# tsubo164/Fujiyama-Renderer

Hardware: AMD Instinct MI355X
Metric: Mray/s primary+secondary (and ms/frame) at 1920x1080 64spp (higher is better)
Workload: dtype f64; 1 GPU; dragon-class scene, 1920x1080, 8x8 spp, tile 32x32, 2040 tiles, 32 point lights; mesh=dragon, parallelism=tiles%1, tile_deal=auto, blas_build=host binned SAH

## Files before the change

### fujiyama-renderer_amd/csrc/device/fjgpu_api.hip

```cpp
#include <hip/hip_runtime.h>
#include <mutex>
#include <map>
#include <dlfcn.h>

#include <algorithm>
#include <array>
#include <atomic>
#include <cfloat>
#include <cmath>
#include <cstdio>
#include <cstdint>
#include <cstring>
#include <chrono>
#include <functional>
#include <memory>
#include <string>
#include <thread>
#include <vector>

#include "fjgpu.h"
#include "fjgpu_api_common.h"
#include "fjgpu_build.h"
#include "fjgpu_kernels.h"
#include "fjgpu_lbvh.h"
#include "fjgpu_light_cone.h"
#include "fjgpu_light_hull.h"
#include "fjgpu_matte.h"
#include "fjgpu_raysort.h"
#include "fjgpu_scene.h"
#include "fjgpu_tlas.h"

static thread_local std::string t_last_error;

int fjgpu::fail(int code, const std::string &msg)
{
  t_last_error = msg;
  return code;
}

namespace {

using fjgpu::fail;
using fjgpu::DeviceBuffers;

struct Rccl {
  typedef void *comm_t;
  int (*CommInitAll)(comm_t *, int, const int *) = nullptr;
  int (*CommDestroy)(comm_t) = nullptr;
  int (*GroupStart)() = nullptr;
  int (*GroupEnd)() = nullptr;
  int (*Send)(const void *, size_t, int, int, comm_t, hipStream_t) = nullptr;
  int (*Recv)(void *, size_t, int, int, comm_t, hipStream_t) = nullptr;
  const char *(*GetErrorString)(int) = nullptr;
  void *handle = nullptr;
  bool ok = false;
  static constexpr int kFloat = 7;
};

Rccl &rccl()
{
  static Rccl R;
  static std::once_flag once;
  std::call_once(once, []() {
    for (const char *name : {"librccl.so.1", "librccl.so", "/opt/rocm/lib/librccl.so.1"}) { R.handle = dlopen(name, RTLD_NOW | RTLD_LOCAL); if (R.handle) break; }
    if (!R.handle) return;
    auto sym = [&](const char *n) { return dlsym(R.handle, n); };
    R.CommInitAll = (decltype(R.CommInitAll)) sym("ncclCommInitAll");
    R.CommDestroy = (decltype(R.CommDestroy)) sym("ncclCommDestroy");
    R.GroupStart = (decltype(R.GroupStart)) sym("ncclGroupStart");
    R.GroupEnd = (decltype(R.GroupEnd)) sym("ncclGroupEnd");
    R.Send = (decltype(R.Send)) sym("ncclSend");
    R.Recv = (decltype(R.Recv)) sym("ncclRecv");
    R.GetErrorString = (decltype(R.GetErrorString)) sym("ncclGetErrorString");
    R.ok = R.CommInitAll && R.CommDestroy && R.GroupStart && R.GroupEnd && R.Send && R.Recv;
  });
  return R;
}

#define FJ_RCCL_RETRY_CALLS 64
// ... 176 lines not shown
int fjgpu_global_option(const char *name, long value)
{
  if (!name) return fail(FJGPU_EINVAL, "bad option call");
  if (std::string(name) == "ray_sort") { g_ray_sort = value < -1 ? -1 : (value > 9 ? 9 : value); return 0; }
  if (std::string(name) == "ray_sort_min") { g_ray_sort_min = value < 1 ? 1 : value; return 0; }
  if (std::string(name) == "device_tlas") { g_device_tlas = value != 0; return 0; }
  if (std::string(name) == "tlas_verify") { g_tlas_verify = value != 0; return 0; }
  if (std::string(name) == "split_shadow") { g_split_shadow = value != 0; return 0; }
  if (std::string(name) == "inst_lds") { g_inst_lds = value != 0; return 0; }
  if (std::string(name) == "curve_anyhit") { g_curve_anyhit = value != 0; return 0; }
  if (std::string(name) == "flat_groups") { g_flat_groups = value < 0 ? 0 : (value > 2 ? 2 : value); return 0; }
  if (std::string(name) == "compact_squeue") { g_compact_squeue = value != 0; return 0; }
  if (std::string(name) == "batch_tiles") { g_batch_tiles = value < 0 ? 0 : value; return 0; }
  if (std::string(name) == "device_build") { g_device_build = value < 0 ? -1 : (value > 2 ? 2 : value); return 0; }
  if (std::string(name) == "blas_treelet_passes") { g_treelet_passes = value < 0 ? 0 : (value > 8 ? 8 : value); return 0; }
  if (std::string(name) == "single_frame_build") { g_single_frame = value != 0; return 0; }
  if (std::string(name) == "speculative_walk") { g_spec_walk = value != 0; return 0; }
  if (std::string(name) == "anyhit_filter_off") { set_anyhit_filter_off(value); return 0; }
  if (std::string(name) == "cold_start") { g_cold_start = value != 0; return 0; }
  if (std::string(name) == "cold_batch_samples") { g_cold_batch_samples = value > 0 ? value : (long) FJ_COLD_BATCH_SAMPLES; return 0; }
  if (std::string(name) == "multi_exchange") { if (value < 0 || value > 1) return fail(FJGPU_EINVAL, "multi_exchange: 0 peer copies, 1 RCCL send / recv"); g_multi_exchange = value; return 0; }
  return fail(FJGPU_EINVAL, std::string("unknown global option ") + name);
}

const char *fjgpu_last_error(void) { return t_last_error.c_str(); }

int fjgpu_device_count(void)
{
  int n = 0;
  if (hipGetDeviceCount(&n) != hipSuccess) return 0;
  return n;
}

int fjgpu_tile_count(const fj_render_desc *render)
{
  if (!render) return 0;
  if (const char *why = bad_tiling(render)) { (void) fail(FJGPU_EINVAL, why); return 0; }
  std::vector<fjgpu::TileRect> t;
  fjgpu::GenerateTiles(*render, &t);
  return (int) t.size();
}

int fjgpu_tile_rect(const fj_render_desc *render, int tile_id, int32_t rect[4])
{
  if (!render || !rect) return fail(FJGPU_EINVAL, "null argument");
  if (const char *why = bad_tiling(render)) return fail(FJGPU_EINVAL, why);
  std::vector<fjgpu::TileRect> t;
  fjgpu::GenerateTiles(*render, &t);
  if (tile_id < 0 || tile_id >= (int) t.size()) return FJGPU_EINVAL;
  rect[0] = t[tile_id].xmin; rect[1] = t[tile_id].ymin; rect[2] = t[tile_id].xmax; rect[3] = t[tile_id].ymax;
  return 0;
}

}

static void build_light_hull_rows(const fjgpu::HostScene &hs, const std::vector<double> &cone_reach, std::vector<DLightCone> &hulls,
    std::vector<int32_t> &rows, int *n_rows, int *n_records)
{
  const size_t nl = hs.light_samples.size();
  rows.assign(hs.groups.size(), -1);
  hulls.clear();
  if (!hs.area_lights.empty()) return;
  for (size_t g = 0; g < hs.groups.size() && nl; g++) {
    if (hs.groups[g].n_instances != 1) continue;
    const DInstance &I = hs.instances[hs.group_members[hs.group_member_first[g]]];
    const fjgpu::HostPrimSet &ps = hs.primsets[I.primset];
    if (I.xform >= 0 || ps.type != FJ_PRIMSET_MESH || !ps.mesh || ps.mesh->velocity || ps.mesh->n_points <= 0) continue;
    std::vector<size_t> lights;
    for (size_t l = 0; l < nl; l++) if (hs.light_samples[l].type == FJ_POINT_LIGHT) lights.push_back(l);
    if (lights.empty()) continue;
    const size_t nv = (size_t) ps.mesh->n_points, nk = lights.size();
    const size_t chunk = 16384, nchunks = (nv + chunk - 1) / chunk;
    size_t workers = std::min(16u, std::max(1u, std::thread::hardware_concurrency()));
    if (const char *omp = getenv("OMP_NUM_THREADS")) { const long v = atol(omp); if (v >= 1) workers = std::min<size_t>(workers, (size_t) v); }
    const unsigned hc = (unsigned) std::max<size_t>(1, std::min(workers, nchunks));
    auto over_chunks = [&](const std::function<void(size_t)> &fn) {
      std::atomic<size_t> next(0);
      std::vector<std::thread> th;
      for (unsigned t = 0; t < hc; t++) th.emplace_back([&]() { for (size_t c; (c = next.fetch_add(1)) < nchunks;) fn(c); });
      for (auto &t : th) t.join();
    };
    std::vector<double> W(3 * nv), csum(3 * nchunks, 0.);
    over_chunks([&](size_t c) {
      double s[3] = {0., 0., 0.};
      for (size_t i = c * chunk; i < std::min(nv, (c + 1) * chunk); i++) {
        light_hull_world(I.M, ps.mesh->P + 3 * i, &W[3 * i]);
        for (int k = 0; k < 3; k++) s[k] += W[3 * i + k];
      }
      for (int k = 0; k < 3; k++) csum[3 * c + k] = s[k];
    });
    double ctr[3] = {0., 0., 0.};
    for (size_t c = 0; c < nchunks; c++) for (int k = 0; k < 3; k++) ctr[k] += csum[3 * c + k];
    for (int k = 0; k < 3; k++) ctr[k] /= (double) nv;
    std::vector<LightHullAcc> acc(nk), part(nk * nchunks);
    for (size_t k = 0; k < nk; k++) light_hull_frame(hs.light_samples[lights[k]].P, ctr, &acc[k]);
    over_chunks([&](size_t c) {
      for (size_t k = 0; k < nk; k++) {
        LightHullAcc A = acc[k];
        for (size_t i = c * chunk; i < std::min(nv, (c + 1) * chunk) && A.ok; i++) light_hull_add(&A, &W[3 * i]);
        part[k * nchunks + c] = A;
      }
    });
    for (size_t k = 0; k < nk; k++) for (size_t c = 0; c < nchunks; c++) light_hull_merge(&acc[k], &part[k * nchunks + c]);
    const size_t at = hulls.size();
    hulls.resize(at + nl);
    std::memset(&hulls[at], 0, nl * sizeof(DLightCone));
// ... 134 lines not shown
    const fj_texture_desc &t = desc->textures[i];
    dtex[i].width = t.width; dtex[i].height = t.height; dtex[i].nchannels = t.nchannels; dtex[i].tilesize = t.tilesize;
    const size_t n = (t.width && t.tiles) ? (size_t) (t.width / t.tilesize) * (t.height / t.tilesize) * t.tilesize * t.tilesize * t.nchannels : 0;
    e |= M.upload(t.tiles, n, &dtex[i].tiles);
    if (!dtex[i].tiles) dtex[i].width = dtex[i].height = 0;
  }
  DScene &S = sc->S;
  std::memset(&S, 0, sizeof(S));
  {
    std::vector<std::array<double, 6>> qgrid(dps.size());
    for (size_t i = 0; i < dps.size(); i++) {
      DPrimSet &P = dps[i];
      P.qnodes = nullptr;
      if (P.type != FJ_PRIMSET_MESH || P.n_prims == 0 || e) continue;
      const size_t n_nodes = std::max<size_t>(1, hs.primsets[i].nodes.size());
      for (int a = 0; a < 3; a++) {
        qgrid[i][a] = P.bounds[a];
        qgrid[i][3 + a] = std::max(1e-300, (P.bounds[3 + a] - P.bounds[a]) / 65535. * (1 + 1e-9));
      }
      DNodeQ *q = nullptr;
      if (M.alloc(n_nodes, &q)) { e = 1; continue; }
      if (launch_quantize_nodes(nullptr, P.nodes, (uint32_t) n_nodes, &qgrid[i][0], &qgrid[i][3], q)) e = 1;
      P.qnodes = q;
    }
    std::vector<const DNodeQ *> cq(dps.size(), nullptr);
    for (size_t i = 0; FJ_CURVE_QNODES && FJ_CLOSEST_QNODES && i < dps.size(); i++) {
      const DPrimSet &P = dps[i];
      if (P.type != FJ_PRIMSET_CURVE || P.n_prims == 0 || e) continue;
      const size_t n_nodes = std::max<size_t>(1, hs.primsets[i].nodes.size());
      for (int a = 0; a < 3; a++) {
        const double pad = 1e-4 * std::max(1., P.bounds[3 + a] - P.bounds[a]);
        qgrid[i][a] = P.bounds[a] - pad;
        qgrid[i][3 + a] = std::max(1e-300, (P.bounds[3 + a] - P.bounds[a] + 2 * pad) / 65535. * (1 + 1e-9));
      }
      DNodeQ *q = nullptr;
      if (M.alloc(n_nodes, &q)) { e = 1; continue; }
      if (launch_quantize_nodes(nullptr, P.nodes, (uint32_t) n_nodes, &qgrid[i][0], &qgrid[i][3], q)) e = 1;
      cq[i] = q;
    }
    lap("quantised nodes");
    e |= M.upload(dps.data(), dps.size(), &S.primsets);
    {
      std::vector<DInstance> di = hs.instances;
      for (DInstance &I : di) {
        const DPrimSet &P = dps[I.primset];
        std::memcpy(I.pbounds, P.bounds, sizeof(I.pbounds));
        I.pnodes = P.nodes; I.proot = P.root; I.pn_prims = P.n_prims;
        I.pqnodes = P.qnodes ? P.qnodes : cq[I.primset];
        I.sh_indices = P.indices; I.sh_N = P.N; I.sh_vN = P.vN; I.sh_uv = P.uv; I.sh_face_group = P.face_group; I.sh_type = P.type; I.sh_pad = 0;
        for (int k = 0; k < 3; k++) { I.qorigin[k] = qgrid[I.primset][k]; I.qcell[k] = qgrid[I.primset][3 + k]; }
      }
      e |= M.upload(di.data(), di.size(), &S.instances);
      std::vector<DInstEntry> ie(di.size());
      bool any_curves = false, any_motion = !hs.xforms.empty();
      for (const auto &ps : hs.primsets) {
        if (ps.type == FJ_PRIMSET_CURVE && ps.n_prims > 0) any_curves = true;
        if (!ps.tri_vel.empty() || !ps.curve_vel.empty()) any_motion = true;
      }
      for (size_t k = 0; k < di.size(); k++) {
        const DInstance &I = di[k];
        DInstEntry &E = ie[k];
        std::memcpy(E.Minv, I.Minv, sizeof(E.Minv));
        std::memcpy(E.pbounds, I.pbounds, sizeof(E.pbounds));
        for (int a = 0; a < 3; a++) { E.tbounds[a] = -INFINITY; E.tbounds[3 + a] = INFINITY; }
        if (I.xform < 0 && I.pn_prims > 0) {
          double mn[3] = {INFINITY, INFINITY, INFINITY}, mx[3] = {-INFINITY, -INFINITY, -INFINITY};
          for (int c = 0; c < 8; c++) {
            const double p[3] = {I.pbounds[(c & 1) ? 3 : 0], I.pbounds[(c & 2) ? 4 : 1], I.pbounds[(c & 4) ? 5 : 2]};
            for (int a = 0; a < 3; a++) {
              const double w = I.M[4 * a] * p[0] + I.M[4 * a + 1] * p[1] + I.M[4 * a + 2] * p[2] + I.M[4 * a + 3];
              mn[a] = std::min(mn[a], w); mx[a] = std::max(mx[a], w);
            }
          }
          bool finite = true;
          for (int a = 0; a < 3; a++) finite = finite && std::isfinite(mn[a]) && std::isfinite(mx[a]);
          if (finite)
            for (int a = 0; a < 3; a++) {
              const double pad = 1e-7 * (mx[a] - mn[a]) + 1e-7 * std::max(std::fabs(mn[a]), std::fabs(mx[a])) + 1e-9;
              E.tbounds[a] = mn[a] - pad; E.tbounds[3 + a] = mx[a] + pad;
            }
        }
        for (int a = 0; a < 3; a++) { E.qorigin[a] = I.qorigin[a]; E.qcell[a] = I.qcell[a]; }
        const DPrimSet &P = dps[I.primset];
        const bool quantised = FJ_CLOSEST_QNODES && (!any_curves || FJ_CURVE_QNODES) && !any_motion;
        E.nodes = quantised ? (const void *) I.pqnodes : (const void *) I.pnodes;
        E.ptype = P.type; E.pad = 0;
        E.proot = I.proot; E.pn_prims = I.pn_prims; E.primset = I.primset; E.xform = I.xform;
        E.tri_verts = P.tri_verts; E.tri_verts32 = P.type == FJ_PRIMSET_CURVE ? P.curve_capsule : P.tri_verts32; E.tri_vel = P.tri_vel; E.prim_ids = P.prim_ids;
      }
      e |= M.upload(ie.data(), ie.size(), &S.inst_entries);
    }
    uintptr_t lo = UINTPTR_MAX, hi = 0;
    auto tris_of = [](const DPrimSet &P) { return (uintptr_t) (P.tri_verts32 ? (const void *) P.tri_verts32 : (const void *) P.tri_verts); };
    for (size_t i = 0; i < dps.size(); i++) {
      const DPrimSet &P = dps[i];
      if (!P.qnodes) continue;
      const uintptr_t pn = (uintptr_t) P.qnodes, pt = tris_of(P);
      lo = std::min(lo, std::min(pn, pt)); hi = std::max(hi, std::max(pn, pt));
    }
    bool fits = lo != UINTPTR_MAX && lo % 128 == 0 && (hi - lo) / 128 < 0xffffffffull;
    for (size_t i = 0; i < dps.size(); i++) {
      const DPrimSet &P = dps[i];
      if (P.qnodes && (((uintptr_t) P.qnodes - lo) % 128 != 0 || (tris_of(P) - lo) % 128 != 0)) fits = false;
    }
    for (const DPrimSet &P : dps) if (P.qnodes && !P.tri_verts32) fits = false;
    S.blas_base = fits ? (const char *) lo : nullptr;
    if (!fits && lo != UINTPTR_MAX && getenv("FJGPU_VERBOSE"))
      fprintf(stderr, "fjgpu: BLAS arrays span %zu bytes from %p: no 32-bit offsets, the general shadow walk is used\n", (size_t) (hi - lo), (void *) lo);
    std::vector<DAnyInst> ai(hs.instances.size());
    for (size_t i = 0; i < hs.instances.size(); i++) {
      const DInstance &I = hs.instances[i];
      const DPrimSet &P = dps[I.primset];
      DAnyInst &a = ai[i];
      std::memset(&a, 0, sizeof(a));
      std::memcpy(a.Minv, I.Minv, sizeof(a.Minv));
      std::memcpy(a.bounds, P.bounds, sizeof(a.bounds));
      a.root = P.root;
      a.n_prims = (P.qnodes && S.blas_base) ? P.n_prims : 0;
      if (a.n_prims) {
        for (int k = 0; k < 3; k++) { a.qorigin[k] = qgrid[I.primset][k]; a.qcell[k] = qgrid[I.primset][3 + k]; }
        a.node_base = (uint32_t) (((uintptr_t) P.qnodes - lo) / 128);
        a.tri_base = (uint32_t) ((tris_of(P) - lo) / 128);
        a.tris_f32 = P.tri_verts32 ? 1 : 0;
        double bm = 0;
        for (int k = 0; k < 6; k++) bm = std::max(bm, std::fabs(P.bounds[k]));
        a.fbound = std::nextafter((float) bm, INFINITY);
      }
    }
    e |= M.upload(ai.data(), ai.size(), &S.any_insts);
  }
  if (g_device_tlas && e == 0 && !hs.groups.empty()) {
    std::vector<int> mcount(hs.groups.size()), nfirst, ncount;
    for (size_t g = 0; g < hs.groups.size(); g++) mcount[g] = hs.groups[g].n_instances;
    DTNode *d_nodes = nullptr;
    std::string terr;
    if (TlasBuildDevice(S.instances, hs.group_members, hs.group_member_first, mcount, &nfirst, &ncount, &d_nodes, &terr))
      return fail(FJGPU_ENODEV, terr);
    M.ptrs.push_back(d_nodes);
    size_t total = 0;
    for (int c : ncount) total += (size_t) c;
    if (g_tlas_verify) {
      std::vector<DTNode> got(total);
      HIP_TRY(hipMemcpy(got.data(), d_nodes, total * sizeof(DTNode), hipMemcpyDeviceToHost));
      bool same = total == hs.group_nodes.size();
      for (size_t g = 0; same && g < hs.groups.size(); g++) same = nfirst[g] == hs.groups[g].first && ncount[g] == hs.groups[g].count;
      if (same && total) same = std::memcmp(got.data(), hs.group_nodes.data(), total * sizeof(DTNode)) == 0;
      if (!same) return fail(FJGPU_ENODEV, "device TLAS build differs from the host's build");
    }
    std::vector<DGroup> groups = hs.groups;
    for (size_t g = 0; g < groups.size(); g++) { groups[g].first = nfirst[g]; groups[g].count = ncount[g]; }
    e |= M.upload(groups.data(), groups.size(), &S.groups);
    S.group_nodes = d_nodes;
    S.n_group_nodes = (int32_t) total;
  } else {
    e |= M.upload(hs.groups.data(), hs.groups.size(), &S.groups);
    e |= M.upload(hs.group_nodes.data(), hs.group_nodes.size(), &S.group_nodes);
    S.n_group_nodes = (int32_t) hs.group_nodes.size();
  }
  static_assert(sizeof(DInstEntry) == 8 * FJ_INST_LDS_ENTRY_WORDS && sizeof(DTNode) == 56 && sizeof(DGroup) == 64, "LDS copy of the instance level");
  S.curve_anyhit = (g_curve_anyhit && !getenv("FJGPU_NO_CURVE_ANYHIT")) ? 1 : 0;
  S.inst_lds = (g_inst_lds && !getenv("FJGPU_NO_INST_LDS")) ? 1 : 0;
  e |= M.upload(hs.shaders.data(), hs.shaders.size(), &S.shaders);
  e |= M.upload(hs.xforms.data(), hs.xforms.size(), &S.xforms);
  S.cam_xform = nullptr;
  if (!hs.cam_static) e |= M.upload(&hs.cam_xform, 1, &S.cam_xform);
  S.has_motion = hs.xforms.empty() ? 0 : 1;
  for (const auto &ps : hs.primsets) if (!ps.tri_vel.empty() || !ps.curve_vel.empty()) S.has_motion = 1;
  S.multi_shadow_groups = 0;
  for (const DInstance &I : hs.instances) {
    bool gathers = false;
    for (int k = 0; k < I.n_shaders; k++)
      if (I.shaders[k] >= 0 && (hs.shaders[I.shaders[k]].type == FJ_SHADER_PLASTIC || hs.shaders[I.shaders[k]].type == FJ_SHADER_HAIR)) gathers = true;
    if (gathers && I.shadow_target >= 0 && I.shadow_target < (int) hs.groups.size() && hs.groups[I.shadow_target].n_instances > 1)
      S.multi_shadow_groups = 1;
  }
  S.time_tab = nullptr; S.time_start = 0; S.time_end = 0;
  S.lrec_hair = nullptr;
  e |= M.upload(dtex.data(), dtex.size(), &S.textures);
  e |= M.upload(hs.light_samples.data(), hs.light_samples.size(), &S.light_samples);
  e |= M.upload(hs.area_lights.data(), hs.area_lights.size(), &S.area_lights);
  S.light_cones = nullptr; S.cone_rows = nullptr;
  std::vector<double> cone_reach;
  {
    const size_t nl = hs.light_samples.size();
    std::vector<int32_t> rows(hs.groups.size(), -1);
    std::vector<DLightCone> cones;
    cone_reach.assign(hs.groups.size(), -1.);
    for (size_t g = 0; g < hs.groups.size() && nl; g++) {
      if (hs.groups[g].n_instances != 1) continue;
      const size_t at = cones.size();
      cones.resize(at + nl);
      int built = 0;
      double reach = 1e300;
      for (size_t l = 0; l < nl; l++) {
        DLightCone &C = cones[at + l];
        const DLightSample &LS = hs.light_samples[l];
        if (LS.type == FJ_POINT_LIGHT || LS.type == FJ_DOME_LIGHT) light_cone_build(LS.P, hs.groups[g].sbounds, &C);
        else std::memset(&C, 0, sizeof(C));
        if (C.count > 0) { built++; reach = std::min(reach, C.reach); }
      }
      if (!built) { cones.resize(at); continue; }
      for (size_t l = 0; l < nl; l++) cones[at + l].reach = reach;
      rows[g] = (int32_t) (at / nl);
      cone_reach[g] = reach;
      sc->cone_rows++; sc->cone_records += built;
    }
    if (!cones.empty()) {
      e |= M.upload(cones.data(), cones.size(), &S.light_cones);
      e |= M.upload(rows.data(), rows.size(), &S.cone_rows);
    }
  }
  S.light_hulls = nullptr; S.hull_rows = nullptr;
  {
// ... 187 lines not shown
  for (hipEvent_t e : scene->ev_frame) if (e) (void) hipEventDestroy(e);
  for (hipEvent_t e : scene->ev_pool) (void) hipEventDestroy(e);
  if (scene->d_frame) (void) hipFree(scene->d_frame);
  if (scene->d_slab) (void) hipFree(scene->d_slab);
  if (scene->d_rects) (void) hipFree(scene->d_rects);
  delete scene;
}

int fjgpu_host_instance_level(const fj_scene_desc *desc, int group, int32_t *out_inst, int32_t *out_skip, double *out_box, int cap)
{
  if (!desc || group < 0 || group >= desc->n_groups) return fail(FJGPU_EINVAL, "bad instance-level query");
  fjgpu::HostScene hs;
  std::string err;
  const int e = fjgpu::BuildHostScene(desc, &hs, &err, true);
  if (e) return fail(e, err);
  const DGroup &G = hs.groups[group];
  for (int k = 0; k < G.count && k < cap; k++) {
    const DTNode &nd = hs.group_nodes[G.first + k];
    if (out_inst) out_inst[k] = nd.inst;
    if (out_skip) out_skip[k] = nd.inst < 0 ? nd.skip - G.first : 0;
    if (out_box) std::memcpy(out_box + 6 * (size_t) k, nd.box, sizeof(nd.box));
  }
  return G.count;
}

int fjgpu_host_light_hulls(const fj_scene_desc *desc, int group, void *out_records, double *out_Pl, int cap, double *out_M)
{
  if (!desc || group < 0 || group >= desc->n_groups) return fail(FJGPU_EINVAL, "bad light-hull query");
  fjgpu::HostScene hs;
  std::string err;
  const int e = fjgpu::BuildHostScene(desc, &hs, &err, true);
  if (e) return fail(e, err);
  std::vector<int32_t> rows;
  std::vector<DLightCone> hulls;
  int n_rows = 0, n_records = 0;
  std::vector<double> cone_reach(hs.groups.size(), -1.);
  for (size_t g = 0; g < hs.groups.size(); g++) cone_reach[g] = box_cone_row_reach(hs, g);
  build_light_hull_rows(hs, cone_reach, hulls, rows, &n_rows, &n_records);
  if (out_M) {
    if (hs.groups[group].n_instances != 1) return fail(FJGPU_EINVAL, "light-hull query: the group has several instances");
    std::memcpy(out_M, hs.instances[hs.group_members[hs.group_member_first[group]]].M, 12 * sizeof(double));
  }
  const size_t nl = hs.light_samples.size();
  for (size_t l = 0; l < nl && (int) l < cap; l++) {
    if (out_records) {
      if (rows[group] >= 0) std::memcpy((char *) out_records + l * sizeof(DLightCone), &hulls[(size_t) rows[group] * nl + l], sizeof(DLightCone));
      else std::memset((char *) out_records + l * sizeof(DLightCone), 0, sizeof(DLightCone));
    }
    if (out_Pl) for (int k = 0; k < 3; k++) out_Pl[3 * l + k] = hs.light_samples[l].P[k];
  }
  return (int) nl;
}

int fjgpu_host_curve_blas(const fj_scene_desc *desc, int curve_set, int32_t *out_curve, float *out_capsule, int32_t *out_depth,
                          float *out_box, int cap, int32_t *out_grid_n, double *out_grid_cell, double *out_bounds)
{
  if (!desc || curve_set < 0 || curve_set >= desc->n_curves) return fail(FJGPU_EINVAL, "bad curve-BLAS query");
  fjgpu::HostPrimSet ps;
  std::string err;
  const int e = fjgpu::BuildCurveSet(desc->curves[curve_set], &ps, &err);
  if (e) return fail(e, err);
  const int n = ps.n_prims;
  for (int k = 0; k < 3; k++) {
    if (out_grid_n) out_grid_n[k] = ps.grid_n[k];
    if (out_grid_cell) out_grid_cell[k] = ps.grid_cell[k];
  }
  if (out_bounds) std::memcpy(out_bounds, ps.bounds, sizeof(ps.bounds));
  for (int s = 0; s < n && s < cap; s++) {
    if (out_curve) out_curve[s] = (int32_t) ps.prim_ids[s];
    if (out_capsule) std::memcpy(out_capsule + 7 * (size_t) s, &ps.curve_capsule[(size_t) s * 8], 7 * sizeof(float));
    if (out_depth) out_depth[s] = ps.curve_depth[s];
  }
  if (out_box && n > 0) {
    if (ps.root & FJ_LEAF_FLAG) {
      if (cap > 0) for (int k = 0; k < 6; k++) out_box[k] = (float) ps.bounds[k];
    } else {
      std::vector<char> seen((size_t) n, 0);
      std::vector<uint32_t> todo(1, ps.root);
      while (!todo.empty()) {
        const uint32_t at = todo.back();
        todo.pop_back();
        if (at >= ps.nodes.size()) return fail(FJGPU_EINVAL, "curve-BLAS query: node index out of range");
        const DNode &nd = ps.nodes.data()[at];
        for (int k = 0; k < 4; k++) {
          const uint32_t c = nd.child[k];
          if (c == FJ_NO_CHILD) continue;
          if (!(c & FJ_LEAF_FLAG)) { todo.push_back(c); continue; }
          const uint32_t first = (c & ~FJ_LEAF_FLAG) >> 3, count = (c & 7u) + 1;
          for (uint32_t s = first; s < first + count && s < (uint32_t) n; s++) {
            seen[s] = 1;
            if ((int) s < cap) for (int a = 0; a < 3; a++) { out_box[6 * (size_t) s + a] = nd.box[k][2 * a]; out_box[6 * (size_t) s + 3 + a] = nd.box[k][2 * a + 1]; }
          }
        }
      }
      for (int s = 0; s < n; s++) if (!seen[s]) return fail(FJGPU_EINVAL, "curve-BLAS query: a slot has no leaf");
    }
  }
  return n;
}

int fjgpu_build_config(const char *name, double *value)
{
  if (!name || !value) return fail(FJGPU_EINVAL, "bad build_config call");
  if (!kernels_build_config(name, value)) return fail(FJGPU_EINVAL, std::string("unknown build_config name ") + name);
  return 0;
}
// ... 5 lines not shown
  if (n == "node_record_bytes") { *value = (double) sizeof(DNode); return 0; }
  if (n == "anyhit_node_record_bytes") { *value = (double) sizeof(DNodeQ); return 0; }
  if (n == "tri_record_bytes") { *value = scene->tri_record_bytes; return 0; }
  if (n == "scene_bytes") { *value = (double) scene->mem.bytes; return 0; }
  if (n == "work_bytes") { *value = (double) (scene->work ? scene->work->bytes : 0); return 0; }
  if (n == "stack_need") { *value = scene->stack_need; return 0; }
  if (n == "sampler_seed") { *value = (double) scene->sampler_seed; return 0; }
  if (n == "blas_nodes") { *value = (double) scene->blas_nodes; return 0; }
  if (n == "blas_treelet_passes") { *value = (double) scene->blas_treelet_passes; return 0; }
  if (n == "blas_treelets_changed") { *value = (double) scene->blas_treelets_changed; return 0; }
  if (n == "blas_sah_cost_initial") { *value = scene->blas_sah_cost_initial; return 0; }
  if (n == "blas_sah_cost") { *value = scene->blas_sah_cost; return 0; }
  if (n == "stack_peak") { *value = (double) std::max(scene->stack_peak_closest, scene->stack_peak_shadow); return 0; }
  if (n == "stack_peak_closest") { *value = (double) scene->stack_peak_closest; return 0; }
  if (n == "stack_peak_shadow") { *value = (double) scene->stack_peak_shadow; return 0; }
  if (n == "stack_lds") { *value = FJ_STACK_LDS; return 0; }
  if (n == "stack_lds_anyhit") { *value = FJ_STACK_LDS_ANYHIT; return 0; }
  if (n == "stack_lds_curves") { *value = FJ_STACK_LDS_CURVES; return 0; }
  if (n == "stack_lds_canyhit") { *value = FJ_STACK_LDS_CANYHIT; return 0; }
  if (n == "stack_lds_min") { *value = FJ_STACK_LDS_MIN; return 0; }
  if (n == "curve_anyhit") {
    const DScene &S = scene->S;
    *value = (S.has_curves && !S.has_motion && S.all_opaque && S.curve_anyhit && S.inst_lds && S.n_group_nodes <= FJ_INST_LDS_NODES_CURVES &&
              S.n_instances <= FJ_INST_LDS_INSTS_CURVES && S.n_groups <= FJ_INST_LDS_GROUPS_CURVES && FJ_CURVE_QNODES && FJ_CLOSEST_QNODES) ? 1 : 0;
    return 0;
  }
  if (n == "lean_anyhit") { *value = (scene->S.all_opaque && !scene->S.has_curves && !scene->S.has_motion && scene->S.blas_base) ? 1 : 0; return 0; }
  if (n == "closest_kernel") {
    const DScene &S = scene->S;
    const bool flat = !S.has_motion && !S.has_curves && S.flats;
    *value = S.has_motion ? 3 : (S.has_curves ? 2 : (flat ? 4 : (S.incoherent_rays ? 1 : 0)));
    return 0;
  }
  if (n == "closest_node_record_bytes") { *value = (double) ((scene->S.has_motion || (scene->S.has_curves && !FJ_CURVE_QNODES) || !FJ_CLOSEST_QNODES) ? sizeof(DNode) : sizeof(DNodeQ)); return 0; }
  if (n == "light_cone_rows") { *value = scene->cone_rows; return 0; }
  if (n == "light_cone_records") { *value = scene->cone_records; return 0; }
  if (n == "light_cone_verdicts" || n == "light_cone_contradictions") {
    double v = -1, c = -1;
    if (hipSetDevice(scene->device) != hipSuccess || hipDeviceSynchronize() != hipSuccess) return fail(FJGPU_ENODEV, "hipSetDevice / hipDeviceSynchronize");
    light_cone_validate_counts(&v, &c);
    *value = n == "light_cone_verdicts" ? v : c;
    return 0;
  }
  if (n == "light_hull_rows") { *value = scene->hull_rows; return 0; }
  if (n == "light_hull_records") { *value = scene->hull_records; return 0; }
  if (n == "light_hull_verdicts" || n == "light_hull_contradictions") {
    double v = -1, c = -1;
    if (hipSetDevice(scene->device) != hipSuccess || hipDeviceSynchronize() != hipSuccess) return fail(FJGPU_ENODEV, "hipSetDevice / hipDeviceSynchronize");
    light_hull_validate_counts(&v, &c);
    if (n == "light_hull_verdicts") *value = v >= 0 ? v : (double) scene->hull_verdicts;
    else *value = c;
    return 0;
  }
  {
    static const char *const tf[5] = {"tri_filter_miss", "tri_filter_hit", "tri_filter_maybe", "tri_filter_exact_hits", "tri_filter_contradictions"};
    for (int k = 0; k < 5; k++)
      if (n == tf[k]) {
        double c[5];
        if (hipSetDevice(scene->device) != hipSuccess || hipDeviceSynchronize() != hipSuccess) return fail(FJGPU_ENODEV, "hipSetDevice / hipDeviceSynchronize");
        tri_filter_validate_counts(c);
        *value = c[k];
        return 0;
      }
  }
  if (n == "accum_memsets") { *value = (double) scene->accum_memsets; return 0; }
  if (n == "has_curves") { *value = scene->S.has_curves; return 0; }
  if (n == "has_motion") { *value = scene->S.has_motion; return 0; }
  return fail(FJGPU_EINVAL, "unknown query " + n);
}

int fjgpu_set_batch_callback(fjgpu_scene *scene, fjgpu_batch_fn fn, void *user)
{
  if (!scene) return fail(FJGPU_EINVAL, "null scene");
  scene->batch_fn = fn; scene->batch_user = fn ? user : nullptr;
  return 0;
}

int fjgpu_dev_rccl_selftest(int device, int n_floats)
{
  int nd = 0;
  if (hipGetDeviceCount(&nd) != hipSuccess || device < 0 || device >= nd) return fail(FJGPU_ENODEV, "no such HIP device");
  if (n_floats < 1) return fail(FJGPU_EINVAL, "bad size");
  HIP_TRY(hipSetDevice(device));
  std::string why;
  const std::vector<Rccl::comm_t> *comms = rccl_comms(std::vector<int>{device}, &why);
  if (!comms) return fail(FJGPU_ENODEV, "RCCL: " + why);
  Rccl &R = rccl();
  DeviceBuffers M;
  std::vector<float> src((size_t) n_floats), got((size_t) n_floats, -1.f);
  for (int i = 0; i < n_floats; i++) src[(size_t) i] = (float) (i % 1013) * .5f;
  const float *d_src = nullptr;
  float *d_dst = nullptr;
  if (M.upload(src.data(), src.size(), &d_src) || M.alloc(src.size(), &d_dst)) return fail(FJGPU_ENOMEM, "device allocation failed");
  HIP_TRY(hipMemset(d_dst, 0xff, sizeof(float) * src.size()));
  int e = R.GroupStart();
  if (!e) e = R.Send(d_src, src.size(), Rccl::kFloat, 0, (*comms)[0], nullptr);
  if (!e) e = R.Recv(d_dst, src.size(), Rccl::kFloat, 0, (*comms)[0], nullptr);
  const int e2 = R.GroupEnd();
  if (e || e2) return fail(FJGPU_ENODEV, std::string("RCCL self exchange: ") + (R.GetErrorString ? R.GetErrorString(e ? e : e2) : "error"));
  HIP_TRY(hipStreamSynchronize(nullptr));
  HIP_TRY(hipMemcpy(got.data(), d_dst, sizeof(float) * got.size(), hipMemcpyDeviceToHost));
  for (size_t i = 0; i < got.size(); i++) if (got[i] != src[i]) return fail(FJGPU_ENODEV, "RCCL self exchange returned other data");
  return 0;
}

int fjgpu_dev_sort_pairs(int device, const uint32_t *keys, int n, int key_bits, uint32_t *keys_out, uint32_t *perm, int repeats, double *sort_ms)
// ... 28 lines not shown
  if (sort_ms) *sort_ms = best;
  if (keys_out) HIP_TRY(hipMemcpy(keys_out, d_out, sizeof(uint32_t) * (size_t) n, hipMemcpyDeviceToHost));
  if (perm) HIP_TRY(hipMemcpy(perm, d_perm, sizeof(uint32_t) * (size_t) n, hipMemcpyDeviceToHost));
  return 0;
}

int fjgpu_dev_slab32_batch(int device, int n, const double *rays, const double *grid, const uint32_t *words, void *out)
{
  if (n < 0 || (n > 0 && (!rays || !grid || !words || !out))) return fail(FJGPU_EINVAL, "bad slab32 batch call");
  int nd = 0;
  if (hipGetDeviceCount(&nd) != hipSuccess || device < 0 || device >= nd) return fail(FJGPU_ENODEV, "no such HIP device");
  HIP_TRY(hipSetDevice(device));
  if (n == 0) return 0;
  DeviceBuffers M;
  const double *d_rays = nullptr, *d_grid = nullptr;
  const uint32_t *d_words = nullptr;
  char *d_out = nullptr;
  if (M.upload(rays, (size_t) n * 8, &d_rays) || M.upload(grid, (size_t) n * 6, &d_grid) || M.upload(words, (size_t) n * 3, &d_words) || M.alloc((size_t) n * 128, &d_out))
    return fail(FJGPU_ENOMEM, "device allocation failed for the slab32 batch");
  if (launch_slab32_batch(nullptr, (uint32_t) n, d_rays, d_grid, d_words, d_out)) return fail(FJGPU_ENODEV, "the slab32 batch launch failed");
  HIP_TRY(hipStreamSynchronize(nullptr));
  HIP_TRY(hipMemcpy(out, d_out, (size_t) n * 128, hipMemcpyDeviceToHost));
  return 0;
}

int fjgpu_dev_quantize_nodes(int device, int n, const void *nodes, const double *origin, const double *cell, void *out)
{
  if (n < 0 || !origin || !cell || (n > 0 && (!nodes || !out))) return fail(FJGPU_EINVAL, "bad quantize call");
  int nd = 0;
  if (hipGetDeviceCount(&nd) != hipSuccess || device < 0 || device >= nd) return fail(FJGPU_ENODEV, "no such HIP device");
  HIP_TRY(hipSetDevice(device));
  if (n == 0) return 0;
  DeviceBuffers M;
  const DNode *d_nodes = nullptr;
  DNodeQ *d_out = nullptr;
  if (M.upload((const DNode *) nodes, (size_t) n, &d_nodes) || M.alloc((size_t) n, &d_out)) return fail(FJGPU_ENOMEM, "device allocation failed for the quantiser");
  if (launch_quantize_nodes(nullptr, d_nodes, (uint32_t) n, origin, cell, d_out)) return fail(FJGPU_ENODEV, "the quantiser's launch failed");
  HIP_TRY(hipStreamSynchronize(nullptr));
  HIP_TRY(hipMemcpy(out, d_out, sizeof(DNodeQ) * (size_t) n, hipMemcpyDeviceToHost));
  return 0;
}

int fjgpu_set_option(fjgpu_scene *scene, const char *name, long value)
{
  if (!scene || !name) return fail(FJGPU_EINVAL, "bad option call");
  const std::string n(name);
  if (n == "batch_tiles") { scene->batch_tiles = value; return 0; }
  if (n == "batch_samples") { scene->batch_samples = value < 0 ? 0 : value; return 0; }
  if (n == "aov_batch_samples") { scene->aov_batch_samples = value < 0 ? 0 : value; return 0; }
  if (n == "count_nodes") { scene->count_events = value != 0; return 0; }
  if (n == "count_all_shadow") { scene->count_all_shadow = value != 0; return 0; }
  if (n == "light_cones") { scene->light_cones = value != 0; return 0; }
  if (n == "light_hulls") { scene->light_hulls = value != 0; return 0; }
  if (n == "shade_first_touch") {
    if (value != 0 && value != 1) return fail(FJGPU_EINVAL, "shade_first_touch: 0 (memset and atomic adds at the camera level) or 1 (one store per sample)");
    scene->shade_first_touch = value;
    return 0;
  }
  if (n == "sampler_seed") {
    if (value < 0 || value > 65535) return fail(FJGPU_EINVAL, "sampler_seed: " + std::to_string(value) + " is outside 0..65535 (0: the unseeded streams)");
    scene->sampler_seed = value;
    return 0;
  }
  if (n == "overlap_shadow") {
    if (value < 0 || value > 2) return fail(FJGPU_EINVAL, "overlap_shadow: 0 off, 1 on, 2 by the batch size");
    scene->overlap = value;
    return 0;
  }
  if (n == "release_work") {
    if (value && scene->work) {
      if (hipSetDevice(scene->device) != hipSuccess) return fail(FJGPU_ENODEV, "hipSetDevice");
      (void) hipDeviceSynchronize();
      fjgpu::ForgetWorkArena(scene);
    }
    return 0;
  }
  return fail(FJGPU_EINVAL, "unknown option " + n);
}

int fjgpu_render_frame_multi(fjgpu_scene *const *scenes, int n_scenes, const fj_render_desc *r,
    const int32_t *tile_ids, int n_tiles, float *h_fb, fjgpu_stats *stats)
{
  if (!scenes || n_scenes < 1 || !r || !h_fb) return fail(FJGPU_EINVAL, "null argument");
  for (int k = 0; k < n_scenes; k++) if (!scenes[k]) return fail(FJGPU_EINVAL, "null scene");
  if (const char *why = bad_render(r)) return fail(FJGPU_EINVAL, why);
  std::vector<fjgpu::TileRect> all;
  fjgpu::GenerateTiles(*r, &all);
  std::vector<int32_t> ids;
  if (const int e = listed_tiles(tile_ids, n_tiles, all.size(), &ids)) return e;
  const int G = n_scenes;
  const size_t npx = (size_t) r->xres * r->yres;
  const int tile_px = r->tile_w * r->tile_h;
  std::vector<std::vector<int32_t>> mine(G);
  for (size_t k = 0; k < ids.size(); k++) mine[k % G].push_back(ids[k]);
  fjgpu_scene *first = scenes[0];

  HIP_TRY(hipSetDevice(first->device));
  if (grow((void **) &first->d_frame, &first->d_frame_n, npx * 4, sizeof(float))) return fail(FJGPU_ENOMEM, "device allocation failed for the frame");
  HIP_TRY(hipMemset(first->d_frame, 0, npx * 4 * sizeof(float)));
  std::vector<size_t> stage_off(G, 0);
  size_t stage_px = 0, rects_n = 0;
  for (int d = 1; d < G; d++) { stage_off[d] = stage_px; stage_px += mine[d].size() * (size_t) tile_px; rects_n += mine[d].size(); }
  if (G > 1) {
    if (grow((void **) &first->d_slab, &first->d_slab_n, stage_px * 4, sizeof(float)) ||
        grow((void **) &first->d_rects, &first->d_rects_n, rects_n * 4, sizeof(int32_t)))
      return fail(FJGPU_ENOMEM, "device allocation failed for the tile slabs");
// ... 113 lines not shown
  return fjgpu_render_frame_multi(one, 1, r, nullptr, 0, h_fb, stats);
}

int fjgpu_trace(fjgpu_scene *sc, int group, int n, const double *rays, double *out_t, int32_t *out_ids,
    double *out_uv, fjgpu_stats *stats)
{
  if (!sc || !rays || !out_t || !out_ids || n < 0) return fail(FJGPU_EINVAL, "null argument");
  if (group < 0 || group >= sc->S.n_groups) return fail(FJGPU_EINVAL, "group out of range");
  if (n == 0) return 0;
  HIP_TRY(hipSetDevice(sc->device));
  DeviceBuffers W;
  DRay *d_rays; DHit *d_hits; DCounters *d_cnt;
  double *d_ranges;
  if (W.alloc((size_t) n, &d_rays) || W.alloc((size_t) n * 2, &d_ranges) || W.alloc((size_t) n, &d_hits) || W.alloc(1, &d_cnt))
    return fail(FJGPU_ENOMEM, "device allocation failed");
  {
    std::vector<DRay> hr((size_t) n);
    std::vector<double> hg((size_t) n * 2);
    for (int i = 0; i < n; i++) {
      for (int k = 0; k < 3; k++) { hr[i].o[k] = rays[8 * (size_t) i + k]; hr[i].d[k] = rays[8 * (size_t) i + 3 + k]; }
      hg[2 * (size_t) i] = rays[8 * (size_t) i + 6]; hg[2 * (size_t) i + 1] = rays[8 * (size_t) i + 7];
    }
    HIP_TRY(hipMemcpy(d_rays, hr.data(), sizeof(DRay) * (size_t) n, hipMemcpyHostToDevice));
    HIP_TRY(hipMemcpy(d_ranges, hg.data(), sizeof(double) * 2 * (size_t) n, hipMemcpyHostToDevice));
  }
  HIP_TRY(hipMemset(d_cnt, 0, sizeof(DCounters)));
  DScene S = sc->S;
  S.target_group = group;
  S.trace_ranges = d_ranges;
  hipEvent_t e0, e1;
  HIP_TRY(hipEventCreate(&e0));
  HIP_TRY(hipEventCreate(&e1));
  (void) hipEventRecord(e0, nullptr);
  const int le = launch_trace_closest(nullptr, S, d_rays, nullptr, d_hits, (uint32_t) n, d_cnt, (int) sc->count_events);
  (void) hipEventRecord(e1, nullptr);
  if (le) return fail(FJGPU_ENODEV, std::string("trace launch: ") + hipGetErrorString((hipError_t) le));
  HIP_TRY(hipDeviceSynchronize());
  float ms = 0;
  (void) hipEventElapsedTime(&ms, e0, e1);
  (void) hipEventDestroy(e0); (void) hipEventDestroy(e1);
  std::vector<DHit> h((size_t) n);
  HIP_TRY(hipMemcpy(h.data(), d_hits, sizeof(DHit) * (size_t) n, hipMemcpyDeviceToHost));
  for (int i = 0; i < n; i++) {
    out_t[i] = h[i].inst >= 0 ? h[i].t : DBL_MAX;
    out_ids[2 * i] = h[i].inst;
    out_ids[2 * i + 1] = h[i].inst >= 0 ? h[i].prim : -1;
    if (out_uv) { out_uv[2 * i] = h[i].inst >= 0 ? h[i].u : 0; out_uv[2 * i + 1] = h[i].inst >= 0 ? h[i].v : 0; }
  }
  sc->stack_peak_closest = sc->stack_peak_shadow = 0;
  DCounters hc;
  if (stats || sc->count_events) {
    HIP_TRY(hipMemcpy(&hc, d_cnt, sizeof(hc), hipMemcpyDeviceToHost));
    sc->stack_peak_closest = hc.stack_peak;
  }
  if (stats) {
    std::memset(stats, 0, sizeof(*stats));
    stats->nodes_visited = hc.nodes; stats->prims_tested = hc.prims; stats->insts_tested = hc.insts; stats->rays_traced = hc.traced;
    stats->trace_ms = ms; stats->total_ms = ms; stats->trace_launches = 1;
  }
  return 0;
}

#ifndef FJ_AOV_BATCH_SAMPLES
#define FJ_AOV_BATCH_SAMPLES ((long) 4 << 20)
#endif

struct AovSetup {
  std::vector<fjgpu::TileRect> all;
  int margin[2];
  GenParams gp;
  DScene S;
};
static int aov_setup(fjgpu_scene *sc, const fj_render_desc *r, const char *who, AovSetup *a)
{
  if (r->sampler_type == 1) return fail(FJGPU_EUNSUPPORTED, std::string(who) + ": the adaptive sampler is not supported (fixed-grid sampler only)");
  if (r->sampler_type != 0) return fail(FJGPU_EINVAL, "unknown sampler_type");
  if (const char *why = bad_render(r)) return fail(FJGPU_EINVAL, why);
  if (sc->S.cam_xform) return fail(FJGPU_EUNSUPPORTED, std::string(who) + ": a time-sampled camera is not supported (static cameras only)");
  if (sc->S.has_motion) return fail(FJGPU_EUNSUPPORTED, std::string(who) + ": a scene with motion (time-sampled transforms or vertex velocities) is not supported (static scenes only)");
  fjgpu::GenerateTiles(*r, &a->all);
  fjgpu::SamplerMargin(*r, a->margin);
  a->gp = gen_params(r, a->margin);
  a->S = sc->S;
  camera_uv_size(sc->cam_fov, r, a->S.cam_uv_size);
  a->S.time_start = r->time_start; a->S.time_end = r->time_end;
  a->S.lrec_hair = nullptr;
  a->S.cam_uv = nullptr; a->S.cam_tk = nullptr; a->S.cam_slot0 = 0;
  a->S.trace_ranges = nullptr; a->S.trace_n_dev = nullptr; a->S.ray_perm = nullptr;
  a->S.shadow_join = nullptr;
  return 0;
}

struct MatteCall { const fjgpu_matte_desc *desc; const fjgpu_matte_buffers *out; };
static int render_aov_body(const char *who_, fjgpu_scene *sc, const fj_render_desc *r, const int32_t *tile_ids, int n_tiles,
    const fjgpu_aov_buffers *out, float *d_albedo, void *hip_stream, fjgpu_stats *stats, const MatteCall *matte = nullptr)
{
  const std::string who(who_);
  const bool reduce = out && (out->depth || out->position || out->normal || out->uv || out->ids || out->coverage);
  if (!reduce && !d_albedo && !matte) return fail(FJGPU_EINVAL, who + ": every buffer pointer is NULL, nothing to write");
  if (tile_ids && n_tiles < 0) return fail(FJGPU_EINVAL, who + ": negative tile count");
  AovSetup A;
  if (const int e = aov_setup(sc, r, who_, &A)) return e;
  HIP_TRY(hipSetDevice(sc->device));
  hipStream_t st = static_cast<hipStream_t>(hip_stream);

  std::vector<int32_t> ids;
// ... 226 lines not shown
```

### fujiyama-renderer_amd/csrc/device/fjgpu_dev_math.h

```cpp
#ifndef FJGPU_DEV_MATH_H
#define FJGPU_DEV_MATH_H

#include "fjgpu_slab32.h"
__device__ __forceinline__ V3 mk(double x, double y, double z) { V3 r; r.x = x; r.y = y; r.z = z; return r; }
__device__ __forceinline__ V3 operator+(V3 a, V3 b) { return mk(a.x + b.x, a.y + b.y, a.z + b.z); }
__device__ __forceinline__ V3 operator-(V3 a, V3 b) { return mk(a.x - b.x, a.y - b.y, a.z - b.z); }
__device__ __forceinline__ V3 operator*(V3 a, double s) { return mk(a.x * s, a.y * s, a.z * s); }
__device__ __forceinline__ V3 operator*(double s, V3 a) { return mk(a.x * s, a.y * s, a.z * s); }
__device__ __forceinline__ double dot(V3 a, V3 b) { return a.x * b.x + a.y * b.y + a.z * b.z; }
__device__ __forceinline__ V3 cross(V3 a, V3 b) { return mk(a.y * b.z - a.z * b.y, a.z * b.x - a.x * b.z, a.x * b.y - a.y * b.x); }
__device__ __forceinline__ V3 normalize(V3 a)
{
  const double len = sqrt(dot(a, a));
  if (len == 0) return a;
  const double inv = 1. / len;
  return a * inv;
}
#define FJ_GLOBAL __attribute__((address_space(1)))
typedef float fj_v4f __attribute__((ext_vector_type(4)));
typedef uint32_t fj_v4u __attribute__((ext_vector_type(4)));

__device__ __forceinline__ V3 ld3(const double *p) { return mk(p[0], p[1], p[2]); }
__device__ __forceinline__ V3 ld3(const FJ_GLOBAL double *p) { return mk(p[0], p[1], p[2]); }
#define FJ_G(T, ptr) ((const FJ_GLOBAL T *) (ptr))
// ... 100 lines not shown
    *v0 = mk(p[0], p[1], p[2]); *v1 = mk(p[3], p[4], p[5]); *v2 = mk(p[6], p[7], p[8]);
  }
}

__device__ __forceinline__ bool tri_ray(V3 v0, V3 v1, V3 v2, V3 orig, V3 dir, double *t, double *u, double *v)
{
  const V3 edge1 = v1 - v0;
  const V3 edge2 = v2 - v0;
  const V3 pvec = cross(dir, edge2);
  const double det = dot(edge1, pvec);
  if (det > -1e-6 && det < 1e-6) return false;
  const double inv_det = 1.0 / det;
  const V3 tvec = orig - v0;
  const double uu = dot(tvec, pvec) * inv_det;
  if (uu < 0.0 || uu > 1.0) return false;
  const V3 qvec = cross(tvec, edge1);
  const double vv = dot(dir, qvec) * inv_det;
  if (vv < 0.0 || uu + vv > 1.0) return false;
  *t = dot(edge2, qvec) * inv_det;
  *u = uu;
  *v = vv;
  return true;
}

__device__ __forceinline__ bool tri_ray_early(V3 v0, V3 v1, V3 v2, V3 orig, V3 dir, double *t, double *u, double *v)
{
  const V3 edge1 = v1 - v0;
  const V3 edge2 = v2 - v0;
  const V3 pvec = cross(dir, edge2);
  const double det = dot(edge1, pvec);
  if (det > -1e-6 && det < 1e-6) return false;
  const double adet = fabs(det);
  const V3 tvec = orig - v0;
  const double U = dot(tvec, pvec);
  const double aU = fabs(U);
  if (((U < 0.0) != (det < 0.0)) ? aU > 1e-100 * adet : aU > adet * (1.0 + 1e-10)) return false;
  const V3 qvec = cross(tvec, edge1);
  const double V = dot(dir, qvec);
  const double aV = fabs(V);
  if (((V < 0.0) != (det < 0.0)) ? aV > 1e-100 * adet : aV > adet * (1.0 + 1e-10)) return false;
  const double inv_det = 1.0 / det;
  const double uu = U * inv_det;
  if (uu < 0.0 || uu > 1.0) return false;
  const double vv = V * inv_det;
  if (vv < 0.0 || uu + vv > 1.0) return false;
  *t = dot(edge2, qvec) * inv_det;
  *u = uu;
  *v = vv;
  return true;
}

struct Best { double t, u, v; int inst, prim; };

struct LocalCounters { uint32_t nodes, prims, insts, stack_peak; };

__device__ __forceinline__ unsigned long long wave_sum(unsigned long long v)
{
  for (int off = 32; off > 0; off >>= 1) {
    const unsigned lo = __shfl_xor((unsigned) (v & 0xffffffffull), off);
    const unsigned hi = __shfl_xor((unsigned) (v >> 32), off);
    v += ((unsigned long long) hi << 32) | lo;
  }
  return v;
}

__device__ __forceinline__ void flush_counters(DCounters *cnt, unsigned long long nodes, unsigned long long prims,
    unsigned long long insts, unsigned long long traced, unsigned long long shadow)
{
  nodes = wave_sum(nodes); prims = wave_sum(prims); insts = wave_sum(insts);
  traced = wave_sum(traced); shadow = wave_sum(shadow);
  if (__lane_id() == 0) {
    if (nodes) atomicAdd(&cnt->nodes, nodes);
    if (prims) atomicAdd(&cnt->prims, prims);
    if (insts) atomicAdd(&cnt->insts, insts);
    if (traced) atomicAdd(&cnt->traced, traced);
    if (shadow) atomicAdd(&cnt->rays[CXT_SHADOW_RAY], shadow);
  }
}

__device__ __forceinline__ void flush_stack_peak(unsigned long long *peak, uint32_t v)
{
  for (int off = 32; off > 0; off >>= 1) { const uint32_t o = __shfl_xor(v, off); v = o > v ? o : v; }
  if (__lane_id() == 0 && v) atomicMax(peak, (unsigned long long) v);
}

__device__ __forceinline__ void flush_shadow_walk_counters(DCounters *cnt, unsigned long long nodes, unsigned long long prims,
    unsigned long long insts)
{
  nodes = wave_sum(nodes); prims = wave_sum(prims); insts = wave_sum(insts);
  if (__lane_id() == 0) {
    if (nodes) atomicAdd(&cnt->sh_nodes, nodes);
    if (prims) atomicAdd(&cnt->sh_prims, prims);
    if (insts) atomicAdd(&cnt->sh_insts, insts);
  }
}

#endif
```

### fujiyama-renderer_amd/csrc/device/fjgpu_dev_shadow.h

```cpp
#ifndef FJGPU_DEV_SHADOW_H
#define FJGPU_DEV_SHADOW_H

#ifndef SQ_CHUNK
#define SQ_CHUNK 512u
#endif
#ifndef JQ_CHUNK
#define JQ_CHUNK 64u
#endif
#define SQ_INVALID 0xffffffffu
__device__ __forceinline__ const DShadowRayC *sq_c(const DShadowRay *squeue, uint32_t i) { return (const DShadowRayC *) squeue + i; }
#define SQ_FIELD(S, squeue, i, f) ((S).compact_squeue ? sq_c(squeue, i)->f : (squeue)[i].f)
__device__ __forceinline__ const float *sq_colour(const DScene &S, const DShadowRay *squeue, uint32_t i) { return S.compact_squeue ? sq_c(squeue, i)->c : squeue[i].c; }
__device__ __forceinline__ void sq_ray(const DScene &S, const DShadowRay *squeue, uint32_t i, V3 *o, V3 *d, double *tmax)
{
  if (!S.compact_squeue) {
    const DShadowRay *q = &squeue[i];
    *o = mk(q->o[0], q->o[1], q->o[2]); *d = mk(q->d[0], q->d[1], q->d[2]); *tmax = q->tmax;
    return;
  }
  const DShadowRayC *q = sq_c(squeue, i);
  const V3 Ps = mk(q->o[0], q->o[1], q->o[2]);
  const DLightSample *LS = &S.light_samples[q->light];
  const V3 Pl = mk(LS->P[0], LS->P[1], LS->P[2]);
  V3 Ln = mk(Pl.x - Ps.x, Pl.y - Ps.y, Pl.z - Ps.z);
// ... 422 lines not shown
  const DShadowRay *squeue;
  float *s_accum;
  __device__ bool fetch(uint32_t i, RayIn *r) const
  {
    const DShadowRay q = squeue[i];
    if (q.sample == SQ_INVALID) return false;
    r->o = mk(q.o[0], q.o[1], q.o[2]); r->d = mk(q.d[0], q.d[1], q.d[2]);
    r->tmin = .0001; r->tmax = q.tmax;
    r->time = S->has_motion ? sample_time(*S, q.tindex) : 0.;
    r->group = q.group;
    r->anyhit = S->groups[q.group].all_opaque != 0;
    return true;
  }
  __device__ void finish(uint32_t i, const Best &b) const
  {
    float ac = 1.f;
    if (b.inst >= 0) {
      float Os = 1.f;
      const DInstance *I = &S->instances[b.inst];
      const DPrimSet *P = &S->primsets[I->primset];
      const int sg = (P->face_group && b.prim >= 0) ? P->face_group[b.prim] : 0;
      int sid;
      if (sg < 0 || sg >= I->n_shaders) sid = I->shaders[0];
      else { sid = I->shaders[sg]; if (sid < 0) sid = I->shaders[0]; }
      if (sid >= 0 && S->shaders[sid].type == FJ_SHADER_PLASTIC) Os = S->shaders[sid].opacity;
      Os = (float) clampd(Os, 0, 1);
      ac = 1 - Os;
    }
    if (ac == 0.f) return;
    const DShadowRay *q = &squeue[i];
    const float r0 = q->c[0] * ac, r1 = q->c[1] * ac, r2 = q->c[2] * ac;
    float *acc = s_accum + 4 * (size_t) q->sample;
    if (r0 != 0.f) atomicAdd(acc + 0, r0);
    if (r1 != 0.f) atomicAdd(acc + 1, r1);
    if (r2 != 0.f) atomicAdd(acc + 2, r2);
  }
};

template <bool kCurves, bool kCount, bool kMotion, bool kInstLds = false, bool kAnyOnly = false>
__global__ void __launch_bounds__(BLOCK, kMotion ? FJ_MOTION_MINB : (kCurves ? FJ_CURVE_MINB : FJ_SHADOW_MINB)) k_shadow_trace(DScene S, const DShadowRay *squeue, float *s_accum,
    DCounters *cnt, TravTune tune)
{
  __shared__ uint32_t s_stack[(kCurves ? FJ_STACK_LDS_CURVES : FJ_STACK_LDS) * BLOCK];
  __shared__ double s_rayspace[kCurves ? FJ_RAYSPACE_DOUBLES * BLOCK : 1];
  __shared__ double s_inst[kInstLds ? InstLdsOf<kCurves>::T::WORDS : 1];
  if (kInstLds) InstLdsOf<kCurves>::T::fill(S, s_inst);
  const uint32_t n = cnt->shadow_count;
  ShadowPolicy pol;
  pol.S = &S; pol.squeue = squeue; pol.s_accum = s_accum;
  LocalCounters lc = {0, 0, 0, 0};
  traverse_persistent<kCurves, kCount, kMotion, kInstLds, kAnyOnly>(S, pol, tune, n, &cnt->shadow_xcd_head[0][0], make_stack(s_stack, S.stack_overflow_shadow, kCurves ? s_rayspace : nullptr), &lc, s_inst);
  if (kCount) {
    flush_counters(cnt, lc.nodes, lc.prims, lc.insts, 0, 0);
    flush_stack_peak(&cnt->sh_stack_peak, lc.stack_peak);
    flush_shadow_walk_counters(cnt, lc.nodes, lc.prims, lc.insts);
    if (blockIdx.x == 0 && threadIdx.x == 0) atomicAdd(&cnt->squeued, (unsigned long long) n);
  }
}

#endif
```

### fujiyama-renderer_amd/csrc/device/fjgpu_dev_traverse.h

```cpp
#ifndef FJGPU_DEV_TRAVERSE_H
#define FJGPU_DEV_TRAVERSE_H

#define TRAV_DONE 0xffffffffu
#ifndef FJ_TINY_PRIMS
#define FJ_TINY_PRIMS 4
#endif
#ifdef FJ_PHASE_STATS
__device__ unsigned long long g_phase[16];
#endif
#ifdef FJ_WAVE_TIMELINE
#define FJ_TL_WAVES 8192
__device__ unsigned long long g_timeline[FJ_TL_WAVES * 6];
struct WaveTimeline {
  unsigned long long t0, tdry, tclaim;
  uint32_t iters, tail, iclaim, worst_ticks, worst_iters, claims;
  __device__ __forceinline__ void begin() { t0 = tclaim = wall_clock64(); tdry = 0; iters = tail = iclaim = worst_ticks = worst_iters = claims = 0; }
  __device__ __forceinline__ void iter(bool dry) { iters++; if (dry) { if (!tdry) tdry = wall_clock64(); tail++; } }
  __device__ __forceinline__ void claim()
  {
    const unsigned long long now = wall_clock64();
    const uint32_t d = (uint32_t) (now - tclaim);
    if (claims && d > worst_ticks) { worst_ticks = d; worst_iters = iters - iclaim; }
    tclaim = now; iclaim = iters; claims++;
  }
  __device__ __forceinline__ void end()
  {
    claim();
    const uint32_t w = blockIdx.x * (BLOCK / 64) + (threadIdx.x >> 6);
    if (__lane_id() == 0 && w < FJ_TL_WAVES) {
      const unsigned long long t1 = wall_clock64();
      g_timeline[6 * w + 0] = t0; g_timeline[6 * w + 1] = tdry ? tdry : t1; g_timeline[6 * w + 2] = t1;
      g_timeline[6 * w + 3] = ((unsigned long long) iters << 32) | tail;
      g_timeline[6 * w + 4] = ((unsigned long long) worst_ticks << 32) | worst_iters;
      g_timeline[6 * w + 5] = claims;
    }
  }
};
__device__ unsigned long long g_rayhist[64];
#ifdef FJ_RAY_HIST
#define FJ_TL_RAY(steps) do { const uint32_t s_ = (steps); const int b_ = 31 - __clz((int) (s_ | 1u)); atomicAdd(&g_rayhist[b_], 1ull); atomicAdd(&g_rayhist[32 + b_], (unsigned long long) s_); } while (0)
#else
#define FJ_TL_RAY(steps) do { } while (0)
#endif
#define FJ_TL_CLAIM() tl_.claim()
#define FJ_TL_DECL() WaveTimeline tl_; tl_.begin()
#define FJ_TL_ITER(dry) tl_.iter(dry)
#define FJ_TL_END() tl_.end()
#else
#define FJ_TL_RAY(steps) do { } while (0)
#define FJ_TL_CLAIM() do { } while (0)
#define FJ_TL_DECL() do { } while (0)
#define FJ_TL_ITER(dry) do { } while (0)
#define FJ_TL_END() do { } while (0)
#endif
struct TravTune { uint32_t refill, steps, grab, leaf_wait, min_inner, anyhit_steps, refill_curves, steps_curves, steps_phased, min_inner_phased, refill_canyhit, steps_canyhit, min_inner_canyhit, leaf_wait_canyhit, refill_flat, steps_flat, min_inner_flat, leaf_bias8, leaf_bias8_flat, leaf_bias8_phased, leaf_bias8_canyhit, exact_min, filter_off; };
#define TRAV_REFILL tune.refill
#define TRAV_STEPS (int) tune.steps
#define TRAV_GRAB tune.grab

__device__ __forceinline__ uint32_t adaptive_grab(uint32_t grab, uint32_t n)
{
// ... 51 lines not shown
  uint32_t ovf_stride;
  double *rayspace;
  int lds_n;
  __device__ __forceinline__ void push(int &sp, uint32_t v) const
  {
    if (sp < lds_n) lds[sp * BLOCK] = v;
    else ovf[(size_t) (sp - lds_n) * ovf_stride] = v;
    sp++;
  }
  __device__ __forceinline__ uint32_t pop(int &sp) const
  {
    --sp;
    uint32_t v;
    if (sp < lds_n) v = lds[sp * BLOCK];
    else v = ovf[(size_t) (sp - lds_n) * ovf_stride];
    return v;
  }
};
__device__ __forceinline__ TravStack make_stack(uint32_t *s_stack, uint32_t *ovf, double *s_rayspace = nullptr, int lds_entries = 0)
{
  TravStack st;
  st.lds = (trav_lds_u32 *) (s_stack + threadIdx.x);
  st.lds_n = lds_entries ? lds_entries : (s_rayspace ? FJ_STACK_LDS_CURVES : FJ_STACK_LDS);
  st.rayspace = s_rayspace ? s_rayspace + threadIdx.x : nullptr;
  st.ovf_stride = gridDim.x * BLOCK;
  st.ovf = ovf ? (FJ_GLOBAL uint32_t *) (ovf + (size_t) blockIdx.x * BLOCK + threadIdx.x) : nullptr;
  return st;
}

template <int NODES_, int INSTS_, int GROUPS_> struct InstLdsT {
  static constexpr int NODES = NODES_, INSTS = INSTS_, GROUPS = GROUPS_;
  static constexpr int ENTRIES_AT = NODES * 7, GROUPS_AT = ENTRIES_AT + INSTS * FJ_INST_LDS_ENTRY_WORDS;
  static constexpr int WORDS = GROUPS_AT + GROUPS * 8;
  static bool fits(const DScene &S)
  {
    return S.inst_lds && S.n_group_nodes <= NODES && S.n_instances <= INSTS && S.n_groups <= GROUPS;
  }
  static __device__ __forceinline__ void fill(const DScene &S, double *s_inst)
  {
    const unsigned long long *src_n = (const unsigned long long *) S.group_nodes, *src_e = (const unsigned long long *) S.inst_entries;
    const unsigned long long *src_g = (const unsigned long long *) S.groups;
    unsigned long long *dst = (unsigned long long *) s_inst;
    for (uint32_t w = threadIdx.x; w < (uint32_t) S.n_group_nodes * 7u; w += BLOCK) dst[w] = src_n[w];
    for (uint32_t w = threadIdx.x; w < (uint32_t) S.n_instances * FJ_INST_LDS_ENTRY_WORDS; w += BLOCK) dst[ENTRIES_AT + w] = src_e[w];
    for (uint32_t w = threadIdx.x; w < (uint32_t) S.n_groups * 8u; w += BLOCK) dst[GROUPS_AT + w] = src_g[w];
    __syncthreads();
  }
};
typedef InstLdsT<FJ_INST_LDS_NODES, FJ_INST_LDS_INSTS, FJ_INST_LDS_GROUPS> InstLds;
typedef InstLdsT<FJ_INST_LDS_NODES_BIG, FJ_INST_LDS_INSTS_BIG, FJ_INST_LDS_GROUPS_BIG> InstLdsBig;
typedef InstLdsT<FJ_INST_LDS_NODES_CURVES, FJ_INST_LDS_INSTS_CURVES, FJ_INST_LDS_GROUPS_CURVES> InstLdsCurves;
template <bool kCurves> struct InstLdsOf { typedef InstLdsBig T; };
template <> struct InstLdsOf<true> { typedef InstLdsCurves T; };

template <bool kCurves, bool kCount, bool kMotion, bool kInstLds, bool kAnyOnly, class Policy>
__device__ void traverse_persistent(const DScene &S, Policy &pol, TravTune tune, uint32_t n, uint32_t *head, TravStack stk, LocalCounters *lc, const double *s_inst)
{
  const DTNode *gnodes = kInstLds ? (const DTNode *) s_inst : S.group_nodes;
  typedef typename InstLdsOf<kCurves>::T IL;
  const DInstEntry *gents = kInstLds ? (const DInstEntry *) (s_inst + IL::ENTRIES_AT) : S.inst_entries;
  const DGroup *ggroups = kInstLds ? (const DGroup *) (s_inst + IL::GROUPS_AT) : S.groups;
  const unsigned lane = __lane_id();
  bool head_live = true;
  const unsigned long long lt_mask = (1ull << lane) - 1ull;
  uint32_t next = 0, range_end = 0;
  tune.grab = adaptive_grab(tune.grab, n);
  QueueClaim qc;
  qc.init(head, n, tune.grab);
  if (kCurves) { tune.refill = tune.refill_curves; tune.steps = tune.steps_curves; }
  bool have = false;
  uint32_t idx = 0;
  V3 o = mk(0, 0, 0), oo = o, od = o, d = o, winv = o;
  Slab32 s32 = {{0, 0, 0}, {0, 0, 0}, {0, 0, 0}};
  double tmin = kAnyOnly ? .0001 : 0, tmax = 0, rtime = 0;
  Best best;
  best.t = DBL_MAX; best.u = best.v = 0; best.inst = -1; best.prim = -1;
  int ti = 0, tend = 0, ii = -1;
  int group = 0;
  bool single = false;
  const double *gsb = nullptr;
  bool anyhit = kAnyOnly, dead_ray = false, plain = false;
  bool deep = false;
  const DPrimSet *P = nullptr;
  const DNode *nodes = nullptr;
  uint32_t cur = TRAV_DONE;
  uint32_t last_curve = 0xffffffffu;
  uint32_t pend = 0xffffffffu;
  int sp = 0;
#ifdef FJ_PHASE_STATS
  unsigned long long it_all = 0, it_tail = 0;
  unsigned long long cyc[4] = {0, 0, 0, 0}, c_prev = __builtin_readcyclecounter();
#define FJ_CYC(k) do { const unsigned long long c_now = __builtin_readcyclecounter(); cyc[k] += c_now - c_prev; c_prev = c_now; } while (0)
#else
#define FJ_CYC(k) do { } while (0)
#endif

  FJ_TL_DECL();
  for (;;) {
    FJ_TL_ITER(!head_live && next >= range_end);
#ifdef FJ_PHASE_STATS
    it_all++;
    if (!head_live && next >= range_end) it_tail++;
#endif
    const unsigned long long idle = __ballot(!have);
    if (next >= range_end && head_live && (idle == ~0ull || (unsigned) __popcll(idle) >= TRAV_REFILL))
      { head_live = qc.claim(lane, &next, &range_end); FJ_TL_CLAIM(); }
    if (idle == ~0ull || ((unsigned) __popcll(idle) >= TRAV_REFILL && next < range_end)) {
      if (!have) {
        const uint32_t my = next + (uint32_t) __popcll(idle & lt_mask);
        if (my < range_end) {
          RayIn r;
          r.o = r.d = mk(0, 0, 1); r.tmin = r.tmax = r.time = 0; r.group = 0; r.anyhit = false;
          have = pol.fetch(my, &r);
          idx = my;
          tmin = kAnyOnly ? .0001 : r.tmin; tmax = r.tmax; anyhit = kAnyOnly ? true : r.anyhit;
          if (kMotion) rtime = r.time;
          group = r.group;
          const DGroup *G = &ggroups[r.group];
          ti = G->first; tend = ti + G->count;
          best.t = DBL_MAX; best.u = best.v = 0; best.inst = -1; best.prim = -1;
          cur = TRAV_DONE; sp = 0;
          if (!kCurves) {
            o = r.o; d = r.d;
            single = G->n_instances == 1;
            gsb = G->sbounds;
            dead_ray = has_negative_zero(d);
            winv = mk(filter_rcp(d.x), filter_rcp(d.y), filter_rcp(d.z));
            plain = plain_dir(d);
          }
        }
      }
      next += (uint32_t) __popcll(idle);
      if (__ballot(have) == 0ull) {
        if (next >= range_end && !head_live) {
#ifdef FJ_PHASE_STATS
          if (lane == 0) { atomicMax(&g_phase[12], it_tail); atomicAdd(&g_phase[13], it_tail); atomicAdd(&g_phase[14], it_all); atomicAdd(&g_phase[15], 1ull);
            atomicAdd(&g_phase[1], cyc[0]); atomicAdd(&g_phase[3], cyc[1]); atomicAdd(&g_phase[5], cyc[2]); atomicAdd(&g_phase[7], cyc[3]); }
#endif
          FJ_TL_END();
          break;
        }
        continue;
      }
    }

    if (have && cur == TRAV_DONE && (!kCurves || pend == 0xffffffffu)) {
      bool found = false;
      uint32_t root = TRAV_DONE;
      if (kCurves) {
        RayIn r;
        r.o = r.d = mk(0, 0, 1); r.tmin = r.tmax = r.time = 0; r.group = 0; r.anyhit = false;
        pol.fetch(idx, &r);
        o = r.o; d = r.d;
        single = ggroups[group].n_instances == 1;
        gsb = ggroups[group].sbounds;
        dead_ray = has_negative_zero(d);
        winv = mk(filter_rcp(d.x), filter_rcp(d.y), filter_rcp(d.z));
        plain = plain_dir(d);
      }
      while (!dead_ray && ti < tend) {
        const DTNode *tn_ = &gnodes[ti];
        if (tn_->inst < 0) {
          double tq;
          ti = slab(tn_->box, tn_->box + 3, o, winv, tmin, tmax, &tq) ? ti + 1 : tn_->skip;
          continue;
        }
        ii = tn_->inst;
        ti++;
        const DInstEntry *I = &gents[ii];
        if (kCount) lc->insts++;
        double tn;
        const double tfar = anyhit ? tmax : fmin(tmax, best.t);
        if (!slab(I->tbounds, I->tbounds + 3, o, winv, tmin, tfar, &tn)) continue;
        if (!box_ray_ref_fast(single ? gsb : tn_->box, o, d, winv, plain, tmin, tmax)) continue;
        if (kMotion && I->xform >= 0) {
          double tm[12], tmi[12];
          xform_at(&S.xforms[I->xform], rtime, tm, tmi);
          oo = xpoint(tmi, o);
          od = xvector(tmi, d);
        } else {
          oo = xpoint(I->Minv, o);
          od = xvector(I->Minv, d);
        }
        if (has_negative_zero(od)) continue;
        const V3 inv = mk(filter_rcp(od.x), filter_rcp(od.y), filter_rcp(od.z));
        P = &S.primsets[I->primset];
        nodes = (const DNode *) I->nodes;
        if (I->pn_prims == 0) continue;
        if (!slab(I->pbounds, I->pbounds + 3, oo, inv, tmin, tfar, &tn)) continue;
        if (FJ_CLOSEST_QNODES && (!kCurves || (FJ_CURVE_QNODES && !kMotion))) s32 = slab32q_setup(oo, inv, I->qorigin, I->qcell);
        else s32 = slab32_setup(oo, inv, I->pbounds);
        root = I->proot;
        found = true;
        break;
      }
      if (found) {
        cur = root; sp = 0; last_curve = 0xffffffffu;
      }
      else { pol.finish(idx, best); have = false; }
    }

    FJ_CYC(0);
    for (int step = 0; step < TRAV_STEPS; step++) {
      const bool inner = have && !(cur & FJ_LEAF_FLAG);
      if (__ballot(inner) == 0ull) break;
        if (inner) {
        if (kCount) lc->nodes++;
        const double tf2 = anyhit ? tmax : fmin(tmax, best.t);
        const float tmin32 = f32_below(tmin), tmax32 = f32_above(tf2);
        float t0, t1, t2, t3;
        bool h0, h1, h2, h3;
        fj_v4u e;
        if (FJ_CLOSEST_QNODES && (!kCurves || (FJ_CURVE_QNODES && !kMotion))) {
          const FJ_GLOBAL fj_v4u *nq = (const FJ_GLOBAL fj_v4u *) ((const DNodeQ *) nodes + cur);
          const fj_v4u w0 = nq[0], w1 = nq[1], w2 = nq[2];
          e = nq[3];
          const uint32_t shx = slab32_shift(s32.x.i), shy = slab32_shift(s32.y.i), shz = slab32_shift(s32.z.i);
          h0 = slab32q_test(w0.x, w0.y, w0.z, s32, shx, shy, shz, tmin32, tmax32, &t0);
          h1 = slab32q_test(w0.w, w1.x, w1.y, s32, shx, shy, shz, tmin32, tmax32, &t1);
          h2 = slab32q_test(w1.z, w1.w, w2.x, s32, shx, shy, shz, tmin32, tmax32, &t2) && e.z != FJ_NO_CHILD;
          h3 = slab32q_test(w2.y, w2.z, w2.w, s32, shx, shy, shz, tmin32, tmax32, &t3) && e.w != FJ_NO_CHILD;
        } else {
        const FJ_GLOBAL fj_v4f *nd = (const FJ_GLOBAL fj_v4f *) (nodes + cur);
        const fj_v4f q0 = nd[0], q1 = nd[1], q2 = nd[2], q3 = nd[3], q4 = nd[4], q5 = nd[5];
        e = ((const FJ_GLOBAL fj_v4u *) nd)[6];
        h0 = slab32_test(q0.xy, q0.zw, q1.xy, s32, tmin32, tmax32, &t0);
        h1 = slab32_test(q1.zw, q2.xy, q2.zw, s32, tmin32, tmax32, &t1);
        h2 = e.z != FJ_NO_CHILD && slab32_test(q3.xy, q3.zw, q4.xy, s32, tmin32, tmax32, &t2);
        h3 = e.w != FJ_NO_CHILD && slab32_test(q4.zw, q5.xy, q5.zw, s32, tmin32, tmax32, &t3);
        }
        float k0 = h0 ? t0 : INFINITY, k1 = h1 ? t1 : INFINITY;
        float k2 = h2 ? t2 : INFINITY, k3 = h3 ? t3 : INFINITY;
        uint32_t r0 = e.x, r1 = e.y, r2 = e.z, r3 = e.w;
#define FJ_CSWAP(ka, ra, kb, rb) { const bool sw = kb < ka; const float tk = sw ? ka : kb; const uint32_t tr = sw ? ra : rb; ka = sw ? kb : ka; ra = sw ? rb : ra; kb = tk; rb = tr; }
        FJ_CSWAP(k0, r0, k1, r1) FJ_CSWAP(k2, r2, k3, r3) FJ_CSWAP(k0, r0, k2, r2) FJ_CSWAP(k1, r1, k3, r3) FJ_CSWAP(k1, r1, k2, r2)
#undef FJ_CSWAP
        const int nh = (int) h0 + (int) h1 + (int) h2 + (int) h3;
        if (nh == 0) cur = (sp == 0) ? TRAV_DONE : stk.pop(sp);
        else {
          cur = r0;
          if (nh > 3) stk.push(sp, r3);
          if (nh > 2) stk.push(sp, r2);
          if (nh > 1) stk.push(sp, r1);
          if (kCount && (uint32_t) sp > lc->stack_peak) lc->stack_peak = (uint32_t) sp;
        }
      }
    }

    FJ_CYC(1);
    if (have && !deep && (cur & FJ_LEAF_FLAG) && cur != TRAV_DONE) {
      const uint32_t first = (cur & 0x7fffffffu) >> 3;
      const uint32_t cnt = (cur & 7u) + 1;
      bool stop = false;
      if (kCurves && P->type == FJ_PRIMSET_CURVE) {
        const size_t sl = first;
        const uint32_t cid = FJ_G(uint32_t, P->prim_ids)[sl];
        if (cid != last_curve && (!P->curve_capsule || capsule_may_hit(FJ_G(float, P->curve_capsule) + sl * 8, oo, od))) {
          last_curve = cid;
          if (kCount) lc->prims++;
          const FJ_GLOBAL double *cvel = (kMotion && P->curve_vel) ? FJ_G(double, P->curve_vel) + sl * 12 : nullptr;
          deep = true;
          if (deep && pend == 0xffffffffu) { pend = (uint32_t) sl; deep = false; }
        }
      } else {
        for (uint32_t k = 0; k < cnt; k++) {
          double t, u = 0, v = 0;
          if (kCount) lc->prims++;
          V3 v0, v1, v2;
          load_tri(P->tri_verts, P->tri_verts32, first + k, &v0, &v1, &v2);
          if (kMotion && P->tri_vel) {
            const FJ_GLOBAL double *w = FJ_G(double, P->tri_vel) + (size_t) (first + k) * 9;
            v0 = v0 + rtime * ld3(w); v1 = v1 + rtime * ld3(w + 3); v2 = v2 + rtime * ld3(w + 6);
          }
          if (!tri_ray(v0, v1, v2, oo, od, &t, &u, &v)) continue;
          if (!(tmin <= t && t <= tmax)) continue;
          if (kAnyOnly) { stop = true; break; }
          const int pid = (int) FJ_G(uint32_t, P->prim_ids)[first + k];
          if (t < best.t || (t == best.t && best.inst == ii && pid > best.prim)) {
            best.t = t; best.u = u; best.v = v; best.inst = ii; best.prim = pid;
            if (anyhit) { stop = true; break; }
          }
        }
      }
      if (stop) { if (!kAnyOnly) pol.finish(idx, best); have = false; cur = TRAV_DONE; }
      else if (!deep) cur = (sp == 0) ? TRAV_DONE : stk.pop(sp);
    }

    FJ_CYC(2);
    if (kCurves) {
      const bool carrying = have && pend != 0xffffffffu;
      const unsigned long long pendm = __ballot(carrying);
      if (pendm) {
        const unsigned long long busym = __ballot(have && !deep && cur != TRAV_DONE);
        if ((unsigned) __popcll(pendm) >= tune.leaf_wait || busym == 0ull) {
          if (lane == (unsigned) __ffsll((long long) pendm) - 1u) { FJ_CURVE_STAT(2, 1); FJ_CURVE_STAT(3, __popcll(pendm)); }
          double t = 0, u = 0;
          bool hitc = false;
          if (carrying) {
            bool stop = false;
            const size_t sl = pend;
            pend = 0xffffffffu;
            const FJ_GLOBAL double *cvel = (kMotion && P->curve_vel) ? FJ_G(double, P->curve_vel) + sl * 12 : nullptr;
            hitc = curve_ray(FJ_G(double, P->curve_cp) + sl * 12, cvel, rtime, FJ_G(double, P->curve_width)[2 * sl], FJ_G(double, P->curve_width)[2 * sl + 1],
                          (int) FJ_G(int8_t, P->curve_depth)[sl], RaySpace{stk.rayspace, oo, od}, &t, &u);
            if (hitc &&
                (cvel ? curve_listed_in_cell_of_moving(P, FJ_G(double, P->curve_cp) + sl * 12, cvel, oo + t * od)
                      : curve_listed_in_cell_of(P, FJ_G(double, P->curve_cp) + sl * 12, oo + t * od)) &&
                (tmin <= t && t <= tmax)) {
              FJ_CURVE_STAT(4, 1);
              if (kAnyOnly) stop = true;
              else {
                const int pid = (int) FJ_G(uint32_t, P->prim_ids)[sl];
                if (t < best.t || (t == best.t && best.inst == ii && pid > best.prim)) {
                  best.t = t; best.u = u; best.v = (double) sl; best.inst = ii; best.prim = pid;
                  stop = anyhit;
                }
              }
            }
            if (stop) { if (!kAnyOnly) pol.finish(idx, best); have = false; deep = false; cur = TRAV_DONE; }
            else if (deep) {
              pend = (cur & 0x7fffffffu) >> 3;
              deep = false;
              cur = (sp == 0) ? TRAV_DONE : stk.pop(sp);
            }
          }
        }
      }
    }
    FJ_CYC(3);
  }
}

template <bool kCount, bool kMotion, bool kInstLds, class Policy>
__device__ void traverse_phased(const DScene &S, Policy &pol, TravTune tune, uint32_t n, uint32_t *head, TravStack stk, LocalCounters *lc, const double *s_inst)
{
  const DTNode *gnodes = kInstLds ? (const DTNode *) s_inst : S.group_nodes;
  const DInstEntry *gents = kInstLds ? (const DInstEntry *) (s_inst + InstLds::ENTRIES_AT) : S.inst_entries;
  const DGroup *ggroups = kInstLds ? (const DGroup *) (s_inst + InstLds::GROUPS_AT) : S.groups;
  const unsigned lane = __lane_id();
  bool head_live = true;
  uint32_t next = 0, range_end = 0;
  tune.grab = adaptive_grab(tune.grab, n);
  QueueClaim qc;
  qc.init(head, n, tune.grab);
  bool have = false;
  uint32_t idx = 0;
  V3 o = mk(0, 0, 0), oo = o, od = o, d = o;
  Slab32 s32 = {{0, 0, 0}, {0, 0, 0}, {0, 0, 0}};
  double tmin = 0, tmax = 0, rtime = 0;
  Best best;
  best.t = DBL_MAX; best.u = best.v = 0; best.inst = -1; best.prim = -1;
  int ti = 0, tend = 0, ii = -1;
  int group = 0;
  bool anyhit = false;
  const DNode *nodes = nullptr;
  uint32_t cur = TRAV_DONE;
  int sp = 0;
#ifdef FJ_PHASE_STATS
  unsigned long long pcyc[3] = {0, 0, 0}, pex[3] = {0, 0, 0}, pln[3] = {0, 0, 0}, trips_lane = 0, trips_wave = 0, pc_prev = __builtin_readcyclecounter();
#define FJ_PCYC(k, mask) do { const unsigned long long c_now = __builtin_readcyclecounter(); pcyc[k] += c_now - pc_prev; pc_prev = c_now; pex[k]++; pln[k] += __popcll(mask); } while (0)
#else
#define FJ_PCYC(k, mask) do { } while (0)
#endif

  for (;;) {
    const bool fin = cur == TRAV_DONE;
    const bool at_leaf = !fin && (cur & FJ_LEAF_FLAG);
    const bool at_inner = !fin && !at_leaf;
    const unsigned n_leaf = (unsigned) __popcll(__ballot(at_leaf)), n_inner = (unsigned) __popcll(__ballot(at_inner));
    const bool can_fetch = head_live || next < range_end;
    const unsigned long long m_turn = __ballot(fin && (have || can_fetch));

    if ((unsigned) __popcll(m_turn) >= TRAV_REFILL || (n_inner == 0 && n_leaf == 0)) {
      if (m_turn == 0ull) {
#ifdef FJ_PHASE_STATS
        if (lane == 0) {
          for (int k = 0; k < 3; k++) { atomicAdd(&g_phase[1 + 2 * k], pcyc[k]); atomicAdd(&g_phase[2 + 2 * k], pln[k]); atomicAdd(&g_phase[7 + k], pex[k]); }
          atomicAdd(&g_phase[10], trips_lane); atomicAdd(&g_phase[11], trips_wave);
        }
#endif
        break;
      }
      if (next >= range_end && head_live) head_live = qc.claim(lane, &next, &range_end);
      const bool fetch = fin && !have;
      const unsigned long long m_fetch = __ballot(fetch);
      if (fetch) {
        const uint32_t my = next + __builtin_amdgcn_mbcnt_hi((uint32_t) (m_fetch >> 32), __builtin_amdgcn_mbcnt_lo((uint32_t) m_fetch, 0u));
        if (my < range_end) {
          RayIn r;
          r.o = r.d = mk(0, 0, 1); r.tmin = r.tmax = r.time = 0; r.group = 0; r.anyhit = false;
          have = pol.fetch(my, &r);
          idx = my;
          o = r.o; d = r.d; tmin = r.tmin; tmax = r.tmax; anyhit = r.anyhit;
          if (kMotion) rtime = r.time;
          group = r.group;
          ti = ggroups[group].first; tend = ti + ggroups[group].count;
          best.t = DBL_MAX; best.u = best.v = 0; best.inst = -1; best.prim = -1;
          sp = 0;
        }
      }
      next += (uint32_t) __popcll(m_fetch);
      if (next > range_end) next = range_end;
#ifdef FJ_PHASE_STATS
      unsigned my_trips = 0;
#endif
      if (fin && have) {
        bool found = false;
        uint32_t root = TRAV_DONE;
        const bool dead_ray = has_negative_zero(d);
        const V3 winv = mk(filter_rcp(d.x), filter_rcp(d.y), filter_rcp(d.z));
        const bool plain = plain_dir(d);
        const bool single = ggroups[group].n_instances == 1;
        const double *gsb = ggroups[group].sbounds;
        while (!dead_ray && ti < tend) {
#ifdef FJ_PHASE_STATS
          my_trips++;
#endif
          const DTNode *tn_ = &gnodes[ti];
          int inst_ = tn_->inst;
          while (inst_ < 0) {
            double tq;
            ti = slab(tn_->box, tn_->box + 3, o, winv, tmin, tmax, &tq) ? ti + 1 : tn_->skip;
            if (ti >= tend) break;
            tn_ = &gnodes[ti];
            inst_ = tn_->inst;
          }
          if (inst_ < 0) break;
          ii = inst_;
          ti++;
          const DInstEntry *I = &gents[ii];
          if (kCount) lc->insts++;
          double tn;
          const double tfar = anyhit ? tmax : fmin(tmax, best.t);
          if (!slab(I->tbounds, I->tbounds + 3, o, winv, tmin, tfar, &tn)) continue;
          if (!box_ray_ref_fast(single ? gsb : tn_->box, o, d, winv, plain, tmin, tmax)) continue;
          if (kMotion && I->xform >= 0) {
            double tm[12], tmi[12];
            xform_at(&S.xforms[I->xform], rtime, tm, tmi);
            oo = xpoint(tmi, o);
            od = xvector(tmi, d);
          } else {
            oo = xpoint(I->Minv, o);
            od = xvector(I->Minv, d);
          }
          if (has_negative_zero(od)) continue;
          if (I->pn_prims == 0) continue;
          if (FJ_TINY_PRIMS > 0 && !kMotion && I->pn_prims <= FJ_TINY_PRIMS) {
            bool stop = false;
            for (int k = 0; k < I->pn_prims; k++) {
              double t, u = 0, v = 0;
              if (kCount) lc->prims++;
              V3 v0, v1, v2;
              load_tri(I->tri_verts, I->tri_verts32, (uint32_t) k, &v0, &v1, &v2);
              if (tri_ray(v0, v1, v2, oo, od, &t, &u, &v) && tmin <= t && t <= tmax) {
                const int pid = (int) FJ_G(uint32_t, I->prim_ids)[k];
                if (t < best.t || (t == best.t && best.inst == ii && pid > best.prim)) {
                  best.t = t; best.u = u; best.v = v; best.inst = ii; best.prim = pid;
                  if (anyhit) { stop = true; break; }
                }
              }
            }
            if (stop) break;
            continue;
          }
          const V3 inv = mk(filter_rcp(od.x), filter_rcp(od.y), filter_rcp(od.z));
          nodes = (const DNode *) I->nodes;
          if (!slab(I->pbounds, I->pbounds + 3, oo, inv, tmin, tfar, &tn)) continue;
          if (FJ_CLOSEST_QNODES) s32 = slab32q_setup(oo, inv, I->qorigin, I->qcell);
          else s32 = slab32_setup(oo, inv, I->pbounds);
          root = I->proot;
          found = true;
          break;
        }
        if (found) { cur = root; sp = 0; }
        else { pol.finish(idx, best); have = false; }
      }
#ifdef FJ_PHASE_STATS
      {
        unsigned mx = my_trips, sum = my_trips;
        for (int off = 32; off; off >>= 1) {
          const unsigned other = (unsigned) __shfl_xor((int) mx, off);
          mx = other > mx ? other : mx;
          sum += (unsigned) __shfl_xor((int) sum, off);
        }
        trips_wave += mx;
        trips_lane += sum;
      }
#endif
      FJ_PCYC(0, m_turn);
      continue;
    }

    if (n_inner * tune.leaf_bias8_phased >= n_leaf * 8u) {
      for (uint32_t step = 0;; step++) {
        const bool in_now = step == 0 ? at_inner : (cur != TRAV_DONE && !(cur & FJ_LEAF_FLAG));
        if (step > 0 && (step >= tune.steps_phased || (unsigned) __popcll(__ballot(in_now)) < tune.min_inner_phased)) break;
        if (in_now) {
          if (kCount) lc->nodes++;
          const double tf2 = anyhit ? tmax : fmin(tmax, best.t);
          const float tmin32 = f32_below(tmin), tmax32 = f32_above(tf2);
          float t0, t1, t2, t3;
          bool h0, h1, h2, h3;
          fj_v4u e;
          if (FJ_CLOSEST_QNODES) {
            const FJ_GLOBAL fj_v4u *nq = (const FJ_GLOBAL fj_v4u *) ((const DNodeQ *) nodes + cur);
            const fj_v4u w0 = nq[0], w1 = nq[1], w2 = nq[2];
            e = nq[3];
            const uint32_t shx = slab32_shift(s32.x.i), shy = slab32_shift(s32.y.i), shz = slab32_shift(s32.z.i);
            h0 = slab32q_test(w0.x, w0.y, w0.z, s32, shx, shy, shz, tmin32, tmax32, &t0);
            h1 = slab32q_test(w0.w, w1.x, w1.y, s32, shx, shy, shz, tmin32, tmax32, &t1);
            h2 = slab32q_test(w1.z, w1.w, w2.x, s32, shx, shy, shz, tmin32, tmax32, &t2) && e.z != FJ_NO_CHILD;
            h3 = slab32q_test(w2.y, w2.z, w2.w, s32, shx, shy, shz, tmin32, tmax32, &t3) && e.w != FJ_NO_CHILD;
          } else {
          const FJ_GLOBAL fj_v4f *nd = (const FJ_GLOBAL fj_v4f *) (nodes + cur);
          const fj_v4f q0 = nd[0], q1 = nd[1], q2 = nd[2], q3 = nd[3], q4 = nd[4], q5 = nd[5];
          e = ((const FJ_GLOBAL fj_v4u *) nd)[6];
          h0 = slab32_test(q0.xy, q0.zw, q1.xy, s32, tmin32, tmax32, &t0);
          h1 = slab32_test(q1.zw, q2.xy, q2.zw, s32, tmin32, tmax32, &t1);
          h2 = e.z != FJ_NO_CHILD && slab32_test(q3.xy, q3.zw, q4.xy, s32, tmin32, tmax32, &t2);
          h3 = e.w != FJ_NO_CHILD && slab32_test(q4.zw, q5.xy, q5.zw, s32, tmin32, tmax32, &t3);
          }
          float k0 = h0 ? t0 : INFINITY, k1 = h1 ? t1 : INFINITY;
          float k2 = h2 ? t2 : INFINITY, k3 = h3 ? t3 : INFINITY;
          uint32_t r0 = e.x, r1 = e.y, r2 = e.z, r3 = e.w;
#define FJ_CSWAP(ka, ra, kb, rb) { const bool sw = kb < ka; const float tk = sw ? ka : kb; const uint32_t tr = sw ? ra : rb; ka = sw ? kb : ka; ra = sw ? rb : ra; kb = tk; rb = tr; }
          FJ_CSWAP(k0, r0, k1, r1) FJ_CSWAP(k2, r2, k3, r3) FJ_CSWAP(k0, r0, k2, r2) FJ_CSWAP(k1, r1, k3, r3) FJ_CSWAP(k1, r1, k2, r2)
#undef FJ_CSWAP
          const int nh = (int) h0 + (int) h1 + (int) h2 + (int) h3;
          if (nh == 0) cur = (sp == 0) ? TRAV_DONE : stk.pop(sp);
          else {
            cur = r0;
            if (nh > 3) stk.push(sp, r3);
            if (nh > 2) stk.push(sp, r2);
            if (nh > 1) stk.push(sp, r1);
            if (kCount && (uint32_t) sp > lc->stack_peak) lc->stack_peak = (uint32_t) sp;
          }
        }
        FJ_PCYC(1, __ballot(in_now));
      }
    } else {
      if (at_leaf) {
        const uint32_t first = (cur & 0x7fffffffu) >> 3;
        const uint32_t more = cur & 7u;
        bool stop = false;
        double t, u = 0, v = 0;
        if (kCount) lc->prims++;
        V3 v0, v1, v2;
        const DInstEntry *E = &gents[ii];
        load_tri(E->tri_verts, E->tri_verts32, first, &v0, &v1, &v2);
        if (kMotion && E->tri_vel) {
          const FJ_GLOBAL double *w = FJ_G(double, E->tri_vel) + (size_t) first * 9;
          v0 = v0 + rtime * ld3(w); v1 = v1 + rtime * ld3(w + 3); v2 = v2 + rtime * ld3(w + 6);
        }
        if (tri_ray(v0, v1, v2, oo, od, &t, &u, &v) && tmin <= t && t <= tmax) {
          const int pid = (int) FJ_G(uint32_t, E->prim_ids)[first];
          if (t < best.t || (t == best.t && best.inst == ii && pid > best.prim)) {
            best.t = t; best.u = u; best.v = v; best.inst = ii; best.prim = pid;
            stop = anyhit;
          }
        }
        if (stop) { pol.finish(idx, best); have = false; cur = TRAV_DONE; }
        else if (more) cur = FJ_LEAF_FLAG | ((first + 1u) << 3) | (more - 1u);
        else cur = (sp == 0) ? TRAV_DONE : stk.pop(sp);
      }
      FJ_PCYC(2, __ballot(at_leaf));
    }
  }
}

struct ClosestPolicy {
  const DScene *S;
  const DRay *rays;
  const DPath *paths;
  DHit *hits;
  int default_group;
  __device__ __forceinline__ uint32_t slot(uint32_t i) const { return S->ray_perm ? S->ray_perm[i] : i; }
  __device__ bool fetch(uint32_t k, RayIn *r) const
  {
    const uint32_t i = slot(k);
    const DRay q = rays ? rays[i] : implicit_camera_ray(*S, i);
    r->o = mk(q.o[0], q.o[1], q.o[2]); r->d = mk(q.d[0], q.d[1], q.d[2]);
    if (S->trace_ranges) { r->tmin = S->trace_ranges[2 * (size_t) i]; r->tmax = S->trace_ranges[2 * (size_t) i + 1]; }
    else {
      const uint32_t cx = (rays && paths) ? paths[i].cxt : (uint32_t) CXT_CAMERA_RAY;
      if ((cx & 0x7fu) == CXT_CAMERA_RAY) { r->tmin = S->cam_znear; r->tmax = S->cam_zfar; }
      else { r->tmin = (cx & FJ_CXT_TMIN_1E4) ? .0001 : .001; r->tmax = 1000; }
    }
    r->time = (S->has_motion && paths) ? sample_time(*S, paths[i].flags >> 1) : 0.;
    r->group = paths ? paths[i].group : default_group;
    r->anyhit = false;
    return true;
  }
  __device__ void finish(uint32_t k, const Best &b) const
  {
    DHit h;
    h.t = b.t; h.u = b.u; h.v = b.v; h.inst = b.inst; h.prim = b.prim;
    hits[slot(k)] = h;
  }
  __device__ void finish_miss(uint32_t k) const
  {
    DHit h;
    h.t = DBL_MAX; h.u = h.v = 0; h.inst = -1; h.prim = -1;
    hits[slot(k)] = h;
  }
};

#ifndef FJ_CURVE_MINB
#define FJ_CURVE_MINB 3
#endif
#ifndef FJ_MOTION_MINB
#define FJ_MOTION_MINB 2
#endif
#ifndef FJ_CLOSEST_MINB
#define FJ_CLOSEST_MINB 3
#endif
#ifndef FJ_SHADOW_MINB
#define FJ_SHADOW_MINB 3
#endif
template <bool kCurves, bool kCount, bool kMotion, bool kInstLds = false>
__global__ void __launch_bounds__(BLOCK, kMotion ? FJ_MOTION_MINB : (kCurves ? FJ_CURVE_MINB : FJ_CLOSEST_MINB)) k_trace_closest(DScene S, const DRay *rays, const DPath *paths,
    DHit *hits, uint32_t n, DCounters *cnt, TravTune tune)
{
  if (S.trace_n_dev) { const uint32_t nd_ = *S.trace_n_dev; n = nd_ < n ? nd_ : n; }
  __shared__ uint32_t s_stack[(kCurves ? FJ_STACK_LDS_CURVES : FJ_STACK_LDS) * BLOCK];
  __shared__ double s_rayspace[kCurves ? FJ_RAYSPACE_DOUBLES * BLOCK : 1];
  __shared__ double s_inst[kInstLds ? InstLdsOf<kCurves>::T::WORDS : 1];
  if (kInstLds) InstLdsOf<kCurves>::T::fill(S, s_inst);
  ClosestPolicy pol;
  pol.S = &S; pol.rays = rays; pol.paths = paths; pol.hits = hits; pol.default_group = S.target_group;
  LocalCounters lc = {0, 0, 0, 0};
  traverse_persistent<kCurves, kCount, kMotion, kInstLds, false>(S, pol, tune, n, &cnt->trace_xcd_head[0][0], make_stack(s_stack, S.stack_overflow, kCurves ? s_rayspace : nullptr), &lc, s_inst);
  if (kCount) {
    flush_counters(cnt, lc.nodes, lc.prims, lc.insts, 0, 0);
    flush_stack_peak(&cnt->stack_peak, lc.stack_peak);
    if (blockIdx.x == 0 && threadIdx.x == 0) atomicAdd(&cnt->traced, (unsigned long long) n);
  }
}

#ifndef FJ_PHASED_MINB
#define FJ_PHASED_MINB 4
#endif
template <bool kCount, bool kInstLds>
__global__ void __launch_bounds__(BLOCK, FJ_PHASED_MINB) k_trace_closest_phased(DScene S, const DRay *rays, const DPath *paths,
    DHit *hits, uint32_t n, DCounters *cnt, TravTune tune)
{
  if (S.trace_n_dev) { const uint32_t nd_ = *S.trace_n_dev; n = nd_ < n ? nd_ : n; }
  __shared__ uint32_t s_stack[FJ_STACK_LDS * BLOCK];
  __shared__ double s_inst[kInstLds ? InstLds::WORDS : 1];
  if (kInstLds) InstLds::fill(S, s_inst);
  ClosestPolicy pol;
  pol.S = &S; pol.rays = rays; pol.paths = paths; pol.hits = hits; pol.default_group = S.target_group;
  LocalCounters lc = {0, 0, 0, 0};
  traverse_phased<kCount, false, kInstLds>(S, pol, tune, n, &cnt->trace_xcd_head[0][0], make_stack(s_stack, S.stack_overflow, nullptr, FJ_STACK_LDS), &lc, s_inst);
  if (kCount) {
    flush_counters(cnt, lc.nodes, lc.prims, lc.insts, 0, 0);
    flush_stack_peak(&cnt->stack_peak, lc.stack_peak);
    if (blockIdx.x == 0 && threadIdx.x == 0) atomicAdd(&cnt->traced, (unsigned long long) n);
  }
}

#endif
```

### fujiyama-renderer_amd/csrc/device/fjgpu_frame.hip

```cpp
#include <hip/hip_runtime.h>

#include <algorithm>
#include <cmath>
#include <cstdio>
#include <cstdint>
#include <cstdlib>
#include <cstring>
#include <string>
#include <vector>

#include "fjgpu.h"
#include "fjgpu_api_common.h"
#include "fjgpu_build.h"
#include "fjgpu_kernels.h"
#include "fjgpu_raysort.h"
#include "fjgpu_sample_variance.h"
#include "fjgpu_scene.h"

using fjgpu::fail;
using fjgpu::DeviceBuffers;


void fjgpu::ForgetWorkArena(fjgpu_scene *sc)
{
// ... 220 lines not shown
      query_free(sc);
      set_squeue_max(sc, sc->free_cached);
    }
    bool ok = ensure_work(sc, cap_samples, cap_rays, (int) bt, full_tile_samples) == 0;
    for (int l = P->implicit_cam ? 1 : 0; ok && l <= P->deepest; l++) ok = ensure_level(sc, l, cap_rays) == 0;
    if (ok && sc->ray_sort_bits > 0 && P->deepest >= 1) ok = ensure_sort(sc, cap_rays) == 0;
    if (ok) break;
    (void) hipGetLastError();
    if (bt == 1) return fail(FJGPU_ENOMEM, "device allocation failed for the wavefront work buffers");
    fjgpu::ForgetWorkArena(sc);
    sc->free_cached = 0;
    bt = std::max<long>(1, bt / 2);
    sc->batch_fit_samples = full_tile_samples * (size_t) bt;
  }
  *cap_samples_out = cap_samples; *cap_rays_out = cap_rays;
  return 0;
}


struct LaunchParams {
  DScene S;
  GenParams gp;
  ShadeParams shp;
  ShadowParams swp;
  ResolveParams rp;
  AdaptiveParams ap;
  bool first_touch;
};

void fill_launch_params(const fjgpu_scene *sc, const fj_render_desc *r, const FramePlan &P, size_t cap_rays, LaunchParams *L)
{
  const int *margin = P.margin;
  DScene &S = L->S;
  S = sc->S;
  camera_uv_size(sc->cam_fov, r, S.cam_uv_size);
  S.time_tab = sc->d_tim; S.time_start = r->time_start; S.time_end = r->time_end;
  S.lrec_hair = nullptr;

  L->gp = gen_params(r, margin);
  ShadeParams &shp = L->shp;
  shp.max_diffuse_depth = r->max_diffuse_depth; shp.max_reflect_depth = r->max_reflect_depth; shp.max_refract_depth = r->max_refract_depth;
  shp.count_all_shadow = (int) sc->count_all_shadow;
  shp.ray_capacity = (uint32_t) cap_rays; shp.light_capacity = (uint32_t) cap_rays;
  shp.fc_in = nullptr; shp.fc_out = nullptr;
  shp.next_keys = nullptr; shp.sort_bits = std::max(1, std::min(9, sc->ray_sort_bits)); shp.first_touch = 0;
  L->first_touch = !P.adaptive && sc->shade_first_touch != 0;
  ray_sort_grid(sc->scene_box, shp.sort_bits, shp.sort_lo, shp.sort_scale);
  ShadowParams &swp = L->swp;
  swp.cos_half_pi = std::cos(3.14159265358979323846 / 2.);
  swp.cos_pi = std::cos(3.14159265358979323846);
  swp.pre_resolve = (S.all_opaque && !S.has_curves && !S.has_motion && S.blas_base) ? 1 : 0;
  swp.cast_shadow = r->cast_shadow;
  S.compact_squeue = scene_compact_squeue(S) ? 1 : 0;
  S.pad_cs_ = 0;
  swp.compact = S.compact_squeue;
  swp.light_cones = (sc->light_cones && S.light_cones && S.cone_rows) ? 1 : 0;
  swp.pad_ = 0;
  swp.light_hulls = (swp.light_cones && sc->light_hulls && S.light_hulls && S.hull_rows) ? 1 : 0;
  swp.queue_capacity = (uint32_t) sc->squeue_cap;
  swp.join_capacity = (swp.pre_resolve && sc->split_shadow && sc->d_join) ? (uint32_t) sc->join_cap : 0u;
  S.shadow_join = swp.join_capacity ? sc->d_join : nullptr;
  S.shadow_queue_cap = (uint32_t) sc->squeue_cap;
  ResolveParams &rp = L->rp;
  rp.xres = r->xres; rp.yres = r->yres; rp.rate_x = r->rate_x; rp.rate_y = r->rate_y;
  rp.npx_x = r->rate_x + 2 * margin[0]; rp.npx_y = r->rate_y + 2 * margin[1];
  AdaptiveParams &ap = L->ap;
  std::memset(&ap, 0, sizeof(ap));
  if (P.adaptive) {
    ap.D = r->adaptive_max_subdivision; ap.div = P.a_div;
    ap.margin_x = margin[0]; ap.margin_y = margin[1];
    ap.udelta = 1. / (P.a_div * r->xres);
    ap.vdelta = 1. / (P.a_div * r->yres);
    ap.jitter = r->jitter;
    ap.jittered = r->jitter > 0 ? 1 : 0;
    ap.threshold = (double) r->adaptive_subdivision_threshold;
    ap.ray_capacity = (uint32_t) cap_rays;
    rp.rate_x = rp.rate_y = P.a_div;
    rp.npx_x = P.a_div * (1 + 2 * margin[0]) + 1; rp.npx_y = P.a_div * (1 + 2 * margin[1]) + 1;
  }
  rp.fw = (double) r->filter_w; rp.fh = (double) r->filter_h;
}

struct LaunchTimer {
  struct Span { size_t a, b; double *bucket; };
  fjgpu_scene *sc;
  std::vector<Span> spans;
  size_t ev_used = 0;

  explicit LaunchTimer(fjgpu_scene *scene) : sc(scene) {}
  size_t take_event()
  {
    if (ev_used == sc->ev_pool.size()) { hipEvent_t e = nullptr; if (hipEventCreate(&e) != hipSuccess) return (size_t) -1; sc->ev_pool.push_back(e); }
    return ev_used++;
  }
  template <class Launch> int timed(hipStream_t stream, double *bucket, Launch &&launch)
  {
    const size_t a = take_event(), b = take_event();
    if (a == (size_t) -1 || b == (size_t) -1) return -1;
    (void) hipEventRecord(sc->ev_pool[a], stream);
    const int le = launch();
    (void) hipEventRecord(sc->ev_pool[b], stream);
    if (le) return le;
    spans.push_back(Span{a, b, bucket});
    return 0;
  }
  void drop_last() { spans.pop_back(); }
  void resolve()
// ... 255 lines not shown
  {
    begin_shadow_queue();
    AdaptiveParams ap = L.ap;
    ap.cells0 = B.cells0;
    (void) hipMemsetAsync(sc->d_apstate, 0, (size_t) B.n_samples, st);
    (void) hipMemsetAsync(sc->d_acells, 0, (size_t) B.cells0 * (((((size_t) 1) << (2 * (ap.D + 1))) - 1) / 3), st);
    int rc = T.timed(st, &acc.gen_ms, [&]() { return launch_adaptive_uv(st, ap, sc->d_tiles, nb, B.max_ts, sc->d_jit, sc->d_suv); });
    for (int level = 0; level <= ap.D && rc == 0; level++) {
      ap.level = level;
      (void) hipMemsetAsync(&sc->d_cnt->cam_count, 0, sizeof(uint32_t), st);
      const uint32_t max_pts = (uint32_t) ((B.max_w0 << level) + 1) * (uint32_t) ((B.max_h0 << level) + 1);
      rc = T.timed(st, &acc.gen_ms, [&]() {
        return launch_adaptive_points(st, L.S, ap, sc->d_tiles, nb, max_pts, sc->d_acells, sc->d_suv, sc->d_accum, sc->d_apstate,
            sc->d_aseen, sc->levels[0].rays, sc->levels[0].paths, sc->d_cnt);
      });
      if (rc) return rc;
      DCounters hc;
      if (hipMemcpyAsync(&hc, sc->d_cnt, sizeof(hc), hipMemcpyDeviceToHost, st) != hipSuccess || hipStreamSynchronize(st) != hipSuccess) return -1;
      if (hc.overflow) return fail(FJGPU_ENOMEM, "camera ray queue overflow in the adaptive sampler");
      acc.rays.camera += hc.cam_count;
      if (hc.cam_count) {
        rc = process(0, hc.cam_count);
        if (rc) return rc;
        rc = finish_shadow();
        if (rc) return rc;
      }
      rc = T.timed(st, &acc.resolve_ms, [&]() {
        return launch_adaptive_decide(st, ap, sc->d_tiles, nb, (uint32_t) (B.max_w0 << level) * (uint32_t) (B.max_h0 << level),
            sc->d_acells, sc->d_accum, sc->d_apstate, sc->d_aseen);
      });
    }
    if (rc) return rc;
    return T.timed(st, &acc.resolve_ms, [&]() {
      return launch_adaptive_fill(st, ap, sc->d_tiles, nb, B.max_ts, sc->d_acells, sc->d_accum, sc->d_apstate, sc->d_aseen, sc->d_afinal);
    });
  }
};

void fold_counters(const DCounters &hc, fjgpu_stats *acc, fjgpu_scene *sc)
{
  acc->rays.shadow += hc.rays[CXT_SHADOW_RAY];
  acc->rays.diffuse += hc.rays[CXT_DIFFUSE_RAY];
  acc->rays.reflect += hc.rays[CXT_REFLECT_RAY];
  acc->rays.refract += hc.rays[CXT_REFRACT_RAY];
  acc->nodes_visited += hc.nodes;
  acc->prims_tested += hc.prims;
  acc->insts_tested += hc.insts;
  acc->rays_traced += hc.traced;
  acc->shadow_traversed += hc.squeued;
  acc->shadow_nodes += hc.sh_nodes; acc->shadow_prims += hc.sh_prims; acc->shadow_insts += hc.sh_insts;
  sc->stack_peak_closest = std::max(sc->stack_peak_closest, hc.stack_peak);
  sc->stack_peak_shadow = std::max(sc->stack_peak_shadow, hc.sh_stack_peak);
  sc->hull_verdicts += hc.hull_settled;
  acc->batches++;
}

int render_tiles_once(fjgpu_scene *sc, const fj_render_desc *r, const int32_t *tile_ids, int n_tiles,
    float *d_fb, void *hip_stream, fjgpu_stats *stats, const SampleVarianceOut *sv)
{
  if (const int e = check_request(r)) return e;
  HIP_TRY(hipSetDevice(sc->device));
  hipStream_t st = static_cast<hipStream_t>(hip_stream);
  sc->stack_peak_closest = sc->stack_peak_shadow = 0;
  sc->hull_verdicts = 0;
  sc->accum_memsets = 0;

  FramePlan P;
  if (const int e = plan_tiles(sc, r, tile_ids, n_tiles, &P)) return e;
  if (!sc->work || sc->free_cached == 0) query_free(sc);
  if (sc->levels.size() < (size_t) P.deepest + 1) sc->levels.resize((size_t) P.deepest + 1, fjgpu_scene::Level{nullptr, nullptr, 0, nullptr});
  P.bt = plan_batch_tiles(sc, P, sc->free_cached);

  choose_streams(sc, P);
  size_t cap_samples = 0, cap_rays = 0;
  if (const int e = reserve_arena(sc, &P, &cap_samples, &cap_rays)) return e;
  const size_t a_cells0_cap = P.adaptive ? (size_t) P.bt * (size_t) (r->tile_w + 2 * P.margin[0]) * (size_t) (r->tile_h + 2 * P.margin[1]) : 0;
  const size_t a_cell_bytes = a_cells0_cap * (((((size_t) 1) << (2 * (r->adaptive_max_subdivision + 1))) - 1) / 3);
  if (P.adaptive && a_cells0_cap >= ((size_t) 1 << 32)) return fail(FJGPU_EINVAL, "too many lattice cells per batch: lower the batch_tiles option");
  if (P.adaptive && ensure_adaptive(sc, cap_samples, a_cell_bytes))
    return fail(FJGPU_ENOMEM, "device allocation failed for the adaptive sampler's buffers");

  LaunchParams L;
  fill_launch_params(sc, r, P, cap_rays, &L);

  fjgpu_stats acc;
  std::memset(&acc, 0, sizeof(acc));
  LaunchTimer T(sc);
  BatchRun run(sc, P, L, T, acc, cap_rays, st);
  int rc = 0;
  hipEvent_t *ev_all = sc->ev_frame;
  if (!ev_all[0]) { HIP_TRY(hipEventCreate(&ev_all[0])); HIP_TRY(hipEventCreate(&ev_all[1])); }
  (void) hipEventRecord(ev_all[0], st);
  for (size_t b0 = 0; b0 < P.ids.size() && rc == 0; b0 += (size_t) P.bt) {
    const int nb = (int) std::min<size_t>((size_t) P.bt, P.ids.size() - b0);
    BatchLayout B;
    layout_batch(sc, r, P, b0, nb, &B);
    if ((hipMemcpyAsync(sc->d_tiles, B.td.data(), sizeof(TileDesc) * nb, hipMemcpyHostToDevice, st)) != hipSuccess) { rc = -1; break; }
    if (!L.first_touch) { (void) hipMemsetAsync(sc->d_accum, 0, sizeof(float) * 4 * (size_t) B.n_samples, st); sc->accum_memsets++; }
    (void) hipMemsetAsync(sc->d_cnt, 0, sizeof(DCounters), st);
    rc = P.adaptive ? run.run_adaptive(B, nb) : run.run_fixed(B, nb);
    if (rc) break;
    rc = T.timed(st, &acc.resolve_ms, [&]() {
      return launch_resolve(st, L.rp, sc->d_tiles, nb, B.max_px, sc->d_suv, sc->d_accum, P.adaptive ? sc->d_afinal : nullptr, d_fb);
    });
    if (rc) break;
    if (sv) {
      rc = T.timed(st, &acc.resolve_ms, [&]() {
        return launch_sample_variance(st, L.rp, sc->d_tiles, nb, B.max_px, sc->d_suv, sc->d_accum, sv->albedo, sv->albedo_floor, sv->variance);
      });
      if (rc) break;
    }
    DCounters hc;
    if (hipMemcpyAsync(&hc, sc->d_cnt, sizeof(hc), hipMemcpyDeviceToHost, st) != hipSuccess || hipStreamSynchronize(st) != hipSuccess) { rc = -1; break; }
    if (hc.overflow) { sc->split_overflowed = L.S.shadow_join != nullptr; rc = fail(FJGPU_ENOMEM, "wavefront queue overflow: lower the batch_tiles option"); break; }
    fold_counters(hc, &acc, sc);
    if (sc->batch_fn) {
      const std::vector<int32_t> bids(P.ids.begin() + (long) b0, P.ids.begin() + (long) b0 + nb);
// ... 69 lines not shown
```

### fujiyama-renderer_amd/csrc/device/fjgpu_kernels.h

```cpp
#ifndef FJGPU_KERNELS_H
#define FJGPU_KERNELS_H

#include <hip/hip_runtime.h>
#include "fjgpu_types.h"

struct TileDesc {
  int32_t xmin, ymin, xmax, ymax;
  int32_t nx, ny;
  uint32_t sample_offset;
  int32_t id;
  uint32_t cell_offset;
  int32_t pad;
};

struct GenParams {
  int32_t rate_x, rate_y, margin_x, margin_y;
  double udelta, vdelta, jitter;
  int32_t jittered, pad;
};

struct AovParams {
  int32_t xres, rate_x, rate_y, margin_x, margin_y, pad;
  float *depth, *position, *normal, *uv;
  int32_t *ids;
// ... 11 lines not shown
  int32_t margin_x, margin_y;
  double udelta, vdelta, jitter, threshold;
  int32_t jittered, level;
  uint32_t cells0;
  uint32_t ray_capacity;
};

struct ShadeParams {
  int32_t max_diffuse_depth, max_reflect_depth, max_refract_depth;
  int32_t count_all_shadow;
  uint32_t ray_capacity, light_capacity;
  uint32_t *next_keys;
  const float *fc_in;
  float *fc_out;
  double sort_lo[3], sort_scale[3];
  int32_t sort_bits;
  int32_t first_touch;
};

struct ShadowParams {
  double cos_half_pi, cos_pi;
  uint32_t pre_resolve;
  uint32_t queue_capacity;
  uint32_t join_capacity;
  int32_t cast_shadow;
  int32_t compact;
  int32_t light_cones;
  int32_t light_hulls;
  int32_t pad_;
};

struct ResolveParams {
  int32_t xres, yres, rate_x, rate_y, npx_x, npx_y;
  double fw, fh;
};

int launch_gen_camera(hipStream_t st, const DScene &S, const GenParams &gp, const TileDesc *d_tiles, int n_tiles,
    uint32_t max_tile_samples, const double *jit, const double *tim, double *s_uv, DRay *rays, DPath *paths, uint32_t *s_tk = nullptr);
int launch_trace_closest(hipStream_t st, const DScene &S, const DRay *rays, const DPath *paths, DHit *hits,
    uint32_t n, DCounters *cnt, int count_events);
int launch_shade(hipStream_t st, const DScene &S, const ShadeParams &sp, const DRay *rays, const DPath *paths,
    const DHit *hits, uint32_t n, float *s_accum, DRay *next_rays, DPath *next_paths, DLightRec *lrecs, DCounters *cnt);
uint32_t shadow_queue_padding();
void shadow_queue_reset(hipStream_t st, DCounters *cnt);
int launch_shadow_cull(hipStream_t st, const DScene &S, const ShadowParams &sp, const DLightRec *lrecs, uint32_t b, uint32_t e,
    float *s_accum, DShadowRay *squeue, DCounters *cnt, int count_events, int blocks_per_cu = 0);
int launch_shadow_trace(hipStream_t st, const DScene &S, const DShadowRay *squeue, float *s_accum, DCounters *cnt, int count_events);
int launch_quantize_nodes(hipStream_t st, const DNode *nodes, uint32_t n, const double *origin, const double *cell, DNodeQ *out);
int launch_slab32_batch(hipStream_t st, uint32_t n, const double *rays, const double *grid, const uint32_t *words, void *out);
int launch_move_tiles(hipStream_t st, bool unpack, float *fb, int xres, const int32_t *d_rects, int n_tiles, int tile_px, float *slab);
void set_anyhit_filter_off(long v);
void light_cone_validate_counts(double *verdicts, double *contradictions);
void light_hull_validate_counts(double *verdicts, double *contradictions);
void tri_filter_validate_counts(double out[5]);
bool kernels_build_config(const char *name, double *value);
void debug_phase_stats();
size_t persistent_threads();

int launch_resolve(hipStream_t st, const ResolveParams &rp, const TileDesc *d_tiles, int n_tiles, int max_tile_pixels,
    const double *s_uv, const float *s_accum, const double *s_data64, float *fb);

int launch_aov_reduce(hipStream_t st, const DScene &S, const AovParams &ap, const TileDesc *d_tiles, int n_tiles, int max_tile_pixels,
    const DRay *rays, const DHit *hits);

int launch_aov_albedo(hipStream_t st, const DScene &S, const AlbedoParams &ap, const TileDesc *d_tiles, int n_tiles, int max_tile_pixels,
    const DHit *hits);

int launch_adaptive_uv(hipStream_t st, const AdaptiveParams &ap, const TileDesc *d_tiles, int n_tiles, uint32_t max_tile_samples,
    const double *jit, double *s_uv);
int launch_adaptive_points(hipStream_t st, const DScene &S, const AdaptiveParams &ap, const TileDesc *d_tiles, int n_tiles,
    uint32_t max_tile_points, const uint8_t *cells, const double *s_uv, const float *s_accum, uint8_t *pstate, double *seen,
    DRay *rays, DPath *paths, DCounters *cnt);
int launch_adaptive_decide(hipStream_t st, const AdaptiveParams &ap, const TileDesc *d_tiles, int n_tiles, uint32_t max_tile_cells,
    uint8_t *cells, const float *s_accum, const uint8_t *pstate, const double *seen);
int launch_adaptive_fill(hipStream_t st, const AdaptiveParams &ap, const TileDesc *d_tiles, int n_tiles, uint32_t max_tile_samples,
    const uint8_t *cells, const float *s_accum, const uint8_t *pstate, const double *seen, double *final_data);

#endif
```

### fujiyama-renderer_amd/csrc/device/fjgpu_kernels.hip

```cpp
#include <hip/hip_runtime.h>
#include <float.h>
#include <math.h>
#include <stdint.h>
#include <stdlib.h>
#include <stdio.h>
#include <string.h>

#include "fjgpu_types.h"
#include "fjgpu_kernels.h"
#include "fjgpu_xform_math.h"

#define BLOCK 256

#include "fjgpu_dev_math.h"
#include "fjgpu_tri_filter.h"
#include "fjgpu_light_cone.h"
#include "fjgpu_dev_curve.h"
#include "fjgpu_dev_traverse.h"
#include "fjgpu_dev_flat.h"
#include "fjgpu_dev_shade.h"
#include "fjgpu_dev_shadow.h"
#include "fjgpu_dev_anyhit.h"
#include "fjgpu_dev_anyhit_curves.h"
#include "fjgpu_dev_adaptive.h"
#include "fjgpu_dev_aov.h"
#include "fjgpu_dev_albedo.h"

template <typename TData4>
__global__ void __launch_bounds__(BLOCK) k_resolve(ResolveParams rp, const TileDesc *tiles,
    const double *s_uv, const TData4 *s_data, float *fb)
{
  const TileDesc T = tiles[blockIdx.y];
  const int tw = T.xmax - T.xmin, th = T.ymax - T.ymin;
  const int k = blockIdx.x * (BLOCK / 64) + (threadIdx.x >> 6);
  if (k >= tw * th) return;
  const unsigned lane = __lane_id();
  const int px = T.xmin + k % tw, py = T.ymin + k / tw;
  const size_t base = (size_t) T.sample_offset + (size_t) (py - T.ymin) * rp.rate_y * T.nx + (size_t) (px - T.xmin) * rp.rate_x;
  const int nwin = rp.npx_x * rp.npx_y;
  double acc0 = 0, acc1 = 0, acc2 = 0, acc3 = 0, wsum = 0;
  for (int w = (int) lane; w < nwin; w += 64) {
    const int sy = w / rp.npx_x, sx = w - sy * rp.npx_x;
    const size_t s = base + (size_t) sy * T.nx + sx;
    const double2 uv = reinterpret_cast<const double2 *>(s_uv)[s];
    const TData4 d = s_data[s];
    const double filtx = rp.xres * uv.x - (px + .5);
    const double filty = rp.yres * (1 - uv.y) - (py + .5);
    const double xx = 2 * filtx / rp.fw;
    const double yy = 2 * filty / rp.fh;
    const double wgt = exp(-2 * (xx * xx + yy * yy));
    acc0 += wgt * (double) d.x;
    acc1 += wgt * (double) d.y;
    acc2 += wgt * (double) d.z;
    acc3 += wgt * (double) d.w;
    wsum += wgt;
  }
  for (int off = 32; off > 0; off >>= 1) {
    acc0 += __shfl_xor(acc0, off);
    acc1 += __shfl_xor(acc1, off);
    acc2 += __shfl_xor(acc2, off);
    acc3 += __shfl_xor(acc3, off);
    wsum += __shfl_xor(wsum, off);
  }
  if (lane == 0) {
    const float inv_sum = 1.f / (float) wsum;
    float4 out;
    out.x = (float) acc0 * inv_sum; out.y = (float) acc1 * inv_sum; out.z = (float) acc2 * inv_sum; out.w = (float) acc3 * inv_sum;
    reinterpret_cast<float4 *>(fb)[(size_t) py * rp.xres + px] = out;
  }
// ... 298 lines not shown
  LAUNCH_CHECK();
  TL_DUMP(st, "shadow", persistent_grid(1ull << 30, PERSIST_BLOCKS_PER_CU_MAX));
  return 0;
}

int launch_quantize_nodes(hipStream_t st, const DNode *nodes, uint32_t n, const double *origin, const double *cell, DNodeQ *out)
{
  if (n == 0) return 0;
  hipLaunchKernelGGL(k_quantize_nodes, dim3((n + BLOCK - 1) / BLOCK), dim3(BLOCK), 0, st, nodes, n, origin[0], origin[1], origin[2],
      cell[0], cell[1], cell[2], out);
  LAUNCH_CHECK();
  return 0;
}

int launch_slab32_batch(hipStream_t st, uint32_t n, const double *rays, const double *grid, const uint32_t *words, void *out)
{
  if (n == 0) return 0;
  hipLaunchKernelGGL(k_slab32_batch, dim3((n + BLOCK - 1) / BLOCK), dim3(BLOCK), 0, st, n, rays, grid, words, (Slab32Probe *) out);
  LAUNCH_CHECK();
  return 0;
}

int launch_move_tiles(hipStream_t st, bool unpack, float *fb, int xres, const int32_t *d_rects, int n_tiles, int tile_px, float *slab)
{
  for (int t0 = 0; t0 < n_tiles; t0 += 65535) {
    const int nt = n_tiles - t0 < 65535 ? n_tiles - t0 : 65535;
    const dim3 grid((tile_px + BLOCK - 1) / BLOCK, nt);
    float4 *sl = (float4 *) slab + (size_t) t0 * tile_px;
    if (unpack) hipLaunchKernelGGL(k_move_tiles<true>, grid, dim3(BLOCK), 0, st, (float4 *) fb, xres, (const int4 *) d_rects + t0, tile_px, sl);
    else hipLaunchKernelGGL(k_move_tiles<false>, grid, dim3(BLOCK), 0, st, (float4 *) fb, xres, (const int4 *) d_rects + t0, tile_px, sl);
    LAUNCH_CHECK();
  }
  return 0;
}

void light_cone_validate_counts(double *verdicts, double *contradictions)
{
  *verdicts = -1; *contradictions = -1;
#ifdef FJ_LIGHT_CONE_VALIDATE
  unsigned long long c[2];
  if (hipMemcpyFromSymbol(c, HIP_SYMBOL(g_lightcone), sizeof(c)) == hipSuccess) { *verdicts = (double) c[0]; *contradictions = (double) c[1]; }
#endif
}

void light_hull_validate_counts(double *verdicts, double *contradictions)
{
  *verdicts = -1; *contradictions = -1;
#ifdef FJ_LIGHT_HULL_VALIDATE
  unsigned long long c[2];
  if (hipMemcpyFromSymbol(c, HIP_SYMBOL(g_lighthull), sizeof(c)) == hipSuccess) { *verdicts = (double) c[0]; *contradictions = (double) c[1]; }
#endif
}

void tri_filter_validate_counts(double out[5])
{
  for (int k = 0; k < 5; k++) out[k] = -1;
#ifdef FJ_TRI_FILTER_VALIDATE
  unsigned long long c[8];
  if (hipMemcpyFromSymbol(c, HIP_SYMBOL(g_trifilter), sizeof(c)) == hipSuccess) { out[0] = (double) c[0]; out[1] = (double) c[1]; out[2] = (double) c[2]; out[3] = (double) c[4]; out[4] = (double) c[3]; }
#endif
}

bool kernels_build_config(const char *name, double *value)
{
  static const struct { const char *name; double value; } table[] = {
    {"stack_lds", FJ_STACK_LDS}, {"stack_lds_curves", FJ_STACK_LDS_CURVES}, {"stack_lds_anyhit", FJ_STACK_LDS_ANYHIT},
    {"stack_lds_canyhit", FJ_STACK_LDS_CANYHIT}, {"stack_lds_min", FJ_STACK_LDS_MIN},
    {"slab_perm", FJ_SLAB_PERM},
#ifdef FJ_TRI_FILTER_VALIDATE
    {"tri_filter_validate", 1},
#else
    {"tri_filter_validate", 0},
#endif
#ifdef FJ_LIGHT_CONE_VALIDATE
    {"light_cone_validate", 1},
#else
    {"light_cone_validate", 0},
#endif
#ifdef FJ_LIGHT_HULL_VALIDATE
    {"light_hull_validate", 1},
#else
    {"light_hull_validate", 0},
#endif
  };
  for (const auto &t : table) if (!strcmp(name, t.name)) { *value = t.value; return true; }
  return false;
}

void debug_phase_stats()
{
#ifdef FJ_TRI_FILTER_VALIDATE
  {
    unsigned long long c[8];
    if (hipMemcpyFromSymbol(c, HIP_SYMBOL(g_trifilter), sizeof(c)) == hipSuccess && (c[0] | c[1] | c[2])) {
      fprintf(stderr, "fjgpu tri filter: miss %llu hit %llu maybe %llu | exact hits %llu | CONTRADICTIONS %llu\n", c[0], c[1], c[2], c[4], c[3]);
      unsigned long long z[8] = {0};
      (void) hipMemcpyToSymbol(HIP_SYMBOL(g_trifilter), z, sizeof(z));
    }
  }
#endif
#ifdef FJ_PHASE_STATS
  {
    unsigned long long c[8];
    if (hipMemcpyFromSymbol(c, HIP_SYMBOL(g_curve_stat), sizeof(c)) == hipSuccess && c[2]) {
      fprintf(stderr, "fjgpu phase curves: second-stage execs %llu lanes %llu tests-hit %llu leaf-walks %llu nodes %llu\n", c[2], c[3], c[4], c[0], c[1]);
      unsigned long long z[8] = {0};
      (void) hipMemcpyToSymbol(HIP_SYMBOL(g_curve_stat), z, sizeof(z));
    }
  }
  {
    unsigned long long c[16];
    if (hipMemcpyFromSymbol(c, HIP_SYMBOL(g_cphase), sizeof(c)) == hipSuccess && c[12]) {
      static const char *pn[4] = {"turnover", "inner", "leaf", "ribbon"};
      const double all = (double) (c[0] + c[1] + c[2] + c[3]);
      fprintf(stderr, "fjgpu phase curve-anyhit: %llu iterations", c[12]);
      for (int k = 0; k < 4; k++) fprintf(stderr, " | %s %.1f %% of ticks, %llu execs, %.1f lanes, %.0f ticks each", pn[k], 100. * c[k] / all, c[4 + k], (double) c[8 + k] / (c[4 + k] ? c[4 + k] : 1), (double) c[k] / (c[4 + k] ? c[4 + k] : 1));
      fprintf(stderr, "\n");
      unsigned long long z[16] = {0};
      (void) hipMemcpyToSymbol(HIP_SYMBOL(g_cphase), z, sizeof(z));
    }
  }
  unsigned long long h[16];
  if (hipMemcpyFromSymbol(h, HIP_SYMBOL(g_phase), sizeof(h)) != hipSuccess) return;
  static const char *names[16] = {"iters", "entry_execs|entry_ticks", "entry_lanes", "inner_execs|inner_ticks", "inner_lanes", "leaf_execs|leaf_ticks", "leaf_lanes",
      "tri_execs|stage2_ticks", "tri_lanes", "", "hits", "refills", "tail_iters_max", "tail_iters_sum", "walk_iters_sum", "walk_waves"};
  for (int i = 0; i < 16; i++) if (names[i][0]) fprintf(stderr, "fjgpu phase %-24s %llu\n", names[i], h[i]);
  {
    unsigned long long a[16];
    if (hipMemcpyFromSymbol(a, HIP_SYMBOL(g_ahphase), sizeof(a)) == hipSuccess && a[3] && a[5]) {
      fprintf(stderr, "fjgpu phase anyhit-lanes: %llu iterations | inner steps %llu with %.1f lanes at inner nodes, %.1f idle, %.1f held at a leaf | leaf steps %llu with %.1f lanes, %.1f idle, "
          "%.1f at inner nodes | turnovers %llu with %.1f lanes | %llu rays occluded\n", a[0], a[3], (double) a[4] / a[3], (double) a[7] / a[3], (double) a[8] / a[3], a[5], (double) a[6] / a[5],
          (double) a[9] / a[5], (double) a[11] / a[5], a[1], (double) a[2] / (a[1] ? a[1] : 1), a[10]);
      if (a[12]) fprintf(stderr, "fjgpu phase anyhit-exact: %llu exact phases with %.1f lanes, %llu of them hits\n", a[12], (double) a[13] / a[12], a[14]);
      unsigned long long z[16] = {0};
      (void) hipMemcpyToSymbol(HIP_SYMBOL(g_ahphase), z, sizeof(z));
// ... 83 lines not shown
```

### fujiyama-renderer_amd/csrc/device/fjgpu_scene.h

```cpp
#ifndef FJGPU_SCENE_H
#define FJGPU_SCENE_H

#include <hip/hip_runtime.h>

#include <algorithm>
#include <cstdint>
#include <cstdlib>
#include <memory>
#include <vector>

#include "fjgpu.h"
#include "fjgpu_api_common.h"
#include "fjgpu_build.h"
#include "fjgpu_kernels.h"

#define FJ_LREC_BUFS 4

struct fjgpu_scene {
  int device;
  DScene S;
  fjgpu::DeviceBuffers mem;
  double cam_fov;
  fj_camera_desc camera;
  int n_light_samples;
  long batch_tiles;
  long batch_samples = 0;
  long aov_batch_samples = 0;
  long render_calls = 0;
  long count_events;
  long light_cones = 1;
  int cone_rows = 0, cone_records = 0;
  long light_hulls = 1;
  int hull_rows = 0, hull_records = 0;
  unsigned long long hull_verdicts = 0;
  long count_all_shadow;
  long shade_first_touch = 1;
  unsigned long long accum_memsets = 0;
  unsigned long long stack_peak_closest = 0, stack_peak_shadow = 0;
  std::unique_ptr<fjgpu::DeviceBuffers> work;
  size_t work_samples, work_rays;
  double *d_suv;
  uint32_t *d_stk = nullptr;
  float *d_accum;
  double *d_aseen = nullptr, *d_afinal = nullptr;
  uint8_t *d_apstate = nullptr, *d_acells = nullptr;
  const void *a_owner = nullptr;
  size_t a_samples = 0, a_cell_bytes = 0;
  struct Level { DRay *rays; DPath *paths; size_t cap; uint32_t *keys; float *fc; };
  bool has_filter_rays = false;
  std::vector<Level> levels;
  bool uses_sample_uid;
  int max_children;
  bool bounce_diffuse, bounce_reflect, bounce_refract;
  DHit *d_hits;
  DLightRec *d_lrecs[FJ_LREC_BUFS];
  DLightHair *d_lhair[FJ_LREC_BUFS];
  int lrec_bufs = 2;
  long overlap;
  bool overlap_now = false;
  size_t free_cached = 0;
  hipEvent_t ev_frame[2] = {nullptr, nullptr};
  long early_shadow = 0;
  hipStream_t shadow_stream;
  hipStream_t read_stream = nullptr;
  hipEvent_t ev_shaded = nullptr;
  hipEvent_t ev_shadow_done[FJ_LREC_BUFS];
  std::vector<hipEvent_t> ev_pool;
  DShadowRay *d_squeue;
  size_t squeue_rec_bytes = 0;
  size_t squeue_cap;
  uint32_t *d_join = nullptr; size_t join_cap = 0;
  bool split_overflowed = false;
  uint32_t split_kfac = 1;
  bool split_shadow = false;
  DCounters *d_cnt;
  TileDesc *d_tiles;
  double *d_jit, *d_tim;
  size_t tab_len;
  long sampler_seed = 0;
  long tab_seed = 0;
  int tiles_cap;
  int stack_need;
  double tri_record_bytes;
  size_t blas_nodes;
  long blas_treelet_passes = 0;
  unsigned long long blas_treelets_changed = 0;
  double blas_sah_cost_initial = 0., blas_sah_cost = 0.;
// ... 93 lines not shown
```

### fujiyama-renderer_amd/csrc/device/fjgpu_types.h

```cpp
#ifndef FJGPU_TYPES_H
#define FJGPU_TYPES_H

#include <stdint.h>
#include "fj_scene_desc.h"

struct DNode {
  float box[4][6];
  uint32_t child[4];
  uint32_t pad[4];
};
static_assert(sizeof(DNode) == 128, "DNode must be 128 bytes");

struct DNodeQ {
  uint16_t q[4][6];
  uint32_t child[4];
};
static_assert(sizeof(DNodeQ) == 64, "DNodeQ must be 64 bytes");

#ifndef FJ_CURVE_QNODES
#define FJ_CURVE_QNODES 1
#endif
#ifndef FJ_CLOSEST_QNODES
#define FJ_CLOSEST_QNODES 1
#endif
// ... 29 lines not shown
  const double *velocity;
  const uint32_t *prim_ids;
  const double *P;
  const double *N;
  const double *vN;
  const float *uv;
  const int32_t *indices;
  const int32_t *face_group;
  const double *curve_cp;
  const double *curve_width;
  const float *curve_Cd;
  const int8_t *curve_depth;
  const float *curve_capsule;
  const double *curve_vel;
  double bounds[6];
  double grid_cell[3];
  int32_t grid_n[3];
  int32_t pad2;
  uint32_t root;
  int32_t type;
  int32_t n_prims;
  int32_t pad;
};

struct DInstance {
  double M[12];
  double Minv[12];
  double wbounds[6];
  int32_t primset;
  int32_t n_shaders;
  int32_t shaders[FJ_MAX_SHADING_GROUPS];
  int32_t reflect_target, refract_target, shadow_target;
  int32_t xform;
  int32_t pn_prims;
  uint32_t proot;
  double pbounds[6];
  const DNode *pnodes;
  const DNodeQ *pqnodes;
  double qorigin[3], qcell[3];
  const int32_t *sh_indices;
  const double *sh_N;
  const float *sh_uv;
  const int32_t *sh_face_group;
  const double *sh_vN;
  int32_t sh_type;
  int32_t sh_pad;
};

struct DInstEntry {
  double Minv[12];
  double tbounds[6];
  double pbounds[6];
  double qorigin[3], qcell[3];
  const void *nodes;
  const double *tri_verts;
  const float *tri_verts32;
  const double *tri_vel;
  const uint32_t *prim_ids;
  int32_t ptype;
  int32_t pad;
  uint32_t proot;
  int32_t pn_prims;
  int32_t primset;
  int32_t xform;
};
#define FJ_INST_LDS_ENTRY_WORDS 38
#define FJ_INST_LDS_NODES 39
#define FJ_INST_LDS_INSTS 16
#define FJ_INST_LDS_GROUPS 12
#define FJ_INST_LDS_NODES_BIG 79
#define FJ_INST_LDS_INSTS_BIG 33
#define FJ_INST_LDS_GROUPS_BIG 24
#define FJ_INST_LDS_NODES_CURVES 15
#define FJ_INST_LDS_INSTS_CURVES 6
#define FJ_INST_LDS_GROUPS_CURVES 12
#define FJ_FLAT_LDS_INSTS 80
#define FJ_INST_LDS_BYTES (FJ_INST_LDS_NODES * 56 + FJ_INST_LDS_INSTS * 8 * FJ_INST_LDS_ENTRY_WORDS + FJ_INST_LDS_GROUPS * 64)

struct DAnyInst {
  double Minv[12];
  double bounds[6];
  double qorigin[3], qcell[3];
  uint32_t node_base;
  uint32_t tri_base;
  uint32_t root;
  uint32_t tris_f32;
  int32_t n_prims;
  float fbound;
  uint32_t pad[2];
};
static_assert(sizeof(DAnyInst) == 224, "DAnyInst layout");

#define FJ_TLAS_FLAT 4
struct DTNode {
  double box[6];
  int32_t inst;
  int32_t skip;
};

struct DGroup {
  int32_t first, count;
  int32_t all_opaque;
  int32_t n_instances;
  double sbounds[6];
};

struct DFlatRef { float v[9]; uint32_t inst_ord; uint32_t pid; uint32_t pad; };
static_assert(sizeof(DFlatRef) == 48, "DFlatRef must be 48 bytes");
struct DFlat {
  const DNodeQ *nodes;
  const DFlatRef *refs;
  const double *refbox;
  double qorigin[3], qcell[3];
  uint32_t root;
  int32_t n_inst, n_prims, pad;
};

struct DTexture {
  const float *tiles;
  int32_t width, height, nchannels, tilesize;
};

struct DLightSample {
  double P[3];
  float Cl[3];
  int32_t light;
  int32_t type;
  int32_t ordinal;
};

struct DAreaLight {
  double M[12];
  double N[3];
  float color[3];
  float sample_intensity;
  int32_t double_sided;
  int32_t pad;
};

struct DLightHair;
struct DLightCone;

struct DScene {
  const DPrimSet *primsets;
  const DInstance *instances;
  const DGroup *groups;
  const DTNode *group_nodes;
  const DInstEntry *inst_entries;
  int32_t n_group_nodes;
  int32_t inst_lds;
  const fj_shader_desc *shaders;
  const DTexture *textures;
  const DLightSample *light_samples;
  const DLightCone *light_cones;
  const int32_t *cone_rows;
  const DLightCone *light_hulls;
  const int32_t *hull_rows;
  DLightHair *lrec_hair;
  uint32_t shadow_queue_cap;
  uint32_t cam_slot0;
  uint32_t *shadow_join;
  const DFlat *flats;
  const DAreaLight *area_lights;
  const DAnyInst *any_insts;
  const char *blas_base;
  int32_t n_light_samples;
  int32_t n_instances, n_groups, n_primsets;
  uint32_t *stack_overflow;
  uint32_t *stack_overflow_shadow;
  int32_t all_opaque;
  int32_t has_area;
  int32_t has_hair;
  int32_t has_curves;
  int32_t target_group;
  int32_t curve_anyhit;
  int32_t incoherent_rays;
  const double *cam_uv;
  int32_t compact_squeue;
  int32_t pad_cs_;
  const uint32_t *cam_tk;
  const uint32_t *ray_perm;
  const double *trace_ranges;
  const uint32_t *trace_n_dev;
  const fj_xform_desc *xforms;
  const fj_xform_desc *cam_xform;
  const double *time_tab;
  double time_start, time_end;
  int32_t has_motion;
  int32_t multi_shadow_groups;
  double cam_M[12];
  double cam_uv_size[2];
  double cam_znear, cam_zfar;
};

struct DRay {
  double o[3], d[3];
};
static_assert(sizeof(DRay) == 48, "DRay must be 48 bytes");
#define FJ_CXT_TMIN_1E4 0x80u

enum { CXT_CAMERA_RAY = 0, CXT_SHADOW_RAY, CXT_DIFFUSE_RAY, CXT_REFLECT_RAY, CXT_REFRACT_RAY };

struct DPath {
  uint32_t sample;
  float T[3];
  uint8_t cxt, ddepth, rdepth, tdepth;
  int32_t group;
  uint32_t flags;
  uint32_t rng;
  uint32_t uid;
};
static_assert(sizeof(DPath) == 36, "DPath must be 36 bytes");

struct DHit {
  double t, u, v;
  int32_t inst, prim;
};

struct DLightRec {
  double P[3];
  double N[3];
  float W[3];
  uint32_t sample;
  int32_t group;
  int32_t kind;
  uint32_t uid;
  uint32_t key;
};

struct DLightHair {
  double aux[6];
  float Cd[3];
  uint32_t pad;
};

struct DShadowRay {
  double o[3], d[3], tmax;
  float c[3];
  uint32_t sample;
  int32_t group;
  uint32_t tindex;
};

struct DShadowRayC {
  double o[3];
  float c[3];
  uint32_t sample;
  int32_t group;
  uint32_t tindex;
  uint32_t light;
  uint32_t pad;
};
static_assert(sizeof(DShadowRayC) == 56, "DShadowRayC must be 56 bytes");

struct DCounters {
  unsigned long long rays[5];
  unsigned long long nodes, prims, insts, traced, squeued;
  unsigned long long sh_nodes, sh_prims, sh_insts;
  unsigned long long stack_peak, sh_stack_peak;
  unsigned long long hull_settled;
  uint32_t next_count;
  uint32_t light_count;
  uint32_t overflow;
  uint32_t cam_count;
  uint32_t pad1_[28];
  uint32_t shadow_count;
  uint32_t shadow_head;
  uint32_t pad2_[30];
  uint32_t trace_head;
  uint32_t cull_head;
  uint32_t pad3_[30];
  uint32_t shadow_xcd_head[8][32];
  uint32_t trace_xcd_head[8][32];
  uint32_t join_count;
  uint32_t pad4_[31];
};

#endif
```

### fujiyama-renderer_amd/gpu.py

```python
import ctypes as C

import numpy as np

from . import ffi

_lib = None


class GpuError(RuntimeError):
    pass


def lib():
    global _lib
    if _lib is None:
        L = ffi.load("libfjgpu.so")
        L.fjgpu_last_error.restype = C.c_char_p
        L.fjgpu_device_count.restype = C.c_int
        L.fjgpu_scene_create.argtypes = [C.c_void_p, C.c_int, C.POINTER(C.c_void_p)]
        L.fjgpu_scene_destroy.argtypes = [C.c_void_p]
        L.fjgpu_scene_destroy.restype = None
        L.fjgpu_tile_count.argtypes = [C.POINTER(ffi.RenderDesc)]
        L.fjgpu_tile_rect.argtypes = [C.POINTER(ffi.RenderDesc), C.c_int, C.POINTER(C.c_int32)]
        L.fjgpu_render_tiles.argtypes = [C.c_void_p, C.POINTER(ffi.RenderDesc), C.c_void_p, C.c_int,
# ... 370 lines not shown
            if self._h[k]:
                lib().fjgpu_scene_destroy(self._h[k])
                self._h[k] = None

    def __del__(self):
        try:
            self.close()
        except Exception:
            pass

    def render_frame(self, render, tile_ids=None):
        fb = np.zeros((render.yres, render.xres, 4), dtype=np.float32)
        st = (ffi.GpuStats * self.n)()
        if tile_ids is None:
            ids_p, n = None, 0
        else:
            ids = np.ascontiguousarray(tile_ids, dtype=np.int32)
            ids_p, n = ids.ctypes.data_as(C.c_void_p), len(ids)
        _check(lib().fjgpu_render_frame_multi(self._h, self.n, C.byref(render), ids_p, n, fb.ctypes.data_as(C.c_void_p), st))
        return fb, list(st)


def host_instance_level(scene_desc_ptr, group):
    L = lib()
    L.fjgpu_host_instance_level.argtypes = [C.c_void_p, C.c_int, C.c_void_p, C.c_void_p, C.c_void_p, C.c_int]
    L.fjgpu_host_instance_level.restype = C.c_int
    n = L.fjgpu_host_instance_level(scene_desc_ptr, group, None, None, None, 0)
    if n < 0:
        _check(n)
    inst = np.zeros(n, dtype=np.int32)
    skip = np.zeros(n, dtype=np.int32)
    box = np.zeros((n, 6), dtype=np.float64)
    _check(min(0, L.fjgpu_host_instance_level(scene_desc_ptr, group, inst.ctypes.data_as(C.c_void_p), skip.ctypes.data_as(C.c_void_p),
                                              box.ctypes.data_as(C.c_void_p), n)))
    return inst, skip, box


LIGHT_HULL = np.dtype([("n", np.float64, (6, 3)), ("reach", np.float64), ("count", np.int32), ("pad", np.int32)])


def host_light_hulls(scene_desc_ptr, group):
    L = lib()
    L.fjgpu_host_light_hulls.argtypes = [C.c_void_p, C.c_int, C.c_void_p, C.c_void_p, C.c_int, C.c_void_p]
    L.fjgpu_host_light_hulls.restype = C.c_int
    n = L.fjgpu_host_light_hulls(scene_desc_ptr, group, None, None, 0, None)
    if n < 0:
        _check(n)
    rec = np.zeros(n, dtype=LIGHT_HULL)
    Pl = np.zeros((n, 3), dtype=np.float64)
    M = np.zeros((3, 4), dtype=np.float64)
    _check(min(0, L.fjgpu_host_light_hulls(scene_desc_ptr, group, rec.ctypes.data_as(C.c_void_p), Pl.ctypes.data_as(C.c_void_p), n,
                                           M.ctypes.data_as(C.c_void_p))))
    return rec, Pl, M


def host_curve_blas(scene_desc_ptr, curve_set):
    L = lib()
    L.fjgpu_host_curve_blas.argtypes = [C.c_void_p, C.c_int, C.c_void_p, C.c_void_p, C.c_void_p, C.c_void_p, C.c_int, C.c_void_p, C.c_void_p,
                                        C.c_void_p]
    L.fjgpu_host_curve_blas.restype = C.c_int
    n = L.fjgpu_host_curve_blas(scene_desc_ptr, curve_set, None, None, None, None, 0, None, None, None)
    if n < 0:
        _check(n)
    curve = np.zeros(n, dtype=np.int32)
    cap = np.zeros((n, 7), dtype=np.float32)
    depth = np.zeros(n, dtype=np.int32)
    box = np.zeros((n, 6), dtype=np.float32)
    grid_n = np.zeros(3, dtype=np.int32)
    grid_cell = np.zeros(3, dtype=np.float64)
    bounds = np.zeros(6, dtype=np.float64)
    p = lambda a: a.ctypes.data_as(C.c_void_p)
    _check(min(0, L.fjgpu_host_curve_blas(scene_desc_ptr, curve_set, p(curve), p(cap), p(depth), p(box), n, p(grid_n), p(grid_cell), p(bounds))))
    return dict(curve=curve, A=cap[:, 0:3].copy(), B=cap[:, 3:6].copy(), reach=cap[:, 6].copy(), depth=depth, box=box, grid_n=grid_n,
                grid_cell=grid_cell, bounds=bounds)


DENOISE_ITERATIONS = 5
SIGMA_COLOR = 3.0
SIGMA_NORMAL = 1.0
SIGMA_POSITION_FRACTION = 0.1
ALBEDO_FLOOR = 1e-4


def _device_tensor(a, name, dtype, channels, dev, shape=None):
    import torch
    if a is None:
        return None
    t = a if torch.is_tensor(a) else torch.from_numpy(np.ascontiguousarray(a))
    t = t.to(device=dev, dtype=dtype).contiguous()
    if t.dim() != 3 or t.shape[2] != channels or (shape is not None and tuple(t.shape[:2]) != tuple(shape)):
        raise ValueError("%s must be [H, W, %d]%s, not %s" % (name, channels, "" if shape is None else " with H, W = %d, %d" % tuple(shape),
                                                             tuple(t.shape)))
    return t


def denoise(color, normal=None, position=None, ids=None, iterations=DENOISE_ITERATIONS, sigma_color=SIGMA_COLOR,
            sigma_normal=SIGMA_NORMAL, sigma_position=None, stop_at_ids=True, region=None, device=0, stream=None, out=None,
            albedo=None, albedo_floor=ALBEDO_FLOOR):
    import torch
    dev = torch.device("cuda", device)
    c = _device_tensor(color, "color", torch.float32, 4, dev)
    hw = tuple(c.shape[:2])
    n = _device_tensor(normal, "normal", torch.float32, 3, dev, hw)
    p = _device_tensor(position, "position", torch.float32, 3, dev, hw)
    i = _device_tensor(ids, "ids", torch.int32, 4, dev, hw)
    a = _device_tensor(albedo, "albedo", torch.float32, 3, dev, hw)
# ... 497 lines not shown
```

### include/fjgpu.h

```cpp
#ifndef FJGPU_H
#define FJGPU_H

#include <stdint.h>
#include "fj_scene_desc.h"

#ifdef __cplusplus
extern "C" {
#endif

enum {
  FJGPU_OK = 0,
  FJGPU_ENODEV = -1,
  FJGPU_EINVAL = -2,
  FJGPU_EUNSUPPORTED = -3,
  FJGPU_ENOMEM = -4
};

typedef struct fjgpu_scene fjgpu_scene;

typedef struct fjgpu_stats {
  fj_ray_counts rays;
  uint64_t nodes_visited;
  uint64_t prims_tested;
  uint64_t insts_tested;
// ... 140 lines not shown
  float   alpha_min;
  float   max_history;
  float   tol_position;
  float   cos_normal;
  float   min_history_variance;
  float   albedo_floor;
} fjgpu_temporal_desc;

int fjgpu_denoise_temporal(int device, const fjgpu_temporal_desc *desc,
     const float *color, const float *position, const float *normal, const int32_t *ids,
                         const float *albedo , const float *variance_spatial ,
     const fjgpu_view *prev_view, const float *prev_position, const float *prev_normal, const int32_t *prev_ids,
                         const fjgpu_temporal_history *prev ,
     const fjgpu_temporal_history *next, float *variance_out ,
    void *hip_stream, fjgpu_stats *stats);

typedef struct fjgpu_temporal_clamp {
  int32_t radius;
  float   gamma;
  int32_t stop_at_ids;
  int32_t _pad;
  float  *amount;
} fjgpu_temporal_clamp;

int fjgpu_denoise_temporal_clamped(int device, const fjgpu_temporal_desc *desc, const fjgpu_temporal_clamp *clamp ,
     const float *color, const float *position, const float *normal, const int32_t *ids,
                         const float *albedo , const float *variance_spatial ,
     const fjgpu_view *prev_view, const float *prev_position, const float *prev_normal, const int32_t *prev_ids,
                         const fjgpu_temporal_history *prev ,
     const fjgpu_temporal_history *next, float *variance_out ,
    void *hip_stream, fjgpu_stats *stats);

typedef struct fjgpu_accum_state {
  float *mean;
  float *m2;
  float *count;
} fjgpu_accum_state;

int fjgpu_accumulate(int device, int xres, int yres, const int32_t *rects ,
    int n_rects, const float *color , const fjgpu_accum_state *state, int reset, float *variance_out ,
    void *hip_stream, fjgpu_stats *stats);

int fjgpu_accumulate_tile_error(int device, int xres, int yres, const int32_t *rects, int n_rects,
    const fjgpu_accum_state *state, float lum_floor, float *errors_out , void *hip_stream, fjgpu_stats *stats);

int fjgpu_set_option(fjgpu_scene *scene, const char *name, long value);

int fjgpu_global_option(const char *name, long value);

int fjgpu_host_instance_level(const fj_scene_desc *desc, int group, int32_t *out_inst, int32_t *out_skip, double *out_box, int cap);

int fjgpu_host_light_hulls(const fj_scene_desc *desc, int group, void *out_records, double *out_Pl, int cap, double *out_M);

int fjgpu_host_curve_blas(const fj_scene_desc *desc, int curve_set, int32_t *out_curve, float *out_capsule, int32_t *out_depth,
                          float *out_box, int cap, int32_t *out_grid_n, double *out_grid_cell, double *out_bounds);

int fjgpu_scene_query(const fjgpu_scene *scene, const char *name, double *value);

int fjgpu_build_config(const char *name, double *value);

void fjgpu_host_make_transform(int transform_order, int rotate_order, const double *trs9, double *M16, double *Minv16);
void fjgpu_host_xorshift_f01(int n, double *out);
void fjgpu_host_xorshift_f01_seeded(unsigned seed, int n, double *out);
int32_t fjgpu_host_seeded_tile_id(unsigned seed, int32_t tile_id);
void fjgpu_host_sampler_margin(const fj_render_desc *render, int32_t *margin2);
double fjgpu_host_camera_uv_size_y(double fov);

int fjgpu_dev_rccl_selftest(int device, int n_floats);

int fjgpu_dev_sort_pairs(int device, const uint32_t *keys, int n, int key_bits, uint32_t *keys_out, uint32_t *perm, int repeats, double *sort_ms);

int fjgpu_dev_slab32_batch(int device, int n, const double *rays, const double *grid, const uint32_t *words, void *out);

int fjgpu_dev_quantize_nodes(int device, int n, const void *nodes, const double *origin, const double *cell, void *out);

const char *fjgpu_last_error(void);

#ifdef __cplusplus
}
#endif
#endif
```

Measured before the change: 41620 Mray/s.

## Add per-instance empty-interior hole boxes to skip instance traversal

At scene build, the host computes for each static mesh instance an axis-aligned box inside its bounds that contains no triangles, verified against all faces. The box is stored as six floats in each instance entry. During traversal, a ray segment that lies entirely inside that box skips the instance's BLAS. The hole is only kept when another instance's centre lies inside it. The change enlarges the LDS instance entry, which reduces the number of LDS-cached nodes, and adds a per-instance test to the traversal loop.

```diff
diff --git a/fujiyama-renderer_amd/csrc/device/fjgpu_api.hip b/fujiyama-renderer_amd/csrc/device/fjgpu_api.hip
--- a/fujiyama-renderer_amd/csrc/device/fjgpu_api.hip
+++ b/fujiyama-renderer_amd/csrc/device/fjgpu_api.hip
@@ -25,6 +25,7 @@
 #include "fjgpu_lbvh.h"
 #include "fjgpu_light_cone.h"
 #include "fjgpu_light_hull.h"
+#include "fjgpu_inst_hole.h"
 #include "fjgpu_matte.h"
 #include "fjgpu_raysort.h"
 #include "fjgpu_scene.h"
@@ -307,6 +308,76 @@
   return 0;
 }
 
+}
+
+static void inst_tight_bounds(const DInstance &I, const double *pbounds, int n_prims, double *tb)
+{
+  for (int a = 0; a < 3; a++) { tb[a] = -INFINITY; tb[3 + a] = INFINITY; }
+  if (I.xform >= 0 || n_prims <= 0) return;
+  double mn[3] = {INFINITY, INFINITY, INFINITY}, mx[3] = {-INFINITY, -INFINITY, -INFINITY};
+  for (int c = 0; c < 8; c++) {
+    const double p[3] = {pbounds[(c & 1) ? 3 : 0], pbounds[(c & 2) ? 4 : 1], pbounds[(c & 4) ? 5 : 2]};
+    for (int a = 0; a < 3; a++) {
+      const double w = I.M[4 * a] * p[0] + I.M[4 * a + 1] * p[1] + I.M[4 * a + 2] * p[2] + I.M[4 * a + 3];
+      mn[a] = std::min(mn[a], w); mx[a] = std::max(mx[a], w);
+    }
+  }
+  bool finite = true;
+  for (int a = 0; a < 3; a++) finite = finite && std::isfinite(mn[a]) && std::isfinite(mx[a]);
+  if (!finite) return;
+  for (int a = 0; a < 3; a++) {
+    const double pad = 1e-7 * (mx[a] - mn[a]) + 1e-7 * std::max(std::fabs(mn[a]), std::fabs(mx[a])) + 1e-9;
+    tb[a] = mn[a] - pad; tb[3 + a] = mx[a] + pad;
+  }
+}
+
+static int build_inst_holes(const fjgpu::HostScene &hs, std::vector<float> *holes)
+{
+  holes->assign(hs.instances.size() * 6, 0.f);
+  size_t workers = std::min(16u, std::max(1u, std::thread::hardware_concurrency()));
+  if (const char *omp = getenv("OMP_NUM_THREADS")) { const long v = atol(omp); if (v >= 1) workers = std::min<size_t>(workers, (size_t) v); }
+  auto run = [&](int64_t nch, const std::function<void(int64_t)> &fn) {
+    const size_t nt = (size_t) std::max<int64_t>(1, std::min<int64_t>((int64_t) workers, nch));
+    if (nt == 1) { for (int64_t c = 0; c < nch; c++) fn(c); return; }
+    std::atomic<int64_t> next(0);
+    std::vector<std::thread> th;
+    for (size_t t = 0; t < nt; t++) th.emplace_back([&]() { for (int64_t c; (c = next.fetch_add(1)) < nch;) fn(c); });
+    for (auto &t : th) t.join();
+  };
+  std::vector<double> tbs(hs.instances.size() * 6);
+  for (size_t k = 0; k < hs.instances.size(); k++) {
+    const fjgpu::HostPrimSet &ps = hs.primsets[hs.instances[k].primset];
+    inst_tight_bounds(hs.instances[k], ps.bounds, ps.n_prims, &tbs[6 * k]);
+  }
+  int records = 0;
+  for (size_t k = 0; k < hs.instances.size(); k++) {
+    const DInstance &I = hs.instances[k];
+    float *h = holes->data() + 6 * k;
+    inst_hole_none(h);
+    const fjgpu::HostPrimSet &ps = hs.primsets[I.primset];
+    if (I.xform >= 0 || ps.type != FJ_PRIMSET_MESH || !ps.mesh || ps.mesh->velocity || ps.n_prims <= 0 || ps.mesh->n_faces <= 0) continue;
+    auto serves = [&](const float *b) {
+      for (size_t j = 0; j < hs.instances.size(); j++) {
+        const double *t = &tbs[6 * j];
+        if (j == k || !std::isfinite(t[0] + t[1] + t[2] + t[3] + t[4] + t[5])) continue;
+        bool in = true;
+        for (int a = 0; a < 3; a++) { const double c = .5 * (t[a] + t[3 + a]); in = in && c > (double) b[a] && c < (double) b[3 + a]; }
+        if (in) return true;
+      }
+      return false;
+    };
+    const int64_t nf = ps.mesh->n_faces;
+    if (nf > 65536) {
+      std::vector<int32_t> sub;
+      for (int64_t f = 0; f < nf; f += 64) for (int c = 0; c < 3; c++) sub.push_back(ps.mesh->indices[3 * f + c]);
+      float hs_[6];
+      if (!inst_hole_build(I.M, I.Minv, ps.mesh->P, ps.mesh->n_points, sub.data(), (int64_t) (sub.size() / 3), &tbs[6 * k], hs_, nullptr, run) || !serves(hs_)) continue;
+    }
+    if (!inst_hole_build(I.M, I.Minv, ps.mesh->P, ps.mesh->n_points, ps.mesh->indices, nf, &tbs[6 * k], h, nullptr, run)) continue;
+    if (!serves(h)) { inst_hole_none(h); continue; }
+    records++;
+  }
+  return records;
 }
 
 static void build_light_hull_rows(const fjgpu::HostScene &hs, const std::vector<double> &cone_reach, std::vector<DLightCone> &hulls,
@@ -547,6 +618,9 @@
       }
       e |= M.upload(di.data(), di.size(), &S.instances);
       std::vector<DInstEntry> ie(di.size());
+      std::vector<float> holes;
+      sc->hole_records = build_inst_holes(hs, &holes);
+      lap("instance holes");
       bool any_curves = false, any_motion = !hs.xforms.empty();
       for (const auto &ps : hs.primsets) {
         if (ps.type == FJ_PRIMSET_CURVE && ps.n_prims > 0) any_curves = true;
@@ -557,24 +631,8 @@
         DInstEntry &E = ie[k];
         std::memcpy(E.Minv, I.Minv, sizeof(E.Minv));
         std::memcpy(E.pbounds, I.pbounds, sizeof(E.pbounds));
-        for (int a = 0; a < 3; a++) { E.tbounds[a] = -INFINITY; E.tbounds[3 + a] = INFINITY; }
-        if (I.xform < 0 && I.pn_prims > 0) {
-          double mn[3] = {INFINITY, INFINITY, INFINITY}, mx[3] = {-INFINITY, -INFINITY, -INFINITY};
-          for (int c = 0; c < 8; c++) {
-            const double p[3] = {I.pbounds[(c & 1) ? 3 : 0], I.pbounds[(c & 2) ? 4 : 1], I.pbounds[(c & 4) ? 5 : 2]};
-            for (int a = 0; a < 3; a++) {
-              const double w = I.M[4 * a] * p[0] + I.M[4 * a + 1] * p[1] + I.M[4 * a + 2] * p[2] + I.M[4 * a + 3];
-              mn[a] = std::min(mn[a], w); mx[a] = std::max(mx[a], w);
-            }
-          }
-          bool finite = true;
-          for (int a = 0; a < 3; a++) finite = finite && std::isfinite(mn[a]) && std::isfinite(mx[a]);
-          if (finite)
-            for (int a = 0; a < 3; a++) {
-              const double pad = 1e-7 * (mx[a] - mn[a]) + 1e-7 * std::max(std::fabs(mn[a]), std::fabs(mx[a])) + 1e-9;
-              E.tbounds[a] = mn[a] - pad; E.tbounds[3 + a] = mx[a] + pad;
-            }
-        }
+        inst_tight_bounds(I, I.pbounds, I.pn_prims, E.tbounds);
+        std::memcpy(E.hole, &holes[6 * k], sizeof(E.hole));
         for (int a = 0; a < 3; a++) { E.qorigin[a] = I.qorigin[a]; E.qcell[a] = I.qcell[a]; }
         const DPrimSet &P = dps[I.primset];
         const bool quantised = FJ_CLOSEST_QNODES && (!any_curves || FJ_CURVE_QNODES) && !any_motion;
@@ -654,6 +712,7 @@
   }
   static_assert(sizeof(DInstEntry) == 8 * FJ_INST_LDS_ENTRY_WORDS && sizeof(DTNode) == 56 && sizeof(DGroup) == 64, "LDS copy of the instance level");
   S.curve_anyhit = (g_curve_anyhit && !getenv("FJGPU_NO_CURVE_ANYHIT")) ? 1 : 0;
+  S.inst_holes = 1;
   S.inst_lds = (g_inst_lds && !getenv("FJGPU_NO_INST_LDS")) ? 1 : 0;
   e |= M.upload(hs.shaders.data(), hs.shaders.size(), &S.shaders);
   e |= M.upload(hs.xforms.data(), hs.xforms.size(), &S.xforms);
@@ -947,6 +1006,24 @@
   return (int) nl;
 }
 
+int fjgpu_host_inst_holes(const fj_scene_desc *desc, float *out_holes, double *out_M, double *out_tbounds, int cap)
+{
+  if (!desc) return fail(FJGPU_EINVAL, "bad instance-hole query");
+  fjgpu::HostScene hs;
+  std::string err;
+  const int e = fjgpu::BuildHostScene(desc, &hs, &err, true);
+  if (e) return fail(e, err);
+  std::vector<float> holes;
+  build_inst_holes(hs, &holes);
+  for (size_t k = 0; k < hs.instances.size() && (int) k < cap; k++) {
+    const DInstance &I = hs.instances[k];
+    if (out_holes) std::memcpy(out_holes + 6 * k, &holes[6 * k], 6 * sizeof(float));
+    if (out_M) std::memcpy(out_M + 12 * k, I.M, 12 * sizeof(double));
+    if (out_tbounds) inst_tight_bounds(I, hs.primsets[I.primset].bounds, hs.primsets[I.primset].n_prims, out_tbounds + 6 * k);
+  }
+  return (int) hs.instances.size();
+}
+
 int fjgpu_host_curve_blas(const fj_scene_desc *desc, int curve_set, int32_t *out_curve, float *out_capsule, int32_t *out_depth,
                           float *out_box, int cap, int32_t *out_grid_n, double *out_grid_cell, double *out_bounds)
 {
@@ -1058,6 +1135,15 @@
     else *value = c;
     return 0;
   }
+  if (n == "inst_hole_records") { *value = scene->hole_records; return 0; }
+  if (n == "inst_hole_skips") { *value = (double) scene->hole_skips; return 0; }
+  if (n == "inst_hole_verdicts" || n == "inst_hole_contradictions") {
+    double v = -1, c = -1;
+    if (hipSetDevice(scene->device) != hipSuccess || hipDeviceSynchronize() != hipSuccess) return fail(FJGPU_ENODEV, "hipSetDevice / hipDeviceSynchronize");
+    inst_hole_validate_counts(&v, &c);
+    *value = n == "inst_hole_verdicts" ? v : c;
+    return 0;
+  }
   {
     static const char *const tf[5] = {"tri_filter_miss", "tri_filter_hit", "tri_filter_maybe", "tri_filter_exact_hits", "tri_filter_contradictions"};
     for (int k = 0; k < 5; k++)
@@ -1192,6 +1278,7 @@
   if (n == "count_all_shadow") { scene->count_all_shadow = value != 0; return 0; }
   if (n == "light_cones") { scene->light_cones = value != 0; return 0; }
   if (n == "light_hulls") { scene->light_hulls = value != 0; return 0; }
+  if (n == "inst_holes") { scene->inst_holes = value != 0; scene->S.inst_holes = value != 0 ? 1 : 0; return 0; }
   if (n == "shade_first_touch") {
     if (value != 0 && value != 1) return fail(FJGPU_EINVAL, "shade_first_touch: 0 (memset and atomic adds at the camera level) or 1 (one store per sample)");
     scene->shade_first_touch = value;
@@ -1411,6 +1498,7 @@
   if (stats || sc->count_events) {
     HIP_TRY(hipMemcpy(&hc, d_cnt, sizeof(hc), hipMemcpyDeviceToHost));
     sc->stack_peak_closest = hc.stack_peak;
+    sc->hole_skips = hc.hole_skips;
   }
   if (stats) {
     std::memset(stats, 0, sizeof(*stats));
diff --git a/fujiyama-renderer_amd/csrc/device/fjgpu_dev_math.h b/fujiyama-renderer_amd/csrc/device/fjgpu_dev_math.h
--- a/fujiyama-renderer_amd/csrc/device/fjgpu_dev_math.h
+++ b/fujiyama-renderer_amd/csrc/device/fjgpu_dev_math.h
@@ -176,7 +176,7 @@
 
 struct Best { double t, u, v; int inst, prim; };
 
-struct LocalCounters { uint32_t nodes, prims, insts, stack_peak; };
+struct LocalCounters { uint32_t nodes, prims, insts, stack_peak, hole_skips; };
 
 __device__ __forceinline__ unsigned long long wave_sum(unsigned long long v)
 {
@@ -208,6 +208,12 @@
   if (__lane_id() == 0 && v) atomicMax(peak, (unsigned long long) v);
 }
 
+__device__ __forceinline__ void flush_hole_skips(DCounters *cnt, unsigned long long skips)
+{
+  skips = wave_sum(skips);
+  if (__lane_id() == 0 && skips) atomicAdd(&cnt->hole_skips, skips);
+}
+
 __device__ __forceinline__ void flush_shadow_walk_counters(DCounters *cnt, unsigned long long nodes, unsigned long long prims,
     unsigned long long insts)
 {
diff --git a/fujiyama-renderer_amd/csrc/device/fjgpu_dev_shadow.h b/fujiyama-renderer_amd/csrc/device/fjgpu_dev_shadow.h
--- a/fujiyama-renderer_amd/csrc/device/fjgpu_dev_shadow.h
+++ b/fujiyama-renderer_amd/csrc/device/fjgpu_dev_shadow.h
@@ -498,6 +498,7 @@
   traverse_persistent<kCurves, kCount, kMotion, kInstLds, kAnyOnly>(S, pol, tune, n, &cnt->shadow_xcd_head[0][0], make_stack(s_stack, S.stack_overflow_shadow, kCurves ? s_rayspace : nullptr), &lc, s_inst);
   if (kCount) {
     flush_counters(cnt, lc.nodes, lc.prims, lc.insts, 0, 0);
+    flush_hole_skips(cnt, lc.hole_skips);
     flush_stack_peak(&cnt->sh_stack_peak, lc.stack_peak);
     flush_shadow_walk_counters(cnt, lc.nodes, lc.prims, lc.insts);
     if (blockIdx.x == 0 && threadIdx.x == 0) atomicAdd(&cnt->squeued, (unsigned long long) n);
diff --git a/fujiyama-renderer_amd/csrc/device/fjgpu_dev_traverse.h b/fujiyama-renderer_amd/csrc/device/fjgpu_dev_traverse.h
--- a/fujiyama-renderer_amd/csrc/device/fjgpu_dev_traverse.h
+++ b/fujiyama-renderer_amd/csrc/device/fjgpu_dev_traverse.h
@@ -7,6 +7,9 @@
 #endif
 #ifdef FJ_PHASE_STATS
 __device__ unsigned long long g_phase[16];
+#endif
+#ifdef FJ_INST_HOLE_VALIDATE
+__device__ unsigned long long g_insthole[2];
 #endif
 #ifdef FJ_WAVE_TIMELINE
 #define FJ_TL_WAVES 8192
@@ -164,6 +167,16 @@
 typedef InstLdsT<FJ_INST_LDS_NODES_CURVES, FJ_INST_LDS_INSTS_CURVES, FJ_INST_LDS_GROUPS_CURVES> InstLdsCurves;
 template <bool kCurves> struct InstLdsOf { typedef InstLdsBig T; };
 template <> struct InstLdsOf<true> { typedef InstLdsCurves T; };
+
+#ifdef FJ_INST_HOLE_VALIDATE
+#define FJ_HOLE_RESET() hole_v = false
+#define FJ_HOLE_SKIP() { hole_v = true; atomicAdd(&g_insthole[0], 1ull); }
+#define FJ_HOLE_HIT(closer) do { if (hole_v && (closer)) atomicAdd(&g_insthole[1], 1ull); } while (0)
+#else
+#define FJ_HOLE_RESET() do { } while (0)
+#define FJ_HOLE_SKIP() { if (kCount) lc->hole_skips++; continue; }
+#define FJ_HOLE_HIT(closer) do { } while (0)
+#endif
 
 template <bool kCurves, bool kCount, bool kMotion, bool kInstLds, bool kAnyOnly, class Policy>
 __device__ void traverse_persistent(const DScene &S, Policy &pol, TravTune tune, uint32_t n, uint32_t *head, TravStack stk, LocalCounters *lc, const double *s_inst)
@@ -199,6 +212,9 @@
   uint32_t last_curve = 0xffffffffu;
   uint32_t pend = 0xffffffffu;
   int sp = 0;
+#ifdef FJ_INST_HOLE_VALIDATE
+  bool hole_v = false;
+#endif
 #ifdef FJ_PHASE_STATS
   unsigned long long it_all = 0, it_tail = 0;
   unsigned long long cyc[4] = {0, 0, 0, 0}, c_prev = __builtin_readcyclecounter();
@@ -283,6 +299,8 @@
         if (kCount) lc->insts++;
         double tn;
         const double tfar = anyhit ? tmax : fmin(tmax, best.t);
+        FJ_HOLE_RESET();
+        if (!kCurves && S.inst_holes && I->hole[0] < I->hole[3] && inst_hole_verdict(I->hole, o.x, o.y, o.z, d.x, d.y, d.z, tmin, tfar)) FJ_HOLE_SKIP()
         if (!slab(I->tbounds, I->tbounds + 3, o, winv, tmin, tfar, &tn)) continue;
         if (!box_ray_ref_fast(single ? gsb : tn_->box, o, d, winv, plain, tmin, tmax)) continue;
         if (kMotion && I->xform >= 0) {
@@ -386,6 +404,7 @@
           }
           if (!tri_ray(v0, v1, v2, oo, od, &t, &u, &v)) continue;
           if (!(tmin <= t && t <= tmax)) continue;
+          FJ_HOLE_HIT(anyhit || t <= best.t);
           if (kAnyOnly) { stop = true; break; }
           const int pid = (int) FJ_G(uint32_t, P->prim_ids)[first + k];
           if (t < best.t || (t == best.t && best.inst == ii && pid > best.prim)) {
@@ -468,6 +487,9 @@
   const DNode *nodes = nullptr;
   uint32_t cur = TRAV_DONE;
   int sp = 0;
+#ifdef FJ_INST_HOLE_VALIDATE
+  bool hole_v = false;
+#endif
 #ifdef FJ_PHASE_STATS
   unsigned long long pcyc[3] = {0, 0, 0}, pex[3] = {0, 0, 0}, pln[3] = {0, 0, 0}, trips_lane = 0, trips_wave = 0, pc_prev = __builtin_readcyclecounter();
 #define FJ_PCYC(k, mask) do { const unsigned long long c_now = __builtin_readcyclecounter(); pcyc[k] += c_now - pc_prev; pc_prev = c_now; pex[k]++; pln[k] += __popcll(mask); } while (0)
@@ -544,6 +566,8 @@
           if (kCount) lc->insts++;
           double tn;
           const double tfar = anyhit ? tmax : fmin(tmax, best.t);
+          FJ_HOLE_RESET();
+          if (!kMotion && S.inst_holes && I->hole[0] < I->hole[3] && inst_hole_verdict(I->hole, o.x, o.y, o.z, d.x, d.y, d.z, tmin, tfar)) FJ_HOLE_SKIP()
           if (!slab(I->tbounds, I->tbounds + 3, o, winv, tmin, tfar, &tn)) continue;
           if (!box_ray_ref_fast(single ? gsb : tn_->box, o, d, winv, plain, tmin, tmax)) continue;
           if (kMotion && I->xform >= 0) {
@@ -565,6 +589,7 @@
               V3 v0, v1, v2;
               load_tri(I->tri_verts, I->tri_verts32, (uint32_t) k, &v0, &v1, &v2);
               if (tri_ray(v0, v1, v2, oo, od, &t, &u, &v) && tmin <= t && t <= tmax) {
+                FJ_HOLE_HIT(anyhit || t <= best.t);
                 const int pid = (int) FJ_G(uint32_t, I->prim_ids)[k];
                 if (t < best.t || (t == best.t && best.inst == ii && pid > best.prim)) {
                   best.t = t; best.u = u; best.v = v; best.inst = ii; best.prim = pid;
@@ -665,6 +690,7 @@
           v0 = v0 + rtime * ld3(w); v1 = v1 + rtime * ld3(w + 3); v2 = v2 + rtime * ld3(w + 6);
         }
         if (tri_ray(v0, v1, v2, oo, od, &t, &u, &v) && tmin <= t && t <= tmax) {
+          FJ_HOLE_HIT(anyhit || t <= best.t);
           const int pid = (int) FJ_G(uint32_t, E->prim_ids)[first];
           if (t < best.t || (t == best.t && best.inst == ii && pid > best.prim)) {
             best.t = t; best.u = u; best.v = v; best.inst = ii; best.prim = pid;
@@ -744,6 +770,7 @@
   traverse_persistent<kCurves, kCount, kMotion, kInstLds, false>(S, pol, tune, n, &cnt->trace_xcd_head[0][0], make_stack(s_stack, S.stack_overflow, kCurves ? s_rayspace : nullptr), &lc, s_inst);
   if (kCount) {
     flush_counters(cnt, lc.nodes, lc.prims, lc.insts, 0, 0);
+    flush_hole_skips(cnt, lc.hole_skips);
     flush_stack_peak(&cnt->stack_peak, lc.stack_peak);
     if (blockIdx.x == 0 && threadIdx.x == 0) atomicAdd(&cnt->traced, (unsigned long long) n);
   }
@@ -766,6 +793,7 @@
   traverse_phased<kCount, false, kInstLds>(S, pol, tune, n, &cnt->trace_xcd_head[0][0], make_stack(s_stack, S.stack_overflow, nullptr, FJ_STACK_LDS), &lc, s_inst);
   if (kCount) {
     flush_counters(cnt, lc.nodes, lc.prims, lc.insts, 0, 0);
+    flush_hole_skips(cnt, lc.hole_skips);
     flush_stack_peak(&cnt->stack_peak, lc.stack_peak);
     if (blockIdx.x == 0 && threadIdx.x == 0) atomicAdd(&cnt->traced, (unsigned long long) n);
   }
diff --git a/fujiyama-renderer_amd/csrc/device/fjgpu_frame.hip b/fujiyama-renderer_amd/csrc/device/fjgpu_frame.hip
--- a/fujiyama-renderer_amd/csrc/device/fjgpu_frame.hip
+++ b/fujiyama-renderer_amd/csrc/device/fjgpu_frame.hip
@@ -296,7 +296,7 @@
   swp.pre_resolve = (S.all_opaque && !S.has_curves && !S.has_motion && S.blas_base) ? 1 : 0;
   swp.cast_shadow = r->cast_shadow;
   S.compact_squeue = scene_compact_squeue(S) ? 1 : 0;
-  S.pad_cs_ = 0;
+  S.inst_holes = sc->inst_holes ? 1 : 0;
   swp.compact = S.compact_squeue;
   swp.light_cones = (sc->light_cones && S.light_cones && S.cone_rows) ? 1 : 0;
   swp.pad_ = 0;
@@ -658,6 +658,7 @@
   sc->stack_peak_closest = std::max(sc->stack_peak_closest, hc.stack_peak);
   sc->stack_peak_shadow = std::max(sc->stack_peak_shadow, hc.sh_stack_peak);
   sc->hull_verdicts += hc.hull_settled;
+  sc->hole_skips += hc.hole_skips;
   acc->batches++;
 }
 
@@ -669,6 +670,7 @@
   hipStream_t st = static_cast<hipStream_t>(hip_stream);
   sc->stack_peak_closest = sc->stack_peak_shadow = 0;
   sc->hull_verdicts = 0;
+  sc->hole_skips = 0;
   sc->accum_memsets = 0;
 
   FramePlan P;
diff --git a/fujiyama-renderer_amd/csrc/device/fjgpu_inst_hole.h b/fujiyama-renderer_amd/csrc/device/fjgpu_inst_hole.h
--- /dev/null
+++ b/fujiyama-renderer_amd/csrc/device/fjgpu_inst_hole.h
@@ -0,0 +1,169 @@
+#ifndef FJGPU_INST_HOLE_H
+#define FJGPU_INST_HOLE_H
+
+#include <stdint.h>
+#include <vector>
+
+#if defined(__HIPCC__) || defined(__CUDACC__)
+#define FJ_IH_FN __host__ __device__ __forceinline__
+#else
+#define FJ_IH_FN static inline
+#endif
+
+#define FJ_IH_DELTA 1e-9
+#define FJ_IH_MIN_SCALE 1e-3
+#define FJ_IH_REACH 64.
+#define FJ_IH_MAX_COND 256.
+
+FJ_IH_FN double ih_abs(double x) { return __builtin_fabs(x); }
+FJ_IH_FN double ih_min(double a, double b) { return a < b ? a : b; }
+FJ_IH_FN double ih_max(double a, double b) { return a > b ? a : b; }
+
+FJ_IH_FN void inst_hole_none(float *hole)
+{
+  for (int a = 0; a < 3; a++) { hole[a] = __builtin_inff(); hole[3 + a] = -__builtin_inff(); }
+}
+FJ_IH_FN bool inst_hole_present(const float *hole) { return hole[0] < hole[3] && hole[1] < hole[4] && hole[2] < hole[5]; }
+
+FJ_IH_FN bool inst_hole_verdict(const float *hole, double ox, double oy, double oz, double dx, double dy, double dz, double tmin, double tfar)
+{
+  const double lx = (double) hole[0], ly = (double) hole[1], lz = (double) hole[2];
+  const double hx = (double) hole[3], hy = (double) hole[4], hz = (double) hole[5];
+  const double ax = ox + tmin * dx, bx = ox + tfar * dx;
+  bool in = tmin >= 0. && tmin + tmin <= tfar;
+  in = in && ax > lx && ax < hx && bx > lx && bx < hx;
+  const double ay = oy + tmin * dy, by = oy + tfar * dy;
+  in = in && ay > ly && ay < hy && by > ly && by < hy;
+  const double az = oz + tmin * dz, bz = oz + tfar * dz;
+  in = in && az > lz && az < hz && bz > lz && bz < hz;
+  return in;
+}
+
+
+FJ_IH_FN void inst_hole_tri_box(const double *M, const double *P, int64_t n_points, const int32_t *idx, int64_t f, double delta, double *b)
+{
+  for (int a = 0; a < 3; a++) { b[a] = __builtin_inf(); b[3 + a] = -__builtin_inf(); }
+  for (int k = 0; k < 3; k++) {
+    const int64_t p = idx[3 * f + k];
+    if (p < 0 || p >= n_points) { for (int a = 0; a < 6; a++) b[a] = __builtin_nan(""); return; }
+    const double *v = P + 3 * p;
+    for (int a = 0; a < 3; a++) {
+      const double w = M[4 * a] * v[0] + M[4 * a + 1] * v[1] + M[4 * a + 2] * v[2] + M[4 * a + 3];
+      b[a] = !(w >= b[a]) ? w : b[a];
+      b[3 + a] = !(w <= b[3 + a]) ? w : b[3 + a];
+    }
+  }
+  for (int a = 0; a < 3; a++) { b[a] -= delta; b[3 + a] += delta; }
+}
+
+FJ_IH_FN double inst_hole_pass_scale(const double *M, const double *P, int64_t n_points, const int32_t *idx, int64_t f0, int64_t f1, double delta, const double *c, const double *h)
+{
+  double s = __builtin_inf();
+  for (int64_t f = f0; f < f1 && s > 0.; f++) {
+    double b[6], si = 0.;
+    inst_hole_tri_box(M, P, n_points, idx, f, delta, b);
+    for (int a = 0; a < 3; a++) {
+      const double g = ih_max(b[a] - c[a], c[a] - b[3 + a]);
+      if (!(g == g)) return 0.;
+      if (g > 0.) si = ih_max(si, h[a] > 0. ? g / h[a] : __builtin_inf());
+    }
+    s = ih_min(s, si);
+  }
+  return s;
+}
+
+FJ_IH_FN double inst_hole_pass_extend(const double *M, const double *P, int64_t n_points, const int32_t *idx, int64_t f0, int64_t f1, double delta, const double *box, int axis, int side)
+{
+  const int a1 = (axis + 1) % 3, a2 = (axis + 2) % 3;
+  double lim = side ? __builtin_inf() : -__builtin_inf();
+  for (int64_t f = f0; f < f1; f++) {
+    double b[6];
+    inst_hole_tri_box(M, P, n_points, idx, f, delta, b);
+    if (!(b[a1] <= box[3 + a1] && b[3 + a1] >= box[a1] && b[a2] <= box[3 + a2] && b[3 + a2] >= box[a2])) continue;
+    if (side) { if (b[3 + axis] >= box[3 + axis]) lim = ih_min(lim, ih_max(b[axis], box[3 + axis])); }
+    else { if (b[axis] <= box[axis]) lim = ih_max(lim, ih_min(b[3 + axis], box[axis])); }
+  }
+  return lim;
+}
+
+FJ_IH_FN int inst_hole_pass_verify(const double *M, const double *P, int64_t n_points, const int32_t *idx, int64_t f0, int64_t f1, double delta, const double *box)
+{
+  for (int64_t f = f0; f < f1; f++) {
+    double b[6];
+    inst_hole_tri_box(M, P, n_points, idx, f, delta, b);
+    bool apart = false;
+    for (int a = 0; a < 3; a++) apart = apart || b[a] >= box[3 + a] || b[3 + a] <= box[a];
+    if (!apart) return 1;
+  }
+  return 0;
+}
+
+FJ_IH_FN float inst_hole_f32_up(double x) { float f = (float) x; if ((double) f < x) f = __builtin_nextafterf(f, __builtin_inff()); return f; }
+FJ_IH_FN float inst_hole_f32_down(double x) { float f = (float) x; if ((double) f > x) f = __builtin_nextafterf(f, -__builtin_inff()); return f; }
+
+FJ_IH_FN double inst_hole_ext(const double *M, const double *Minv, const double *tb)
+{
+  double ext = 0., na = 0., ni = 0., tr = 0.;
+  for (int k = 0; k < 6; k++) ext = ih_max(ext, ih_abs(tb[k]));
+  for (int a = 0; a < 3; a++) {
+    na = ih_max(na, (ih_abs(M[4 * a]) + ih_abs(M[4 * a + 1])) + ih_abs(M[4 * a + 2]));
+    ni = ih_max(ni, (ih_abs(Minv[4 * a]) + ih_abs(Minv[4 * a + 1])) + ih_abs(Minv[4 * a + 2]));
+    tr = ih_max(tr, ih_abs(M[4 * a + 3]));
+  }
+  if (!(ext > 0.) || !(ext < 1e150)) return 0.;
+  if (!(na * ni <= FJ_IH_MAX_COND) || !(tr <= FJ_IH_REACH * ext)) return 0.;
+  return ext;
+}
+
+#define FJ_IH_CHUNK 16384
+template <class Run>
+static inline int inst_hole_build(const double *M, const double *Minv, const double *P, int64_t n_points, const int32_t *idx, int64_t n_faces, const double *tb, float *hole, int *passes, Run run)
+{
+  inst_hole_none(hole);
+  if (passes) *passes = 0;
+  const double ext = inst_hole_ext(M, Minv, tb);
+  if (n_faces <= 0 || !P || !idx || !(ext > 0.)) return 0;
+  const double delta = FJ_IH_DELTA * ext, reach = FJ_IH_REACH * ext;
+  double c[3], h[3];
+  for (int a = 0; a < 3; a++) {
+    if (!(tb[a] <= tb[3 + a]) || !(ih_abs(tb[a]) < 1e150) || !(ih_abs(tb[3 + a]) < 1e150)) return 0;
+    c[a] = .5 * (tb[a] + tb[3 + a]); h[a] = .5 * (tb[3 + a] - tb[a]);
+  }
+  const int64_t nch = (n_faces + FJ_IH_CHUNK - 1) / FJ_IH_CHUNK;
+  std::vector<double> partv((std::size_t) nch, 0.);
+  double *part = partv.data();
+  auto lo_of = [&](int64_t ch) { return ch * (int64_t) FJ_IH_CHUNK; };
+  auto hi_of = [&](int64_t ch) { const int64_t e = (ch + 1) * (int64_t) FJ_IH_CHUNK; return e < n_faces ? e : n_faces; };
+  run(nch, [&](int64_t ch) { part[ch] = inst_hole_pass_scale(M, P, n_points, idx, lo_of(ch), hi_of(ch), delta, c, h); });
+  if (passes) (*passes)++;
+  double s = __builtin_inf();
+  for (int64_t ch = 0; ch < nch; ch++) s = ih_min(s, part[ch]);
+  s = ih_min(s, 1.) * (1. - 1e-9);
+  if (!(s >= FJ_IH_MIN_SCALE)) return 0;
+  double box[6];
+  for (int a = 0; a < 3; a++) { box[a] = ih_max(c[a] - s * h[a], -reach); box[3 + a] = ih_min(c[a] + s * h[a], reach); }
+  for (int a = 0; a < 3; a++)
+    for (int side = 0; side < 2; side++) {
+      run(nch, [&](int64_t ch) { part[ch] = inst_hole_pass_extend(M, P, n_points, idx, lo_of(ch), hi_of(ch), delta, box, a, side); });
+      if (passes) (*passes)++;
+      double lim = side ? reach : -reach;
+      for (int64_t ch = 0; ch < nch; ch++) lim = side ? ih_min(lim, part[ch]) : ih_max(lim, part[ch]);
+      if (side) box[3 + a] = ih_max(box[3 + a], lim); else box[a] = ih_min(box[a], lim);
+    }
+  float out[6];
+  double stored[6];
+  for (int a = 0; a < 3; a++) {
+    out[a] = inst_hole_f32_up(box[a]); out[3 + a] = inst_hole_f32_down(box[3 + a]);
+    stored[a] = (double) out[a]; stored[3 + a] = (double) out[3 + a];
+  }
+  int ok = inst_hole_present(out) ? 1 : 0;
+  if (ok) {
+    run(nch, [&](int64_t ch) { part[ch] = (double) inst_hole_pass_verify(M, P, n_points, idx, lo_of(ch), hi_of(ch), delta, stored); });
+    if (passes) (*passes)++;
+    for (int64_t ch = 0; ch < nch; ch++) if (part[ch] != 0.) ok = 0;
+  }
+  if (ok) for (int k = 0; k < 6; k++) hole[k] = out[k];
+  return ok;
+}
+
+#endif
diff --git a/fujiyama-renderer_amd/csrc/device/fjgpu_kernels.h b/fujiyama-renderer_amd/csrc/device/fjgpu_kernels.h
--- a/fujiyama-renderer_amd/csrc/device/fjgpu_kernels.h
+++ b/fujiyama-renderer_amd/csrc/device/fjgpu_kernels.h
@@ -87,6 +87,7 @@
 void set_anyhit_filter_off(long v);
 void light_cone_validate_counts(double *verdicts, double *contradictions);
 void light_hull_validate_counts(double *verdicts, double *contradictions);
+void inst_hole_validate_counts(double *verdicts, double *contradictions);
 void tri_filter_validate_counts(double out[5]);
 bool kernels_build_config(const char *name, double *value);
 void debug_phase_stats();
diff --git a/fujiyama-renderer_amd/csrc/device/fjgpu_kernels.hip b/fujiyama-renderer_amd/csrc/device/fjgpu_kernels.hip
--- a/fujiyama-renderer_amd/csrc/device/fjgpu_kernels.hip
+++ b/fujiyama-renderer_amd/csrc/device/fjgpu_kernels.hip
@@ -15,6 +15,7 @@
 #include "fjgpu_dev_math.h"
 #include "fjgpu_tri_filter.h"
 #include "fjgpu_light_cone.h"
+#include "fjgpu_inst_hole.h"
 #include "fjgpu_dev_curve.h"
 #include "fjgpu_dev_traverse.h"
 #include "fjgpu_dev_flat.h"
@@ -419,6 +420,15 @@
 #endif
 }
 
+void inst_hole_validate_counts(double *verdicts, double *contradictions)
+{
+  *verdicts = -1; *contradictions = -1;
+#ifdef FJ_INST_HOLE_VALIDATE
+  unsigned long long c[2];
+  if (hipMemcpyFromSymbol(c, HIP_SYMBOL(g_insthole), sizeof(c)) == hipSuccess) { *verdicts = (double) c[0]; *contradictions = (double) c[1]; }
+#endif
+}
+
 void tri_filter_validate_counts(double out[5])
 {
   for (int k = 0; k < 5; k++) out[k] = -1;
@@ -448,6 +458,11 @@
     {"light_hull_validate", 1},
 #else
     {"light_hull_validate", 0},
+#endif
+#ifdef FJ_INST_HOLE_VALIDATE
+    {"inst_hole_validate", 1},
+#else
+    {"inst_hole_validate", 0},
 #endif
   };
   for (const auto &t : table) if (!strcmp(name, t.name)) { *value = t.value; return true; }
diff --git a/fujiyama-renderer_amd/csrc/device/fjgpu_scene.h b/fujiyama-renderer_amd/csrc/device/fjgpu_scene.h
--- a/fujiyama-renderer_amd/csrc/device/fjgpu_scene.h
+++ b/fujiyama-renderer_amd/csrc/device/fjgpu_scene.h
@@ -33,6 +33,9 @@
   long light_hulls = 1;
   int hull_rows = 0, hull_records = 0;
   unsigned long long hull_verdicts = 0;
+  long inst_holes = 1;
+  int hole_records = 0;
+  unsigned long long hole_skips = 0;
   long count_all_shadow;
   long shade_first_touch = 1;
   unsigned long long accum_memsets = 0;
diff --git a/fujiyama-renderer_amd/csrc/device/fjgpu_types.h b/fujiyama-renderer_amd/csrc/device/fjgpu_types.h
--- a/fujiyama-renderer_amd/csrc/device/fjgpu_types.h
+++ b/fujiyama-renderer_amd/csrc/device/fjgpu_types.h
@@ -105,6 +105,7 @@
   double tbounds[6];
   double pbounds[6];
   double qorigin[3], qcell[3];
+  float hole[6];
   const void *nodes;
   const double *tri_verts;
   const float *tri_verts32;
@@ -117,8 +118,8 @@
   int32_t primset;
   int32_t xform;
 };
-#define FJ_INST_LDS_ENTRY_WORDS 38
-#define FJ_INST_LDS_NODES 39
+#define FJ_INST_LDS_ENTRY_WORDS 41
+#define FJ_INST_LDS_NODES 38
 #define FJ_INST_LDS_INSTS 16
 #define FJ_INST_LDS_GROUPS 12
 #define FJ_INST_LDS_NODES_BIG 79
@@ -129,6 +130,9 @@
 #define FJ_INST_LDS_GROUPS_CURVES 12
 #define FJ_FLAT_LDS_INSTS 80
 #define FJ_INST_LDS_BYTES (FJ_INST_LDS_NODES * 56 + FJ_INST_LDS_INSTS * 8 * FJ_INST_LDS_ENTRY_WORDS + FJ_INST_LDS_GROUPS * 64)
+static_assert(FJ_INST_LDS_BYTES <= 160 * 1024 / 4 - FJ_STACK_LDS * 256 * 4 || FJ_STACK_LDS != 32, "the phased walk's instance level: 4 blocks per CU");
+static_assert(FJ_INST_LDS_NODES_BIG * 56 + FJ_INST_LDS_INSTS_BIG * 8 * FJ_INST_LDS_ENTRY_WORDS + FJ_INST_LDS_GROUPS_BIG * 64 <= 160 * 1024 / 3 - FJ_STACK_LDS * 256 * 4 || FJ_STACK_LDS != 32,
+              "k_trace_closest / k_shadow_trace: 3 blocks per CU");
 
 struct DAnyInst {
   double Minv[12];
@@ -230,7 +234,7 @@
   int32_t incoherent_rays;
   const double *cam_uv;
   int32_t compact_squeue;
-  int32_t pad_cs_;
+  int32_t inst_holes;
   const uint32_t *cam_tk;
   const uint32_t *ray_perm;
   const double *trace_ranges;
@@ -326,7 +330,10 @@
   uint32_t shadow_xcd_head[8][32];
   uint32_t trace_xcd_head[8][32];
   uint32_t join_count;
-  uint32_t pad4_[31];
-};
-
-#endif
+  uint32_t pad4a_;
+  unsigned long long hole_skips;
+  uint32_t pad4_[28];
+};
+static_assert(sizeof(DCounters) == 5 * 128 + 2 * 8 * 128, "DCounters: five lines and the per-XCD heads");
+
+#endif
diff --git a/fujiyama-renderer_amd/gpu.py b/fujiyama-renderer_amd/gpu.py
--- a/fujiyama-renderer_amd/gpu.py
+++ b/fujiyama-renderer_amd/gpu.py
@@ -446,6 +446,21 @@
     _check(min(0, L.fjgpu_host_light_hulls(scene_desc_ptr, group, rec.ctypes.data_as(C.c_void_p), Pl.ctypes.data_as(C.c_void_p), n,
                                            M.ctypes.data_as(C.c_void_p))))
     return rec, Pl, M
+
+
+def host_inst_holes(scene_desc_ptr):
+    L = lib()
+    L.fjgpu_host_inst_holes.argtypes = [C.c_void_p, C.c_void_p, C.c_void_p, C.c_void_p, C.c_int]
+    L.fjgpu_host_inst_holes.restype = C.c_int
+    n = L.fjgpu_host_inst_holes(scene_desc_ptr, None, None, None, 0)
+    if n < 0:
+        _check(n)
+    holes = np.zeros((n, 6), dtype=np.float32)
+    M = np.zeros((n, 3, 4), dtype=np.float64)
+    tb = np.zeros((n, 6), dtype=np.float64)
+    _check(min(0, L.fjgpu_host_inst_holes(scene_desc_ptr, holes.ctypes.data_as(C.c_void_p), M.ctypes.data_as(C.c_void_p),
+                                          tb.ctypes.data_as(C.c_void_p), n)))
+    return holes, M, tb
 
 
 def host_curve_blas(scene_desc_ptr, curve_set):
diff --git a/include/fjgpu.h b/include/fjgpu.h
--- a/include/fjgpu.h
+++ b/include/fjgpu.h
@@ -216,6 +216,8 @@
 
 int fjgpu_host_light_hulls(const fj_scene_desc *desc, int group, void *out_records, double *out_Pl, int cap, double *out_M);
 
+int fjgpu_host_inst_holes(const fj_scene_desc *desc, float *out_holes, double *out_M, double *out_tbounds, int cap);
+
 int fjgpu_host_curve_blas(const fj_scene_desc *desc, int curve_set, int32_t *out_curve, float *out_capsule, int32_t *out_depth,
                           float *out_box, int cap, int32_t *out_grid_n, double *out_grid_cell, double *out_bounds);
 
```

Measured after the change: 42170 Mray/s (median of 5 runs). About the same (+1.3%).
